# alvinliu0/HumanGaussian

Measured on AMD Instinct MI355X. Metric: rasterize fwd+bwd Gaussians/sec @1024^2, 100k pts, higher is better.
Workload: dtype f32

## Files before the change

### humangaussian_amd/csrc/api.hip

```cpp
#include "hgs_common.h"
#include <stdio.h>
#include <stdlib.h>
#include <algorithm>
#include <atomic>
#include <mutex>

#ifdef HGS_TIMELINE
__device__ unsigned long long hgs_tl[HGS_TL_KERNELS][HGS_TL_SLOTS][4];
#endif
#include "preprocess.hip"
#include "binning.hip"
#include "render_fwd.hip"
#include "knn.hip"
#include "mesh.hip"
#include "fields.hip"
#include "bookkeeping.hip"

extern "C" __global__ void hgs_k_render_bwd(View, Layout, const hgs_status*, const SortRec*, const float*,
                                            const float*, const float*, const float*, const float*,
                                            const float*, const float*, float*, uint32_t);
extern "C" __global__ void hgs_k_pair_reduce_em(View, Layout, const hgs_status*, const SortRec*, const float*, float*, uint32_t, uint32_t);
extern "C" __global__ void hgs_k_pair_reduce_ch(View, Layout, const hgs_status*, const SortRec*, const float*, float*, uint32_t, uint32_t);

namespace {

#ifdef HGS_KNOBS
inline int hgs_knob(const char* name, int dflt) { const char* e = getenv(name); return (e && atoi(e) > 0) ? atoi(e) : dflt; }
#else
inline int hgs_knob(const char*, int dflt) { return dflt; }
#endif

#define HGS_CHUNK_ROWS_MIN_VIEWS 3
#ifndef HGS_PRE_BWD_VPAR_MIN_VIEWS
#define HGS_PRE_BWD_VPAR_MIN_VIEWS 2
#endif
constexpr size_t ALIGN = 256;
struct Carver {
  size_t off = 0;
  size_t take(size_t bytes) { const size_t o = off; off = hgs_align_up(off + bytes, ALIGN); return o; }
};
constexpr size_t HGS_LDS_BINS_MAX = 16384;
#define HGS_BIN_WGS_PER_VIEW_MAX 512
#define HGS_BIN_WGS_TOTAL_MAX 1024
constexpr int HGS_MAX_BIN_WGS_PER_VIEW = HGS_BIN_WGS_PER_VIEW_MAX;
constexpr int HGS_BIN_WGS_TOTAL = HGS_BIN_WGS_TOTAL_MAX;

struct GeomCarve {
  size_t geom, tile_n, tile_start, tile_order, tile_rec, cell_info, items_part, fwd_cells,
      hist, tile_gbase, tile_count, chunk_sums, chunk_base, ctr, status, total;
};

inline int grid_dim(int pixels) { return (pixels + HGS_TILE - 1) / HGS_TILE; }

inline void bin_shape(int B, int P, int& nblk, int& cpw, int& nwg) {
  nblk = (P + HGS_BLOCK - 1) / HGS_BLOCK;
  int want = HGS_BIN_WGS_TOTAL / (B > 0 ? B : 1);
  if (want > HGS_MAX_BIN_WGS_PER_VIEW) want = HGS_MAX_BIN_WGS_PER_VIEW;
  if (want < 1) want = 1;
  cpw = (nblk + want - 1) / want;
  if (cpw < 1) cpw = 1;
  nwg = (nblk + cpw - 1) / cpw;
}

GeomCarve carve_geom(int B, int P, int H, int W) {
  const size_t T = (size_t)grid_dim(W) * grid_dim(H);
  const size_t TT = T * (size_t)B;
  int nblk, cpw, nwg;
  bin_shape(B, P, nblk, cpw, nwg);
  const bool lds = T <= HGS_LDS_BINS_MAX;
  GeomCarve c;
  Carver cv;
  c.geom = cv.take((size_t)B * P * sizeof(GeomRec));
  c.tile_n = cv.take(TT * 4);
  c.tile_start = cv.take(TT * 4);
  c.tile_order = cv.take(TT * 4);
  c.tile_rec = cv.take(TT * 16);
  c.cell_info = cv.take(TT * 16 * sizeof(CellInfo));
  const size_t dcap = hgs_die_cells((int)TT);
  c.items_part = cv.take(HGS_NXCD * 2 * dcap * sizeof(uint4));
  c.fwd_cells = cv.take((size_t)HGS_NXCD * HGS_NFC * dcap * 4);
  c.hist = cv.take(lds ? (size_t)B * nwg * T * 4 : 0);
  c.tile_gbase = cv.take(lds ? (size_t)HGS_ROW_GROUPS * TT * 4 : 0);
  c.tile_count = cv.take(lds ? 0 : TT * 4);
  c.chunk_sums = cv.take((size_t)B * nblk * 4);
  c.chunk_base = cv.take((size_t)B * nblk * 4);
  c.ctr = cv.take(sizeof(Counters));
  c.status = cv.take(sizeof(hgs_status));
  c.total = cv.off;
  return c;
}

struct BinCarve { size_t keys, recs, cell_list, entpair, cstate, items_full, total; };

BinCarve carve_bin(int64_t cap) {
  BinCarve c;
  Carver cv;
  const size_t C = (size_t)(cap > 0 ? cap : 0);
  const size_t NP = C * HGS_PAIRS_PER_ENTRY;
  c.keys = cv.take(C * 8);
  c.recs = cv.take(C * sizeof(SortRec));
  c.cell_list = cv.take(NP * 8);
  c.entpair = cv.take(C * 8);
  c.cstate = cv.take((NP / HGS_SEGLEN + 1) * HGS_CSTATE_FLOATS * sizeof(float));
// ... 355 lines not shown
    if ((scales != nullptr) != (rotations != nullptr)) return HGS_ESHAPE;
    if (has_sr == (cov3D_precomp != nullptr)) return HGS_ESHAPE;
    if (shs && M < (s->sh_degree + 1) * (s->sh_degree + 1)) return HGS_ESHAPE;
    if (entry_capacity > 0 && !bin) return HGS_EINVAL;
    if ((int64_t)B * P >= (1ll << 31) || P >= (1 << 28)) return HGS_EINVAL;
  }
  if (entry_capacity > HGS_MAX_ENTRY_CAPACITY) return HGS_EINVAL;
  hipStream_t stream = static_cast<hipStream_t>(stream_);
  DeviceState* const ds = device_state(stream);
  const int ncu = cu_count(ds);
  const bool aa = (activation_flags & HGS_ANTIALIAS) != 0;
  const View v = make_view(s, B, P, M, entry_capacity, max_tile_entries_hint > 0 ? max_tile_entries_hint : 0,
                           activation_flags & 7);
  const Layout L = make_layout(geom, bin, img, B, P, v.H, v.W, entry_capacity);
  hgs_status* status_dev =
      reinterpret_cast<hgs_status*>(static_cast<char*>(geom) + carve_geom(B, P, v.H, v.W).status);

  HGS_STAGE(0);
  hipError_t e = hipSuccess;
  if (v.nblk == 0) {
    e = hipMemsetAsync(L.ctr, 0, sizeof(Counters), stream);
    if (e != hipSuccess) return hip_rc(e);
  }
  const size_t lds_bytes = (size_t)v.T * 4;
  if (!v.lds_bins) {
    e = hipMemsetAsync(L.tile_count, 0, (size_t)v.TT * 4, stream);
    if (e != hipSuccess) return hip_rc(e);
  }
  if (v.nblk > 0) {
    if (v.lds_bins)
      hipLaunchKernelGGL(aa ? hgs_k_preprocess_fwd_aa : hgs_k_preprocess_fwd, dim3(v.B * v.nwg), dim3(HGS_BLOCK), lds_bytes,
                         stream, v, L, means3D, shs, colors_precomp, opacities, scales, rotations,
                         cov3D_precomp, radii, means2D_leaf);
    else
      hipLaunchKernelGGL(aa ? hgs_k_preprocess_fwd_ga_aa : hgs_k_preprocess_fwd_ga, dim3(v.B * v.nblk), dim3(HGS_BLOCK), 0,
                         stream, v, L, means3D, shs, colors_precomp, opacities, scales, rotations,
                         cov3D_precomp, radii, means2D_leaf);
    HGS_LAUNCH_CHECK();
  }
  HGS_STAGE(1);
  const unsigned bpv = (unsigned)((v.T + HGS_TILES_PER_WG - 1) / HGS_TILES_PER_WG);
  hipLaunchKernelGGL(hgs_k_tiles, dim3(bpv * (unsigned)v.B), dim3(64 * HGS_ROW_GROUPS), 0, stream, v, L);
  HGS_LAUNCH_CHECK();
  HGS_STAGE(2);
  const unsigned order_wgs = (unsigned)((v.TT + HGS_BLOCK - 1) / HGS_BLOCK);
  hgs_status* status_mapped = status_host_mapped ? status_host : nullptr;
  const unsigned nbin = entry_capacity > 0 ? (unsigned)(v.B * (v.lds_bins ? v.nwg : v.nblk)) : 0u;
  if (v.lds_bins && nbin)
    hipLaunchKernelGGL(hgs_k_fill, dim3(nbin + order_wgs), dim3(HGS_BLOCK), lds_bytes, stream, v, L, status_dev,
                       status_mapped, (int)nbin);
  else
    hipLaunchKernelGGL(hgs_k_fill_ga, dim3(nbin + order_wgs), dim3(HGS_BLOCK), 0, stream, v, L, status_dev,
                       status_mapped, (int)nbin);
  HGS_LAUNCH_CHECK();
  if (status_host && !status_host_mapped) {
    e = hipMemcpyAsync(status_host, status_dev, sizeof(hgs_status), hipMemcpyDeviceToHost, stream);
    if (e != hipSuccess) return hip_rc(e);
  }
  if (status_event) {
    e = hipEventRecord(static_cast<hipEvent_t>(status_event), stream);
    if (e != hipSuccess) return hip_rc(e);
  }
  if (entry_capacity > 0) {
    HGS_STAGE(3);
    auto class_grid = [&](int64_t lo) {
      const int64_t g = entry_capacity / lo + 1;
      return (unsigned)(g < v.TT ? g : v.TT);
    };
    const int hint = v.max_tile_hint;
    const bool need_huge = hint <= 0 || hint > 16384, need_large = hint <= 0 || hint > HGS_SORT_LDS_MAX;
    const bool expect_long = hint <= 0 || hint > HGS_SORT_LDS_MAX + HGS_SORT_LDS_MAX / 2 + 64;
    SideStream* side = ((need_huge || need_large) && expect_long) ? side_stream(ds) : nullptr;
    {
      std::unique_lock<std::mutex> side_lk;
      hipStream_t s2 = stream;
      if (side) {
        side_lk = std::unique_lock<std::mutex>(side->mu);
        e = hipEventRecord(side->fork, stream);
        if (e == hipSuccess) e = hipStreamWaitEvent(side->s, side->fork, 0);
        if (e != hipSuccess) return hip_rc(e);
        s2 = side->s;
      }
      if (need_huge) {
        hipLaunchKernelGGL(hgs_k_sort_huge, dim3(class_grid(16384)), dim3(1024), 0, s2, v, L, status_dev);
        HGS_LAUNCH_CHECK();
      }
      if (need_large) {
        hipLaunchKernelGGL(hgs_k_sort_large, dim3(class_grid(HGS_SORT_LDS_MAX)), dim3(1024), 0, s2, v, L, status_dev);
        HGS_LAUNCH_CHECK();
      }
      if (side) {
        e = hipEventRecord(side->join, side->s);
        if (e != hipSuccess) return hip_rc(e);
      }
      const unsigned sort_wgs = std::min<unsigned>(class_grid(1), (unsigned)(hgs_knob("HGS_SORT_WGS_PER_CU", 3) * ncu));
      hipLaunchKernelGGL(v.pairchunks ? hgs_k_sort_lds_ch : hgs_k_sort_lds, dim3(sort_wgs), dim3(HGS_SORT_NT), 0, stream, v, L,
                         status_dev);
      HGS_LAUNCH_CHECK();
      if (side) {
        e = hipStreamWaitEvent(stream, side->join, 0);
        if (e != hipSuccess) return hip_rc(e);
      }
    }
  } else {
    HGS_STAGE(3);
  }
  HGS_STAGE(4);
  {
    const int64_t cells = std::min<int64_t>((int64_t)16 * v.TT, (int64_t)HGS_PAIRS_PER_ENTRY * entry_capacity);
    const int64_t fwd_blocks = (int64_t)hgs_knob("HGS_FWD_BLOCKS_PER_CU", 4) * ncu;
    const unsigned cell_blocks = (unsigned)std::max<int64_t>(4, std::min<int64_t>(fwd_blocks, (cells + 3) / 4) & ~int64_t(3));
    const unsigned bg_blocks = (unsigned)v.TT;
    hipLaunchKernelGGL(store_bwd_state ? hgs_k_render_fwd_store : hgs_k_render_fwd_nostore, dim3(cell_blocks + bg_blocks),
                       dim3(HGS_FWD_THREADS), 0, stream, v, L, cell_blocks, status_dev, status_mapped, L.recs, L.cstate,
                       out_color, out_depth, out_alpha);
  }
  HGS_LAUNCH_CHECK();
  HGS_STAGE(5);
  return HGS_OK;
}

int hgs_forward_batch(const hgs_settings* s, int32_t B, int32_t P, int32_t M, const float* means3D,
                      const float* shs, const float* colors_precomp, const float* opacities,
                      const float* scales, const float* rotations, const float* cov3D_precomp,
                      float* out_color, float* out_depth, float* out_alpha, int32_t* radii,
                      void* geom, void* bin, int64_t entry_capacity, void* img,
                      int32_t store_bwd_state, int32_t max_tile_entries_hint, hgs_status* status_host,
                      int32_t status_host_mapped, void* status_event, void* const* stage_events,
                      void* stream_) {
  return hgs_forward_batch_act(s, B, P, M, means3D, shs, colors_precomp, opacities, scales, rotations, cov3D_precomp,
                               out_color, out_depth, out_alpha, radii, geom, bin, entry_capacity, img, store_bwd_state,
                               max_tile_entries_hint, status_host, status_host_mapped, status_event, stage_events, 0,
                               stream_);
}

int hgs_forward(const hgs_settings* s, int32_t P, int32_t M, const float* means3D,
                const float* shs, const float* colors_precomp, const float* opacities,
                const float* scales, const float* rotations, const float* cov3D_precomp,
                float* out_color, float* out_depth, float* out_alpha, int32_t* radii,
                void* geom, void* bin, int64_t entry_capacity, void* img,
                int32_t store_bwd_state, int32_t max_tile_entries_hint, hgs_status* status_host,
                int32_t status_host_mapped, void* status_event, void* const* stage_events,
                void* stream_) {
  return hgs_forward_batch(s, 1, P, M, means3D, shs, colors_precomp, opacities, scales, rotations,
                           cov3D_precomp, out_color, out_depth, out_alpha, radii, geom, bin, entry_capacity,
                           img, store_bwd_state, max_tile_entries_hint, status_host, status_host_mapped,
                           status_event, stage_events, stream_);
}

}

namespace {
int backward_impl(const hgs_settings* s, int32_t B, int32_t P, int32_t M, const float* means3D,
                           const float* shs, const float* colors_precomp, const float* opacities,
                           const float* scales, const float* rotations, const float* cov3D_precomp,
                           const int32_t* radii, const float* out_color, const float* out_depth,
                           const float* out_alpha, const float* dL_dout_color,
                           const float* dL_dout_depth, const float* dL_dout_alpha, const void* geom,
                           const void* bin, const void* img, const hgs_status* status,
                           int64_t entry_capacity, void* bwd_scratch, float* dL_dmeans3D, float* dL_dmeans2D, float* dL_dshs,
                           float* dL_dcolors_precomp, float* dL_dopacities, float* dL_dscales,
                           float* dL_drotations, float* dL_dcov3D_precomp, void* const* stage_events,
                           int32_t activation_flags, float* pack, int32_t pack_F, void* stream_) {
  (void)radii;
  if (activation_flags & ~(7 | HGS_GRAD_SCALE_TRUE_DERIVATIVE | HGS_ANTIALIAS)) return HGS_EINVAL;
  if ((activation_flags & (HGS_ACT_OPACITY_SIGMOID | HGS_ANTIALIAS)) && P > 0 && !opacities) return HGS_EINVAL;
  if (!batch_ok(s, B) || P < 0 || !geom || !img || entry_capacity < 0 || entry_capacity > HGS_MAX_ENTRY_CAPACITY) return HGS_EINVAL;
  if (status && status->overflow) return HGS_EINVAL;
  if (status && (int64_t)status->reserved[0] != entry_capacity) return HGS_EINVAL;
  if (P == 0) return HGS_OK;
  if (!means3D || !out_color || !out_depth || !out_alpha) return HGS_EINVAL;
  if ((shs != nullptr) == (colors_precomp != nullptr)) return HGS_ESHAPE;
  if ((scales != nullptr) != (rotations != nullptr)) return HGS_ESHAPE;
  if ((scales != nullptr) == (cov3D_precomp != nullptr)) return HGS_ESHAPE;
  if (shs && !dL_dshs) return HGS_EINVAL;
  const bool maybe_entries = status ? status->num_rendered > 0 : entry_capacity > 0;
  if (maybe_entries && (!bin || !bwd_scratch)) return HGS_EINVAL;
  hipStream_t stream = static_cast<hipStream_t>(stream_);
  DeviceState* const ds = device_state(stream);
  const int64_t cap = entry_capacity;
  const View v = make_view(s, B, P, M, cap, 0, activation_flags);
  const Layout L = make_layout(const_cast<void*>(geom), const_cast<void*>(bin),
                               const_cast<void*>(img), B, P, v.H, v.W, cap);
  const hgs_status* status_dev = reinterpret_cast<const hgs_status*>(
      static_cast<const char*>(geom) + carve_geom(B, P, v.H, v.W).status);
  const int64_t X = status ? (int64_t)status->num_rendered : cap;
  const int64_t worst = X * HGS_PAIRS_PER_ENTRY;
  const int64_t pc = (status && status->num_pairs > 0 && (int64_t)status->num_pairs < worst) ? (int64_t)status->num_pairs : worst;
  const uint32_t pair_cap = (uint32_t)(pc > 0xffffffffll ? 0xffffffffll : pc);
  float* rows = static_cast<float*>(bwd_scratch);
  float* pair_rows = rows + (size_t)X * HGS_ROW_FLOATS;
  HGS_STAGE(0);
  if (maybe_entries) {
    const int resident = hgs_knob("HGS_BWD_WAVES_PER_CU", 12) * cu_count(ds);
    hipLaunchKernelGGL(hgs_k_render_bwd, dim3((unsigned)std::max(HGS_NXCD, resident / HGS_BWD_BLOCK_WAVES / HGS_NXCD * HGS_NXCD)), dim3(64 * HGS_BWD_BLOCK_WAVES), 0, stream, v, L, status_dev, L.recs, L.cstate,
                       out_color, out_depth, out_alpha, dL_dout_color, dL_dout_depth, dL_dout_alpha, pair_rows, pair_cap);
    HGS_LAUNCH_CHECK();
    HGS_STAGE(1);
    if (X > 0) {
      const uint32_t R_host = status ? status->num_rendered : 0xffffffffu;
      hipLaunchKernelGGL(v.pairchunks ? hgs_k_pair_reduce_ch : hgs_k_pair_reduce_em, dim3((unsigned)((X + 255) / 256)), dim3(256), 0,
                         stream, v, L, status_dev, L.recs, pair_rows, rows, pair_cap, R_host);
      HGS_LAUNCH_CHECK();
    }
  }
  if (!maybe_entries) HGS_STAGE(1);
  HGS_STAGE(2);
  const int deg = shs ? v.D : 0;
  const int nc = (deg + 1) * (deg + 1);
  const int aa = (activation_flags & HGS_ANTIALIAS) ? 1 : 0;
  const unsigned thr_p = 64u * (unsigned)v.B;
  const size_t lds_p = (size_t)(23 + 3 * nc) * thr_p * sizeof(float);
  const int row_p = hgs_pre_bwd_row(aa, 2, deg);
  const bool vpar_ok = v.B >= HGS_PRE_BWD_VPAR_MIN_VIEWS && thr_p <= (unsigned)hgs_pre_bwd_forms.row[row_p].threads &&
                       (lds_p <= 65536 || pre_bwd_lds_raised(ds, row_p));
  const int mode = v.B == 1 ? 1 : (vpar_ok ? 2 : 0);
  const PreBwdForm& form = hgs_pre_bwd_forms.row[hgs_pre_bwd_row(aa, mode, deg)];
  const unsigned grid = mode == 2 ? (unsigned)((v.P + 63) / 64) : (unsigned)v.nblk, threads = mode == 2 ? thr_p : HGS_BLOCK;
  const size_t lds = mode == 2 ? lds_p : (mode == 1 ? hgs_pre_bwd_stage_bytes(M, deg, shs != nullptr && dL_dshs != nullptr) : 0);
  hipLaunchKernelGGL(form.kernel, dim3(grid), dim3(threads), lds, stream, v, L, status_dev, rows, means3D, shs,
                     colors_precomp, opacities, scales, rotations, cov3D_precomp, dL_dmeans3D, dL_dmeans2D,
                     dL_dshs, dL_dcolors_precomp, dL_dopacities, dL_dscales, dL_drotations,
                     dL_dcov3D_precomp, pack, (int)pack_F);
  HGS_LAUNCH_CHECK();
  HGS_STAGE(3);
  return HGS_OK;
}
}

extern "C" {

int hgs_backward_batch_act(const hgs_settings* s, int32_t B, int32_t P, int32_t M, const float* means3D,
                           const float* shs, const float* colors_precomp, const float* opacities,
                           const float* scales, const float* rotations, const float* cov3D_precomp,
                           const int32_t* radii, const float* out_color, const float* out_depth,
                           const float* out_alpha, const float* dL_dout_color,
                           const float* dL_dout_depth, const float* dL_dout_alpha, const void* geom,
                           const void* bin, const void* img, const hgs_status* status,
                           int64_t entry_capacity, void* bwd_scratch, float* dL_dmeans3D, float* dL_dmeans2D, float* dL_dshs,
                           float* dL_dcolors_precomp, float* dL_dopacities, float* dL_dscales,
                           float* dL_drotations, float* dL_dcov3D_precomp, void* const* stage_events,
                           int32_t activation_flags, void* stream_) {
  return backward_impl(s, B, P, M, means3D, shs, colors_precomp, opacities, scales, rotations, cov3D_precomp, radii, out_color,
                       out_depth, out_alpha, dL_dout_color, dL_dout_depth, dL_dout_alpha, geom, bin, img, status,
                       entry_capacity, bwd_scratch, dL_dmeans3D, dL_dmeans2D, dL_dshs, dL_dcolors_precomp, dL_dopacities,
                       dL_dscales, dL_drotations, dL_dcov3D_precomp, stage_events, activation_flags, nullptr, 0, stream_);
}

int hgs_backward_batch_packed(const hgs_settings* s, int32_t B, int32_t P, int32_t M, const float* means3D,
                              const float* shs, const float* opacities, const float* scales, const float* rotations,
                              const int32_t* radii, const float* out_color, const float* out_depth, const float* out_alpha,
                              const float* dL_dout_color, const float* dL_dout_depth, const float* dL_dout_alpha,
                              const void* geom, const void* bin, const void* img, const hgs_status* status,
                              int64_t entry_capacity, void* bwd_scratch, float* pack, float* dL_dmeans2D_views,
                              void* const* stage_events, int32_t activation_flags, void* stream_) {
  if (!pack || !shs || !scales || !rotations || M < 1) return P == 0 ? HGS_OK : HGS_EINVAL;
  float* marker = pack;
  return backward_impl(s, B, P, M, means3D, shs, nullptr, opacities, scales, rotations, nullptr, radii, out_color, out_depth,
                       out_alpha, dL_dout_color, dL_dout_depth, dL_dout_alpha, geom, bin, img, status, entry_capacity,
                       bwd_scratch, marker, dL_dmeans2D_views, marker, nullptr, marker, marker, marker, nullptr, stage_events,
                       activation_flags, pack, 15 + 3 * M, stream_);
}

int hgs_backward_batch(const hgs_settings* s, int32_t B, int32_t P, int32_t M, const float* means3D,
                       const float* shs, const float* colors_precomp, const float* opacities,
                       const float* scales, const float* rotations, const float* cov3D_precomp,
                       const int32_t* radii, const float* out_color, const float* out_depth,
                       const float* out_alpha, const float* dL_dout_color,
                       const float* dL_dout_depth, const float* dL_dout_alpha, const void* geom,
                       const void* bin, const void* img, const hgs_status* status,
                       int64_t entry_capacity, void* bwd_scratch, float* dL_dmeans3D, float* dL_dmeans2D, float* dL_dshs,
                       float* dL_dcolors_precomp, float* dL_dopacities, float* dL_dscales,
                       float* dL_drotations, float* dL_dcov3D_precomp, void* const* stage_events,
                       void* stream_) {
  return hgs_backward_batch_act(s, B, P, M, means3D, shs, colors_precomp, opacities, scales, rotations, cov3D_precomp,
                                radii, out_color, out_depth, out_alpha, dL_dout_color, dL_dout_depth, dL_dout_alpha,
                                geom, bin, img, status, entry_capacity, bwd_scratch, dL_dmeans3D, dL_dmeans2D, dL_dshs,
                                dL_dcolors_precomp, dL_dopacities, dL_dscales, dL_drotations, dL_dcov3D_precomp,
// ... 372 lines not shown
```

### humangaussian_amd/csrc/binning.hip

```cpp
#include "hgs_common.h"

extern "C" __global__ void __launch_bounds__(64 * HGS_ROW_GROUPS)
hgs_k_tiles(View v, Layout L) {
  __shared__ uint32_t gt[HGS_ROW_GROUPS][HGS_TILES_PER_WG];
  __shared__ uint32_t start_s[HGS_TILES_PER_WG];
  __shared__ uint32_t cls_s[HGS_NCLS];
  const int tid = threadIdx.x, tl = tid & 63;
  const int rg = __builtin_amdgcn_readfirstlane(tid >> 6);
  const int bpv = (v.T + HGS_TILES_PER_WG - 1) / HGS_TILES_PER_WG;
  const int b = (int)blockIdx.x / bpv;
  const int t = ((int)blockIdx.x % bpv) * HGS_TILES_PER_WG + tl;
  const bool valid = t < v.T;
  const size_t g = (size_t)b * v.T + t;
  if (tid < HGS_NCLS) cls_s[tid] = 0;
  uint32_t run = 0;
  if (v.lds_bins) {
    const int rpg = (v.nwg + HGS_ROW_GROUPS - 1) / HGS_ROW_GROUPS;
    const int r0 = rg * rpg, r1 = min(v.nwg, r0 + rpg);
    if (valid) {
      uint32_t* col = L.hist + (size_t)b * v.nwg * v.T + t;
      constexpr int BR = 16;
      for (int r = r0; r < r1; r += BR) {
        uint32_t c[BR];
#pragma unroll
// ... 99 lines not shown
  const int g = blk * HGS_BLOCK + tid;
  const bool valid = g < v.TT;
  const uint32_t n = valid ? L.tile_n[g] : 0u;
  const int c = (valid && n) ? 32 - __clz(n) : 0;
  int leader_of = 0;
  uint32_t rank = 0, cnt = 0;
  unsigned long long todo = __ballot(valid);
  while (todo) {
    const int leader = (int)__builtin_ctzll(todo);
    const int cl = __builtin_amdgcn_readlane(c, leader);
    const unsigned long long same = __ballot(valid && c == cl);
    if (valid && c == cl) {
      leader_of = leader;
      rank = __builtin_amdgcn_mbcnt_hi((uint32_t)(same >> 32), __builtin_amdgcn_mbcnt_lo((uint32_t)same, 0u));
      cnt = (uint32_t)__popcll(same);
    }
    todo &= ~same;
  }
  uint32_t base = 0;
  if (valid && lane == leader_of) base = atomicAdd(&L.ctr->cls_cur[c].v, cnt);
  base = (uint32_t)__shfl((int)base, leader_of, 64);
  const uint32_t pos = cls_base[c] + base + rank;
  if (!valid) return;
  L.tile_order[pos] = (uint32_t)g;
  L.tile_rec[pos] = make_uint4((uint32_t)g, n, L.tile_start[g], 0u);
}

extern "C" __global__ void __launch_bounds__(HGS_BLOCK)
hgs_k_fill(View v, Layout L, hgs_status* __restrict__ status, hgs_status* __restrict__ status_host, int nbin) {
  extern __shared__ __attribute__((aligned(16))) uint32_t lds_cur[];
  if ((int)blockIdx.x >= nbin) {
    place_tiles(v, L, (int)blockIdx.x - nbin, (int)gridDim.x - nbin, status, status_host);
    return;
  }
  if (overflow_from_counters(v, L)) return;
  const int b = (int)blockIdx.x / v.nwg, lw = (int)blockIdx.x % v.nwg;
  const uint32_t* __restrict__ base_row = L.hist + (size_t)blockIdx.x * v.T;
  const int rpg = (v.nwg + HGS_ROW_GROUPS - 1) / HGS_ROW_GROUPS;
  const uint32_t* __restrict__ grp_row = L.tile_gbase + (size_t)(lw / rpg) * v.TT + (size_t)b * v.T;
  for (int t = threadIdx.x; t < v.T; t += HGS_BLOCK) lds_cur[t] = grp_row[t] + base_row[t];
  __syncthreads();
  const GeomRec* __restrict__ geom = L.geom + (size_t)b * v.P;
  for (int c = 0; c < v.cpw; ++c) {
    const int chunk = lw * v.cpw + c;
    if (chunk >= v.nblk) break;
    const int i = chunk * HGS_BLOCK + threadIdx.x;
    if (i >= v.P) continue;
    const uint4 q2 = reinterpret_cast<const uint4*>(&geom[i])[2];
    const uint32_t depth_bits = q2.y, lo = q2.z, hi = q2.w;
    const int minx = lo & 0xffffu, miny = lo >> 16, maxx = hi & 0xffffu, maxy = hi >> 16;
    const unsigned long long key_hi = (unsigned long long)depth_bits << 32;
    for (int ty = miny; ty < maxy; ++ty)
      for (int tx = minx; tx < maxx; ++tx) {
        const uint32_t slot = atomicAdd(&lds_cur[ty * v.grid_x + tx], 1u);
        L.keys[slot] = key_hi | (uint32_t)i;
      }
  }
}

extern "C" __global__ void __launch_bounds__(HGS_BLOCK)
hgs_k_fill_ga(View v, Layout L, hgs_status* __restrict__ status, hgs_status* __restrict__ status_host, int nbin) {
  if ((int)blockIdx.x >= nbin) {
    place_tiles(v, L, (int)blockIdx.x - nbin, (int)gridDim.x - nbin, status, status_host);
    return;
  }
  if (overflow_from_counters(v, L)) return;
  const int b = (int)blockIdx.x / v.nblk, chunk = (int)blockIdx.x % v.nblk;
  const int i = chunk * HGS_BLOCK + threadIdx.x;
  if (i >= v.P) return;
  const uint4 q2 = reinterpret_cast<const uint4*>(&L.geom[(size_t)b * v.P + i])[2];
  const uint32_t depth_bits = q2.y, lo = q2.z, hi = q2.w;
  const int minx = lo & 0xffffu, miny = lo >> 16, maxx = hi & 0xffffu, maxy = hi >> 16;
  const unsigned long long key_hi = (unsigned long long)depth_bits << 32;
  for (int ty = miny; ty < maxy; ++ty)
    for (int tx = minx; tx < maxx; ++tx) {
      const size_t g = (size_t)b * v.T + ty * v.grid_x + tx;
      const uint32_t slot = L.tile_start[g] + atomicAdd(&L.tile_count[g], 1u);
      L.keys[slot] = key_hi | (uint32_t)i;
    }
}

namespace {

__device__ __forceinline__ void hgs_put_pair(const Layout& L, uint32_t rec, uint32_t row_id, uint32_t slot) {
  L.cell_list[slot] = make_uint2(rec, row_id);
}

struct CellAlloc {
  uint32_t len, nfull, rem, nst, i_len, i_st, i_full, pcls, fcls, frank, die;
  unsigned long long b1, b2, b3, got;
};

__device__ __forceinline__ void hgs_alloc_cell_ranges_issue(const Layout& L, uint32_t order_pos, uint32_t len_of_lane, CellAlloc& a) {
  const int lane = (int)threadIdx.x & 63;
  a.die = order_pos % HGS_NXCD;
  const bool cl = lane < 16;
  a.len = cl ? len_of_lane : 0u;
  a.nfull = a.len / HGS_SEGLEN; a.rem = a.len % HGS_SEGLEN;
  const uint32_t nseg = a.nfull + (a.rem ? 1u : 0u);
  a.nst = nseg ? nseg - 1u : 0u;
  a.i_len = hgs_wave_incl_scan(a.len); a.i_st = hgs_wave_incl_scan(a.nst); a.i_full = hgs_wave_incl_scan(a.nfull);
  a.pcls = a.rem ? hgs_item_class(a.rem) : 0u;
  a.b1 = __ballot(a.pcls == 1u); a.b2 = __ballot(a.pcls == 2u); a.b3 = __ballot(a.pcls == 3u);
  const uint32_t t_len = (uint32_t)__builtin_amdgcn_readlane((int)a.i_len, 63);
  const uint32_t t_st = (uint32_t)__builtin_amdgcn_readlane((int)a.i_st, 63);
  const uint32_t t_full = (uint32_t)__builtin_amdgcn_readlane((int)a.i_full, 63);
  a.fcls = hgs_cell_class(a.len);
  unsigned long long fb_ = 0;
  a.frank = 0;
#pragma unroll
  for (int c = 0; c < HGS_NFC; ++c) {
    const unsigned long long bc = __ballot(cl && a.len && a.fcls == (uint32_t)c);
    if (lane == 3 + c) fb_ = bc;
    if (a.fcls == (uint32_t)c) a.frank = (uint32_t)__popcll(bc & ((1ull << lane) - 1ull));
  }
  const unsigned long long add = lane == 0 ? ((unsigned long long)t_len | ((unsigned long long)t_st << 32))
                               : lane == 1 ? ((unsigned long long)t_full | ((unsigned long long)__popcll(a.b1) << 32))
                               : lane == 2 ? ((unsigned long long)__popcll(a.b2) | ((unsigned long long)__popcll(a.b3) << 32))
                                           : (unsigned long long)__popcll(fb_);
  a.got = 0;
  unsigned long long* ctr = lane == 0 ? &L.ctr->alloc_ps : &L.ctr->sched[a.die][min(lane, 2 + HGS_NFC) - 1];
  if (lane < 3 + HGS_NFC && add) a.got = atomicAdd(ctr, add);
}

__device__ __forceinline__ void hgs_alloc_cell_ranges_finish(const View& v, const Layout& L, int g, const CellAlloc& a,
                                                             uint32_t* cell_base, uint32_t& pair_base_out) {
  int lane = (int)threadIdx.x & 63;
  asm volatile("" : "+v"(lane));
  const bool cl = lane < 16;
  const uint32_t fpos = (uint32_t)__shfl((int)(uint32_t)a.got, 3 + (int)a.fcls, 64) + a.frank;
  const uint32_t got_lo = (uint32_t)a.got, got_hi = (uint32_t)(a.got >> 32);
  const uint32_t pb = (uint32_t)__builtin_amdgcn_readlane((int)got_lo, 0);
  const uint32_t sb = (uint32_t)__builtin_amdgcn_readlane((int)got_hi, 0);
  const uint32_t fb = (uint32_t)__builtin_amdgcn_readlane((int)got_lo, 1);
  const uint32_t p1 = (uint32_t)__builtin_amdgcn_readlane((int)got_hi, 1);
  const uint32_t p2 = (uint32_t)__builtin_amdgcn_readlane((int)got_lo, 2);
  const uint32_t p3 = (uint32_t)__builtin_amdgcn_readlane((int)got_hi, 2);
  if (cl) {
    const uint32_t len = a.len, nfull = a.nfull, rem = a.rem;
    const uint32_t base = pb + a.i_len - len;
    cell_base[lane] = base;
    CellInfo ci;
    ci.base = base; ci.len = len; ci.sbase = sb + a.i_st - a.nst; ci.pbase = pb;
    L.cell_info[(size_t)g * 16 + lane] = ci;
    const uint32_t key = (uint32_t)g * 16u + (uint32_t)lane;
    const size_t dcap = hgs_die_cells(v.TT);
    if (len) L.fwd_cells[((size_t)a.die * HGS_NFC + a.fcls) * dcap + fpos] = key;
    uint4* full = L.items_full + ((size_t)a.die * L.full_cap + fb + a.i_full - nfull);
    for (uint32_t sgm = 0; sgm < nfull; ++sgm)
      full[sgm] = make_uint4(key, HGS_SEGLEN, base + sgm * HGS_SEGLEN, sgm ? ci.sbase + sgm - 1u : 0xffffffffu);
    if (rem) {
      const unsigned long long below = (1ull << lane) - 1ull;
      uint4* part = L.items_part + (size_t)a.die * 2 * dcap;
      const uint4 it = make_uint4(key, rem, base + nfull * HGS_SEGLEN, nfull ? ci.sbase + nfull - 1u : 0xffffffffu);
      if (a.pcls == 1u) part[p1 + (uint32_t)__popcll(a.b1 & below)] = it;
      else if (a.pcls == 2u) part[dcap - 1 - (p2 + (uint32_t)__popcll(a.b2 & below))] = it;
      else part[dcap + p3 + (uint32_t)__popcll(a.b3 & below)] = it;
    }
  }
  if (lane == 0) pair_base_out = pb;
}

__device__ __forceinline__ void hgs_alloc_cell_ranges(const View& v, const Layout& L, int g, uint32_t order_pos, const uint32_t* cell_tot,
                                                      uint32_t* cell_base, uint32_t& pair_base_out) {
  if (threadIdx.x < 64) {
    CellAlloc a;
    hgs_alloc_cell_ranges_issue(L, order_pos, (threadIdx.x & 63) < 16 ? cell_tot[threadIdx.x & 63] : 0u, a);
    hgs_alloc_cell_ranges_finish(v, L, g, a, cell_base, pair_base_out);
  }
}

template <int MAXCH>
struct GatherLds {
  uint32_t tab[MAXCH][17];
  uint32_t run[17];
  uint32_t cell_tot[16];
  uint32_t cell_base[16];
  uint32_t pair_base;
};

template <int MAXCH>
__device__ __forceinline__ void gather_records(const View& v, const Layout& L, int g, uint32_t order_pos,
                                               uint32_t start, uint32_t n,
                                               unsigned long long* sorted, int nt, GatherLds<MAXCH>& S) {
  const int t = g % v.T;
  const GeomRec* __restrict__ geom = L.geom + (size_t)(g / v.T) * v.P;
  const uint32_t* __restrict__ cbase = L.chunk_base + (size_t)(g / v.T) * v.nblk;
  const int tx = t % v.grid_x, ty = t / v.grid_x;
  const float x0 = (float)(tx * HGS_TILE), y0 = (float)(ty * HGS_TILE);
  const int tid = (int)threadIdx.x, lane = tid & 63;
  const int wv = tid >> 6, nwaves = nt >> 6;
  if (tid < 16) S.cell_tot[tid] = 0;
  if (tid < 17) S.run[tid] = 0;
  __syncthreads();
  constexpr int GU = 4;
  uint32_t mytot = 0;
  for (uint32_t kb0 = 0; kb0 < n; kb0 += (uint32_t)nt * GU) {
    const uint32_t kb = kb0 + threadIdx.x;
    uint32_t idxv[GU];
    uint4 q0[GU], q1[GU], q2[GU];
    uint32_t q3[GU];
#pragma unroll
    for (int u = 0; u < GU; ++u) {
      const uint32_t k = kb + (uint32_t)u * nt;
      idxv[u] = (k < n) ? (uint32_t)sorted[k] : 0u;
    }
#pragma unroll
    for (int u = 0; u < GU; ++u) {
      const uint32_t k = kb + (uint32_t)u * nt;
      if (k < n) {
        const uint4* gp = reinterpret_cast<const uint4*>(&geom[idxv[u]]);
        q0[u] = gp[0]; q1[u] = gp[1]; q2[u] = gp[2]; q3[u] = gp[3].x;
      }
    }
#pragma unroll
    for (int u = 0; u < GU; ++u) {
      const uint32_t k = kb + (uint32_t)u * nt;
      uint32_t mask = 0;
      if (k < n) {
        const uint32_t idx = idxv[u];
        const uint4 g0 = q0[u], g1 = q1[u], g2 = q2[u];
        const int minx = g2.z & 0xffffu, miny = g2.z >> 16, maxx = g2.w & 0xffffu;
        const uint32_t entry = cbase[idx >> 8] + q3[u] + (uint32_t)((ty - miny) * (maxx - minx) + (tx - minx));
        const float mx = __uint_as_float(g0.x), my = __uint_as_float(g0.y);
        const float ca = __uint_as_float(g0.z), cb = __uint_as_float(g0.w), cc = __uint_as_float(g1.x);
        mask = hgs_cell_mask(mx, my, ca, cb, cc, __uint_as_float(g1.y), x0, y0);
        uint4* dst = reinterpret_cast<uint4*>(&L.recs[start + k]);
        const float qa = -0.5f * ca * HGS_LOG2E, qb = -cb * HGS_LOG2E, qc = -0.5f * cc * HGS_LOG2E;
        dst[0] = make_uint4(g0.x, g0.y, __float_as_uint(qa), __float_as_uint(qb));
        dst[1] = make_uint4(__float_as_uint(qc), g1.y, g1.z, g1.w);
        dst[2] = make_uint4(g2.x, g2.y, entry, v.pairchunks ? hgs_rec_tag(mask, k, n, false) : 0u);
        L.entpair[start + k].x = entry | ((uint32_t)__popc(mask) << 27);
        sorted[k] = (unsigned long long)mask;
      }
#pragma unroll
      for (int c = 0; c < 16; ++c) {
        const unsigned long long bal = __ballot((mask >> c) & 1u);
        if (lane == c) mytot += (uint32_t)__popcll(bal);
      }
    }
  }
  if (lane < 16 && mytot) atomicAdd(&S.cell_tot[lane], mytot);
  __syncthreads();
  hgs_alloc_cell_ranges(v, L, g, order_pos, S.cell_tot, S.cell_base, S.pair_base);
  __syncthreads();
  const uint32_t pair_base = S.pair_base;
  for (uint32_t sc0 = 0; sc0 < n; sc0 += (uint32_t)MAXCH * 64u) {
    const uint32_t nch = min((uint32_t)MAXCH, (n - sc0 + 63u) / 64u);
    for (uint32_t ch = wv; ch < nch; ch += nwaves) {
      const uint32_t k = sc0 + ch * 64u + lane;
      const uint32_t mask = (k < n) ? (uint32_t)sorted[k] : 0u;
      uint32_t mine = 0;
#pragma unroll
      for (int c = 0; c < 16; ++c) {
        const unsigned long long bal = __ballot((mask >> c) & 1u);
        if (lane == c) mine = (uint32_t)__popcll(bal);
      }
      uint32_t tot = mine;
      tot += __builtin_amdgcn_update_dpp(0, (int)tot, HGS_DPP_ROW_SHR(1), 0xf, 0xf, false);
      tot += __builtin_amdgcn_update_dpp(0, (int)tot, HGS_DPP_ROW_SHR(2), 0xf, 0xf, false);
      tot += __builtin_amdgcn_update_dpp(0, (int)tot, HGS_DPP_ROW_SHR(4), 0xf, 0xf, false);
      tot += __builtin_amdgcn_update_dpp(0, (int)tot, HGS_DPP_ROW_SHR(8), 0xf, 0xf, false);
      if (lane < 16) S.tab[ch][lane] = mine;
      if (lane == 15) S.tab[ch][16] = tot;
    }
    __syncthreads();
    for (int col = wv; col < 17; col += nwaves) {
      uint32_t carry = S.run[col];
      for (uint32_t c0 = 0; c0 < nch; c0 += 64u) {
        const uint32_t ch = c0 + lane;
        const uint32_t x = ch < nch ? S.tab[ch][col] : 0u;
        const uint32_t inc = hgs_wave_incl_scan(x);
        if (ch < nch) S.tab[ch][col] = carry + inc - x;
        carry += (uint32_t)__builtin_amdgcn_readlane((int)inc, 63);
      }
      if (lane == 0) S.run[col] = carry;
    }
    __syncthreads();
    for (uint32_t ch = wv; ch < nch; ch += nwaves) {
      const uint32_t k = sc0 + ch * 64u + lane;
      const bool in = k < n;
      const uint32_t mask = in ? (uint32_t)sorted[k] : 0u;
      const uint32_t cnt = (uint32_t)__popc(mask);
      const uint32_t rel = S.tab[ch][16] + hgs_wave_incl_scan(cnt) - cnt;
      if (in) L.entpair[start + k].y = pair_base + rel;
#pragma unroll
      for (int c = 0; c < 16; ++c) {
        const bool bit = (mask >> c) & 1u;
        const unsigned long long bal = __ballot(bit);
        if (bit) {
          const uint32_t rank = S.tab[ch][c] + __builtin_amdgcn_mbcnt_hi((uint32_t)(bal >> 32), __builtin_amdgcn_mbcnt_lo((uint32_t)bal, 0u));
          const uint32_t slot = S.cell_base[c] + rank;
          hgs_put_pair(L, start + k, pair_base + rel + (uint32_t)__popc(mask & ((1u << c) - 1u)), slot);
        }
      }
    }
    __syncthreads();
  }
}

__device__ __forceinline__ uint32_t hgs_spread4(uint32_t nib) {
  return (nib * 0x00204081u) & 0x01010101u;
}
__device__ __forceinline__ uint32_t hgs_bytesum(uint32_t w) { return __builtin_amdgcn_sad_u8(w, 0u, 0u); }

template <int MAXCH>
__device__ __forceinline__ void gather_records_single(const View& v, const Layout& L, int g, uint32_t order_pos,
                                                      uint32_t start, uint32_t n,
                                                      unsigned long long* sorted, int nt, GatherLds<MAXCH>& S) {
  const int t = g % v.T;
  const GeomRec* __restrict__ geom = L.geom + (size_t)(g / v.T) * v.P;
  const uint32_t* __restrict__ cbase = L.chunk_base + (size_t)(g / v.T) * v.nblk;
  const int tx = t % v.grid_x, ty = t / v.grid_x;
  const float x0 = (float)(tx * HGS_TILE), y0 = (float)(ty * HGS_TILE);
  const int tid = (int)threadIdx.x, lane = tid & 63;
  const int wv = tid >> 6, nwaves = nt >> 6;
  const uint32_t nch = (n + 63u) / 64u;
#ifdef HGS_TIMELINE
  const unsigned long long tg0 = wall_clock64();
#define HGS_TG(i) const unsigned long long tg##i = wall_clock64()
#else
#define HGS_TG(i)
#endif
  constexpr int GU = 2;
  for (uint32_t kb0 = 0; kb0 < n; kb0 += (uint32_t)nt * GU) {
    const uint32_t kb = kb0 + threadIdx.x;
    uint32_t idxv[GU];
    uint4 q0[GU], q1[GU], q2[GU];
    uint32_t q3[GU];
#pragma unroll
    for (int u = 0; u < GU; ++u) {
      const uint32_t k = kb + (uint32_t)u * nt;
      idxv[u] = (k < n) ? (uint32_t)sorted[k] : 0u;
    }
#pragma unroll
    for (int u = 0; u < GU; ++u) {
      const uint32_t k = kb + (uint32_t)u * nt;
      if (k < n) {
        const uint4* gp = reinterpret_cast<const uint4*>(&geom[idxv[u]]);
        q0[u] = gp[0]; q1[u] = gp[1]; q2[u] = gp[2]; q3[u] = gp[3].x;
      }
    }
#pragma unroll
    for (int u = 0; u < GU; ++u) {
      const uint32_t k = kb + (uint32_t)u * nt;
      if (kb0 + (uint32_t)u * nt + (uint32_t)(wv * 64) >= n) continue;
      uint32_t mask = 0;
      if (k < n) {
        const uint32_t idx = idxv[u];
        const uint4 g0 = q0[u], g1 = q1[u], g2 = q2[u];
        const int minx = g2.z & 0xffffu, miny = g2.z >> 16, maxx = g2.w & 0xffffu;
        const uint32_t entry = cbase[idx >> 8] + q3[u] + (uint32_t)((ty - miny) * (maxx - minx) + (tx - minx));
        const float mx = __uint_as_float(g0.x), my = __uint_as_float(g0.y);
        const float ca = __uint_as_float(g0.z), cb = __uint_as_float(g0.w), cc = __uint_as_float(g1.x);
        mask = hgs_cell_mask(mx, my, ca, cb, cc, __uint_as_float(g1.y), x0, y0);
        uint4* dst = reinterpret_cast<uint4*>(&L.recs[start + k]);
        const float qa = -0.5f * ca * HGS_LOG2E, qb = -cb * HGS_LOG2E, qc = -0.5f * cc * HGS_LOG2E;
        dst[0] = make_uint4(g0.x, g0.y, __float_as_uint(qa), __float_as_uint(qb));
        dst[1] = make_uint4(__float_as_uint(qc), g1.y, g1.z, g1.w);
        dst[2] = make_uint4(g2.x, g2.y, entry, v.pairchunks ? hgs_rec_tag(mask, k, n, false) : 0u);
        L.entpair[start + k].x = entry | ((uint32_t)__popc(mask) << 27);
        sorted[k] = (unsigned long long)mask;
      }
      const uint32_t ch = k >> 6;
      uint32_t tot[4];
#pragma unroll
      for (int wd = 0; wd < 4; ++wd) tot[wd] = hgs_wave_incl_scan(hgs_spread4((mask >> (4 * wd)) & 0xfu));
      if (lane == 63) {
        S.tab[ch][0] = tot[0]; S.tab[ch][1] = tot[1]; S.tab[ch][2] = tot[2]; S.tab[ch][3] = tot[3];
        S.tab[ch][16] = hgs_bytesum(tot[0]) + hgs_bytesum(tot[1]) + hgs_bytesum(tot[2]) + hgs_bytesum(tot[3]);
      }
    }
  }
  __syncthreads();
  HGS_TG(1);
  {
    uint32_t pk[(MAXCH + 63) / 64][4];
#pragma unroll
    for (int r = 0; r < (MAXCH + 63) / 64; ++r) {
      const uint32_t ch = (uint32_t)r * 64u + lane;
#pragma unroll
      for (int wd = 0; wd < 4; ++wd) pk[r][wd] = (wv < 5 && ch < nch) ? S.tab[ch][wd] : 0u;
    }
    __syncthreads();
    for (int col = wv; col < 5; col += nwaves) {
      uint32_t carry[4] = {0u, 0u, 0u, 0u};
#pragma unroll
      for (int r = 0; r < (MAXCH + 63) / 64; ++r) {
        const uint32_t ch = (uint32_t)r * 64u + lane;
        if ((uint32_t)r * 64u >= nch) break;
        if (col < 4) {
#pragma unroll
          for (int b = 0; b < 4; ++b) {
            const uint32_t x = (pk[r][col] >> (8 * b)) & 0xffu;
            const uint32_t inc = hgs_wave_incl_scan(x);
            if (ch < nch) S.tab[ch][4 * col + b] = carry[b] + inc - x;
            carry[b] += (uint32_t)__builtin_amdgcn_readlane((int)inc, 63);
          }
        } else {
          const uint32_t x = ch < nch ? S.tab[ch][16] : 0u;
          const uint32_t inc = hgs_wave_incl_scan(x);
          if (ch < nch) S.tab[ch][16] = carry[0] + inc - x;
          carry[0] += (uint32_t)__builtin_amdgcn_readlane((int)inc, 63);
        }
      }
      if (col < 4 && lane < 4) S.cell_tot[4 * col + lane] = lane == 0 ? carry[0] : lane == 1 ? carry[1] : lane == 2 ? carry[2] : carry[3];
    }
  }
  __syncthreads();
  HGS_TG(2);
  hgs_alloc_cell_ranges(v, L, g, order_pos, S.cell_tot, S.cell_base, S.pair_base);
  __syncthreads();
  HGS_TG(3);
  const uint32_t pair_base = S.pair_base;
  for (uint32_t ch = wv; ch < nch; ch += nwaves) {
    const uint32_t k = ch * 64u + lane;
    const bool in = k < n;
    uint32_t mask = in ? (uint32_t)sorted[k] : 0u;
    uint32_t ex[4], before = 0;
#pragma unroll
    for (int wd = 0; wd < 4; ++wd) {
      const uint32_t mine = hgs_spread4((mask >> (4 * wd)) & 0xfu);
      ex[wd] = hgs_wave_incl_scan(mine) - mine;
      before += hgs_bytesum(ex[wd]);
    }
    const uint32_t rel = S.tab[ch][16] + before;
    if (in) L.entpair[start + k].y = pair_base + rel;
    uint32_t r = 0;
    while (mask) {
      const int c = __builtin_ctz(mask);
      mask &= mask - 1u;
      const uint32_t exw = (c < 8) ? (c < 4 ? ex[0] : ex[1]) : (c < 12 ? ex[2] : ex[3]);
      const uint32_t slot = S.cell_base[c] + S.tab[ch][c] + ((exw >> (8 * (c & 3))) & 0xffu);
      hgs_put_pair(L, start + k, pair_base + rel + r, slot);
      ++r;
    }
  }
#ifdef HGS_TIMELINE
  if (threadIdx.x == 0 && blockIdx.x < HGS_TL_SLOTS) {
    const unsigned long long tg4 = wall_clock64();
    auto cl = [](unsigned long long d) { return d > 0xffffull ? 0xffffull : d; };
    hgs_tl[2][blockIdx.x][0] = cl(tg1 - tg0) | (cl(tg2 - tg1) << 16) | (cl(tg3 - tg2) << 32) | (cl(tg4 - tg3) << 48);
  }
#endif
}

template <int NT>
__device__ __forceinline__ void bitonic_sort(unsigned long long* keys, uint32_t n) {
  uint32_t npad = 2;
  while (npad < n) npad <<= 1;
  const uint32_t half = npad >> 1;
  for (uint32_t kk = 2; kk <= npad; kk <<= 1) {
    const uint32_t hk = kk >> 1;
    for (uint32_t i = threadIdx.x; i < half; i += NT) {
      const uint32_t blk = i / hk, off = i - blk * hk;
      const uint32_t lo = blk * kk + off, hi = blk * kk + (kk - 1 - off);
      if (hi < n) {
        const unsigned long long a = keys[lo], c = keys[hi];
        if (a > c) { keys[lo] = c; keys[hi] = a; }
      }
    }
    __syncthreads();
    for (uint32_t j = kk >> 2; j > 0; j >>= 1) {
      for (uint32_t i = threadIdx.x; i < half; i += NT) {
        const uint32_t lo = ((i & ~(j - 1)) << 1) | (i & (j - 1));
        const uint32_t hi = lo | j;
        if (hi < n) {
          const unsigned long long a = keys[lo], c = keys[hi];
          if (a > c) { keys[lo] = c; keys[hi] = a; }
        }
      }
      __syncthreads();
    }
  }
}

typedef unsigned long long u64;

}

#define HGS_SORT_LIGHT 16
#define HGS_RANK_BUCKET_MAX 192
#define HGS_RANK_NB_MAX 2048
#define HGS_SORT_NT 256
#define HGS_SORT_WAVES_PER_EU 3
#define HGS_RANK_GU 2

namespace {

#ifdef HGS_TIMELINE
__shared__ unsigned long long hgs_s_tq[8];
#define HGS_TQ(i) { if (threadIdx.x == 0) hgs_s_tq[(i)] = wall_clock64(); }
#else
#define HGS_TQ(i) {}
#endif

__device__ __forceinline__ void lds_barrier() { asm volatile("s_waitcnt lgkmcnt(0)\n\ts_barrier" ::: "memory"); }

struct __attribute__((aligned(16))) RankLds {
  uint32_t hist[HGS_RANK_NB_MAX + 1];
  uint32_t wtot[16];
  uint32_t tot16[8];
  uint32_t dmin, dmax, maxcnt, pad;
};
static_assert(sizeof(uint32_t) * (HGS_RANK_NB_MAX + 1) >= sizeof(uint16_t) * 4096, "the masks of the longest list fit into the histogram");

template <int NT>
__device__ __forceinline__ void bucket_scan(RankLds& R, uint32_t NB) {
  int tid = (int)threadIdx.x;
  asm volatile("" : "+v"(tid));
  const int lane = tid & 63, wv = tid >> 6;
  const uint32_t PER = NB / (uint32_t)NT;
  uint32_t* __restrict__ h = R.hist + (uint32_t)tid * PER;
  uint32_t c[8];
  auto load_counts = [&]() {
#pragma unroll
    for (int i = 0; i < 8; ++i) c[i] = 0u;
    if (PER == 8u) {
      const uint4 a = *reinterpret_cast<const uint4*>(h), b = *reinterpret_cast<const uint4*>(h + 4);
      c[0] = a.x; c[1] = a.y; c[2] = a.z; c[3] = a.w; c[4] = b.x; c[5] = b.y; c[6] = b.z; c[7] = b.w;
    } else if (PER == 4u) {
      const uint4 a = *reinterpret_cast<const uint4*>(h);
      c[0] = a.x; c[1] = a.y; c[2] = a.z; c[3] = a.w;
    } else if (PER == 2u) {
      const uint2 a = *reinterpret_cast<const uint2*>(h);
      c[0] = a.x; c[1] = a.y;
    } else {
      c[0] = h[0];
    }
  };
  load_counts();
  uint32_t sum = 0, mx = 0;
#pragma unroll
  for (int i = 0; i < 8; ++i) { sum += c[i]; mx = max(mx, c[i]); }
  const uint32_t inc = hgs_wave_incl_scan(sum);
  mx = hgs_wave_max_u32(mx);
  if (lane == 63) R.wtot[wv] = inc;
  if (lane == 0 && mx) atomicMax(&R.maxcnt, mx);
  uint32_t base = inc - sum;
  asm volatile("" : "+v"(base));
  lds_barrier();
  load_counts();
#pragma unroll
  for (int w = 0; w < NT / 64; ++w) base += (w < wv) ? R.wtot[w] : 0u;
  uint32_t e[8];
#pragma unroll
  for (int i = 0; i < 8; ++i) { e[i] = base; base += c[i]; }
  if (PER == 8u) {
    *reinterpret_cast<uint4*>(h) = make_uint4(e[0], e[1], e[2], e[3]);
    *reinterpret_cast<uint4*>(h + 4) = make_uint4(e[4], e[5], e[6], e[7]);
  } else if (PER == 4u) {
    *reinterpret_cast<uint4*>(h) = make_uint4(e[0], e[1], e[2], e[3]);
  } else if (PER == 2u) {
    *reinterpret_cast<uint2*>(h) = make_uint2(e[0], e[1]);
  } else {
    h[0] = e[0];
  }
}

template <int NT, bool CH>
__device__ __forceinline__ void cell_lists_from_masks(const View& v, const Layout& L, uint32_t order_pos, uint32_t start, uint32_t n,
                                                      const uint16_t* __restrict__ masks, GatherLds<64>& S, const CellAlloc& ca,
                                                      unsigned long long* tp) {
  const int tid = (int)threadIdx.x, lane = tid & 63, wv = tid >> 6;
  constexpr int nwaves = NT / 64;
  const uint32_t nch = (n + 63u) / 64u;
  for (uint32_t ch = wv; ch < nch; ch += nwaves) {
    const uint32_t k = ch * 64u + lane;
    const uint32_t mask = (k < n) ? (uint32_t)masks[k] : 0u;
    uint32_t tot[4];
#pragma unroll
    for (int wd = 0; wd < 4; ++wd) tot[wd] = hgs_wave_incl_scan(hgs_spread4((mask >> (4 * wd)) & 0xfu));
    if (lane == 63) {
      S.tab[ch][0] = tot[0]; S.tab[ch][1] = tot[1]; S.tab[ch][2] = tot[2]; S.tab[ch][3] = tot[3];
      S.tab[ch][16] = hgs_bytesum(tot[0]) + hgs_bytesum(tot[1]) + hgs_bytesum(tot[2]) + hgs_bytesum(tot[3]);
    }
  }
  lds_barrier();
  {
    uint32_t pk[4];
    const uint32_t ch = (uint32_t)lane;
#pragma unroll
    for (int wd = 0; wd < 4; ++wd) pk[wd] = (ch < nch) ? S.tab[ch][wd] : 0u;
    lds_barrier();
    for (int col = wv; col < 5; col += nwaves) {
      if (col < 4) {
        const uint32_t word = col == 0 ? pk[0] : col == 1 ? pk[1] : col == 2 ? pk[2] : pk[3];
#pragma unroll
        for (int b = 0; b < 4; ++b) {
          const uint32_t x = (word >> (8 * b)) & 0xffu;
          const uint32_t inc = hgs_wave_incl_scan(x);
          if (ch < nch) S.tab[ch][4 * col + b] = inc - x;
        }
      } else {
        const uint32_t x = ch < nch ? S.tab[ch][16] : 0u;
        const uint32_t inc = hgs_wave_incl_scan(x);
        if (ch < nch) S.tab[ch][16] = inc - x;
      }
    }
  }
#ifdef HGS_TIMELINE
  tp[2] = wall_clock64();
#endif
  if (tid < 64) hgs_alloc_cell_ranges_finish(v, L, (int)L.tile_rec[order_pos].x, ca, S.cell_base, S.pair_base);
  lds_barrier();
#ifdef HGS_TIMELINE
  tp[3] = wall_clock64();
#endif
  const uint32_t pair_base = S.pair_base;
  for (uint32_t ch = wv; ch < nch; ch += nwaves) {
    const uint32_t k = ch * 64u + lane;
    const bool in = k < n;
    const uint32_t mask = in ? (uint32_t)masks[k] : 0u;
    uint32_t ex[4], before = 0;
    uint32_t tot[4];
#pragma unroll
    for (int wd = 0; wd < 4; ++wd) {
      const uint32_t mine = hgs_spread4((mask >> (4 * wd)) & 0xfu);
      const uint32_t inc = hgs_wave_incl_scan(mine);
      ex[wd] = inc - mine;
      if (CH) tot[wd] = (uint32_t)__builtin_amdgcn_readlane((int)inc, 63);
      before += hgs_bytesum(ex[wd]);
    }
    const uint32_t rel_chunk = pair_base + S.tab[ch][16];
    const uint32_t rel = rel_chunk + before;
    if (in) L.entpair[start + k].y = CH ? rel_chunk : rel;
    const uint32_t cb = lane < 16 ? S.cell_base[lane] + S.tab[ch][lane] : 0u;
    uint32_t cp = 0;
#pragma unroll
    for (int c = 0; c < 16; ++c) {
      const uint32_t cbase = (uint32_t)__builtin_amdgcn_readlane((int)cb, c);
      if ((mask >> c) & 1u) {
        const uint32_t exc = (ex[c >> 2] >> (8 * (c & 3))) & 0xffu;
        const uint32_t slot = cbase + exc;
        hgs_put_pair(L, start + k, CH ? rel_chunk + cp + exc : rel + (uint32_t)__popc(mask & ((1u << c) - 1u)), slot);
      }
      if (CH) cp += (tot[c >> 2] >> (8 * (c & 3))) & 0xffu;
    }
  }
}

template <int E, int NT>
__device__ __forceinline__ bool rank_keys(const Layout& L, uint32_t start, uint32_t n, uint32_t NB, const u64 (&keyp)[HGS_RANK_GU],
                                          unsigned long long* pairs, RankLds& R) {
  int tid = (int)threadIdx.x;
  asm volatile("" : "+v"(tid));
  const int lane = tid & 63, wv = tid >> 6;
  u64 key[E];
#pragma unroll
  for (int e = 0; e < E; ++e) {
    if (e < HGS_RANK_GU) key[e] = keyp[e];
    else {
      const uint32_t k = (uint32_t)e * NT + (uint32_t)tid;
      const u64 kv = L.keys[start + min(k, n - 1u)];
      key[e] = (k < n) ? kv : ~0ull;
    }
  }
  {
    uint32_t lo = 0xffffffffu, hi = 0u;
#pragma unroll
    for (int e = 0; e < E; ++e) {
      const uint32_t d = (uint32_t)(key[e] >> 32);
      lo = min(lo, d);
      hi = max(hi, key[e] != ~0ull ? d : 0u);
    }
    hi = hgs_wave_max_u32(hi);
    lo = ~hgs_wave_max_u32(~lo);
    lds_barrier();
    if (lane == 0) { atomicMin(&R.dmin, lo); atomicMax(&R.dmax, hi); }
  }
  lds_barrier();
  HGS_TQ(0)
  const float flo = __uint_as_float(R.dmin);
  const float range = __uint_as_float(R.dmax) - flo;
  const float scale = range > 1e-30f ? (float)NB / range : 0.0f;
  uint32_t bp[E];
#pragma unroll
  for (int e = 0; e < E; ++e) {
    bp[e] = 0u;
    if (key[e] != ~0ull) {
      const float x = (__uint_as_float((uint32_t)(key[e] >> 32)) - flo) * scale;
      const uint32_t bkt = (uint32_t)fminf(x, (float)(NB - 1u));
      bp[e] = bkt | (atomicAdd(&R.hist[bkt], 1u) << 12);
    }
  }
  lds_barrier();
  HGS_TQ(1)
  bucket_scan<NT>(R, NB);
  if (tid == 0) R.hist[NB] = n;
  lds_barrier();
  HGS_TQ(2)
  const bool degenerate = R.maxcnt > (uint32_t)HGS_RANK_BUCKET_MAX;
  if (!degenerate) {
    constexpr int EG = E < 8 ? E : 8;
    uint32_t lmax[E / EG];
#pragma unroll
    for (int h = 0; h < E / EG; ++h) lmax[h] = 0u;
#pragma unroll
    for (int e = 0; e < E; ++e) {
      if (key[e] != ~0ull) {
        const uint32_t j0 = R.hist[bp[e] & 0xfffu], j1 = R.hist[(bp[e] & 0xfffu) + 1u];
        pairs[j0 + (bp[e] >> 12)] = key[e];
        bp[e] = j0 | ((j1 - j0) << 12);
        lmax[e / EG] = max(lmax[e / EG], j1 - j0);
      }
    }
    lds_barrier();
    HGS_TQ(3)
#pragma unroll
    for (int h = 0; h < E / EG; ++h) {
      for (uint32_t sidx = 0; sidx < lmax[h]; ++sidx) {
        u64 other[EG];
#pragma unroll
        for (int e = 0; e < EG; ++e) {
          const uint32_t w = bp[h * EG + e];
          const bool on = sidx < ((w >> 12) & 0xffu);
          other[e] = pairs[on ? (w & 0xfffu) + sidx : 0u];
        }
// ... 48 lines not shown
    }
    hi = hgs_wave_max_u32(hi);
    lo = ~hgs_wave_max_u32(~lo);
    lds_barrier();
    if (lane == 0) { atomicMin(&R.dmin, lo); atomicMax(&R.dmax, hi); }
  }
  lds_barrier();
  const float flo = __uint_as_float(R.dmin);
  const float range = __uint_as_float(R.dmax) - flo;
  const float scale = range > 1e-30f ? (float)NB / range : 0.0f;
  const float bmax = (float)(NB - 1u);
  auto bucket_of = [&](u64 key) { return (uint32_t)fminf((__uint_as_float((uint32_t)(key >> 32)) - flo) * scale, bmax); };
#pragma unroll 4
  for (uint32_t k = tid; k < n; k += NT) atomicAdd(&R.hist[bucket_of(keys[k])], 1u);
  lds_barrier();
  bucket_scan<NT>(R, NB);
  lds_barrier();
  const bool degenerate = R.maxcnt > (uint32_t)HGS_RANK_BUCKET_MAX;
  uint32_t rk[16];
  if (!degenerate) {
#pragma unroll 4
    for (uint32_t k = tid; k < n; k += NT) {
      const u64 key = keys[k];
      pairs[atomicAdd(&R.hist[bucket_of(key)], 1u)] = key;
    }
    lds_barrier();
#pragma unroll
    for (int e0 = 0; e0 < 16; e0 += 4) {
      if ((uint32_t)e0 * NT >= n) break;
      u64 key[4];
      uint32_t w[4], lmax = 0;
#pragma unroll
      for (int e = 0; e < 4; ++e) {
        const uint32_t k = (uint32_t)(e0 + e) * NT + (uint32_t)tid;
        key[e] = keys[min(k, last)];
      }
#pragma unroll
      for (int e = 0; e < 4; ++e) {
        const uint32_t k = (uint32_t)(e0 + e) * NT + (uint32_t)tid;
        const uint32_t b = bucket_of(key[e]);
        const uint32_t j1 = R.hist[b], j0 = b ? R.hist[b - 1u] : 0u;
        const uint32_t len = k < n ? j1 - j0 : 0u;
        w[e] = j0 | (len << JB);
        lmax = max(lmax, len);
      }
      for (uint32_t sidx = 0; sidx < lmax; ++sidx) {
        u64 other[4];
#pragma unroll
        for (int e = 0; e < 4; ++e) {
          const bool on = sidx < ((w[e] >> JB) & 0xffu);
          other[e] = pairs[on ? (w[e] & JM) + sidx : 0u];
        }
#pragma unroll
        for (int e = 0; e < 4; ++e) {
          const bool on = sidx < ((w[e] >> JB) & 0xffu);
          w[e] += (on && other[e] < key[e]) ? (1u << (JB + 8)) : 0u;
        }
      }
#pragma unroll
      for (int e = 0; e < 4; ++e) rk[e0 + e] = (w[e] & JM) + (w[e] >> (JB + 8));
    }
    lds_barrier();
#pragma unroll
    for (int e = 0; e < 16; ++e) {
      const uint32_t k = (uint32_t)e * NT + (uint32_t)tid;
      if (k < n) {
        if (SORTED) pairs[rk[e]] = keys[k];
        else pairs[k] = (keys[k] & 0xffffffffull) | ((u64)rk[e] << 32);
      }
    }
    if (SORTED) lds_barrier();
  } else {
    for (uint32_t k = tid; k < n; k += NT) pairs[k] = keys[k];
    __syncthreads();
    bitonic_sort<NT>(pairs, n);
    if (!SORTED) {
      for (uint32_t k = tid; k < n; k += NT) pairs[k] = (pairs[k] & 0xffffffffull) | ((u64)k << 32);
      lds_barrier();
    }
  }
  return degenerate;
}

template <int NT, bool CH>
__device__ __forceinline__ void rank_sort_tile(const View& v, const Layout& L, uint32_t order_pos, int g, uint32_t start, uint32_t n,
                                               unsigned long long* pairs, RankLds& R, GatherLds<64>& S, bool& degenerate_out,
                                               unsigned long long* tp) {
  const int tid = (int)threadIdx.x, lane = tid & 63;
  constexpr int GU = HGS_RANK_GU;
  const int t = g % v.T;
  const GeomRec* __restrict__ geom = L.geom + (size_t)(g / v.T) * v.P;
  const uint32_t* __restrict__ cbase = L.chunk_base + (size_t)(g / v.T) * v.nblk;
  const int tx = t % v.grid_x, ty = t / v.grid_x;
  const float x0 = (float)(tx * HGS_TILE), y0 = (float)(ty * HGS_TILE);
  uint32_t NB = 256u;
  while (NB < 2u * n && NB < (uint32_t)HGS_RANK_NB_MAX) NB <<= 1;
  for (uint32_t i = tid; i <= NB; i += NT) R.hist[i] = 0u;
  if (tid < 8) R.tot16[tid] = 0u;
  if (tid == 0) { R.dmin = 0xffffffffu; R.dmax = 0u; R.maxcnt = 0u; }
  u64 keyp[GU];
#pragma unroll
  for (int u = 0; u < GU; ++u) {
    const uint32_t k = (uint32_t)u * NT + (uint32_t)tid;
    const u64 kv = L.keys[start + min(k, n - 1u)];
    keyp[u] = (k < n) ? kv : ~0ull;
  }
  uint4 Aa[GU], Ab[GU], Ac[GU], Ba[GU], Bb[GU], Bc[GU];
  uint32_t Aoff[GU], Acb[GU], Boff[GU], Bcb[GU];
  u64 Apr[GU], Bpr[GU];
#define HGS_RANK_ISSUE(X, u, PR)                                                              \
  {                                                                                           \
    const u64 pr__ = (PR);                                                                    \
    const uint32_t idx__ = pr__ == ~0ull ? 0u : (uint32_t)pr__;                               \
    const uint4* gp__ = reinterpret_cast<const uint4*>(&geom[idx__]);                         \
    X##a[u] = gp__[0]; X##b[u] = gp__[1]; X##c[u] = gp__[2]; X##off[u] = gp__[3].x;           \
    X##cb[u] = cbase[idx__ >> 8];                                                             \
    X##pr[u] = pr__;                                                                          \
  }
  bool degenerate;
  const bool early = n <= 8u * NT;
  if (early) {
#pragma unroll
    for (int u = 0; u < GU; ++u) HGS_RANK_ISSUE(A, u, keyp[u]);
    if (n <= 2u * NT) degenerate = rank_keys<2, NT>(L, start, n, NB, keyp, pairs, R);
    else if (n <= 4u * NT) degenerate = rank_keys<4, NT>(L, start, n, NB, keyp, pairs, R);
    else degenerate = rank_keys<8, NT>(L, start, n, NB, keyp, pairs, R);
  } else {
    degenerate = rank_keys_stream<NT>(L, start, n, NB, pairs, R);
  }
  degenerate_out = degenerate;
#ifdef HGS_TIMELINE
  tp[0] = wall_clock64();
#endif
  uint16_t* __restrict__ masks = reinterpret_cast<uint16_t*>(R.hist);
  uint32_t acc[4] = {0u, 0u, 0u, 0u};
#define HGS_RANK_ROUND(X, r)                       \
  _Pragma("unroll") for (int u = 0; u < GU; ++u) {                                            \
    const uint32_t k__ = ((r) * (uint32_t)GU + (uint32_t)u) * NT + (uint32_t)tid;             \
    HGS_RANK_ISSUE(X, u, (k__ < n) ? pairs[k__] : ~0ull);                                     \
  }
#define HGS_RANK_CONSUME(X)                                                                   \
  _Pragma("unroll") for (int u = 0; u < GU; ++u) {                                            \
    if (X##pr[u] != ~0ull) {                                                                  \
      const uint32_t k = (uint32_t)(X##pr[u] >> 32);                                          \
      const uint4 g0 = X##a[u], g1 = X##b[u], g2 = X##c[u];                                   \
                           \
      const int minx = g2.z & 0xffffu, miny = g2.z >> 16, maxx = g2.w & 0xffffu;              \
      const uint32_t entry = X##cb[u] + X##off[u] + (uint32_t)((ty - miny) * (maxx - minx) + (tx - minx)); \
      const float mx = __uint_as_float(g0.x), my = __uint_as_float(g0.y);                     \
      const float ca = __uint_as_float(g0.z), cb = __uint_as_float(g0.w), cc = __uint_as_float(g1.x); \
      const uint32_t mask = hgs_cell_mask(mx, my, ca, cb, cc, __uint_as_float(g1.y), x0, y0); \
      uint4* dst = reinterpret_cast<uint4*>(&L.recs[start + k]);                              \
      const float qa = -0.5f * ca * HGS_LOG2E, qb = -cb * HGS_LOG2E, qc = -0.5f * cc * HGS_LOG2E; \
      dst[0] = make_uint4(g0.x, g0.y, __float_as_uint(qa), __float_as_uint(qb));              \
      dst[1] = make_uint4(__float_as_uint(qc), g1.y, g1.z, g1.w);                             \
      dst[2] = make_uint4(g2.x, g2.y, entry, CH ? hgs_rec_tag(mask, k, n, true) : 0u);        \
      L.entpair[start + k].x = entry | ((uint32_t)__popc(mask) << 27);    \
      masks[k] = (uint16_t)mask;                                                              \
      _Pragma("unroll") for (int wd = 0; wd < 4; ++wd) acc[wd] += hgs_spread4((mask >> (4 * wd)) & 0xfu); \
    }                                                                                         \
  }
  if (degenerate || !early) {
    HGS_RANK_ROUND(A, 0u)
  } else {
#pragma unroll
    for (int u = 0; u < GU; ++u) {
      const uint32_t k = (uint32_t)u * NT + (uint32_t)tid;
      Apr[u] = (k < n) ? pairs[k] : ~0ull;
    }
  }
  const uint32_t per_round = (uint32_t)GU * NT;
  for (uint32_t r = 0; r * per_round < n; r += 2u) {
    const bool hb = (r + 1u) * per_round < n, ha = (r + 2u) * per_round < n;
    if (hb) { HGS_RANK_ROUND(B, r + 1u) }
    HGS_RANK_CONSUME(A)
    if (r < 4u) HGS_TQ(4 + r)
    if (ha) { HGS_RANK_ROUND(A, r + 2u) }
    if (hb) { HGS_RANK_CONSUME(B) }
    if (r < 3u) HGS_TQ(5 + r)
  }
#undef HGS_RANK_ISSUE
#undef HGS_RANK_ROUND
#undef HGS_RANK_CONSUME
  {
    uint32_t w16[8];
#pragma unroll
    for (int wd = 0; wd < 4; ++wd) { w16[2 * wd] = acc[wd] & 0x00ff00ffu; w16[2 * wd + 1] = (acc[wd] >> 8) & 0x00ff00ffu; }
#pragma unroll
    for (int i = 0; i < 8; ++i) w16[i] = hgs_wave_incl_scan(w16[i]);
    if (lane == 63) {
#pragma unroll
      for (int i = 0; i < 8; ++i) if (w16[i]) atomicAdd(&R.tot16[i], w16[i]);
    }
  }
  lds_barrier();
#ifdef HGS_TIMELINE
  tp[1] = wall_clock64();
#endif
  CellAlloc ca;
  if (tid < 64) {
    const int c = lane & 15;
    const uint32_t word = R.tot16[2 * (c >> 2) + (c & 1)];
    hgs_alloc_cell_ranges_issue(L, order_pos, (word >> (16 * ((c >> 1) & 1))) & 0xffffu, ca);
  }
  cell_lists_from_masks<NT, CH>(v, L, order_pos, start, n, masks, S, ca, tp);
}

template <int NT, bool CH>
__device__ __forceinline__ void sort_rank_body(const View& v, const Layout& L, const hgs_status* __restrict__ status,
                                               unsigned long long* pairs, RankLds& R, GatherLds<64>& S) {
  if (status->overflow) return;
  const uint32_t active = status->active_tiles;
  const uint32_t G = gridDim.x, ncu = G / 3u, na = min(active, G);
  const bool remap = HGS_SORT_LIGHT > 0 && G == 3u * ncu && status->reserved[1] >= 768u &&
                     na >= 2u * ncu + 3u * (uint32_t)HGS_SORT_LIGHT;
  for (uint32_t b0 = blockIdx.x; b0 < active; b0 += gridDim.x) {
    uint32_t b = b0;
    if (remap && b0 < na) {
      constexpr uint32_t H = (uint32_t)HGS_SORT_LIGHT;
      if (b0 >= ncu && b0 < ncu + H) b = na - 1u - (b0 - ncu);
      else if (b0 >= 2u * ncu && b0 < 2u * ncu + H) b = na - 1u - H - (b0 - 2u * ncu);
      else if (b0 >= na - 2u * H) { const uint32_t j = na - 1u - b0; b = j < H ? ncu + j : 2u * ncu + (j - H); }
    }
    const uint4 tr = L.tile_rec[b];
    const int g = (int)tr.x;
    const uint32_t n = tr.y, start = tr.z;
    if (n == 0 || n > (uint32_t)HGS_SORT_LDS_MAX) continue;
#ifdef HGS_TIMELINE
    const unsigned long long tp0 = wall_clock64();
#endif
    bool degenerate;
    unsigned long long tp[4] = {0, 0, 0, 0};
    rank_sort_tile<NT, CH>(v, L, b, g, start, n, pairs, R, S, degenerate, tp);
#ifdef HGS_TIMELINE
    if (threadIdx.x == 0 && b < HGS_TL_SLOTS) {
      const unsigned long long tpe = wall_clock64();
      auto cl = [](unsigned long long d) { return d > 0xffffull ? 0xffffull : d; };
      hgs_tl[5][b][0] = tp0;
      hgs_tl[5][b][1] = tpe;
      hgs_tl[5][b][2] = degenerate ? 1 : 0;
      hgs_tl[5][b][3] = ((unsigned long long)1 << 32) | n;
      hgs_tl[2][b][0] = cl(tp[0] - tp0) | (cl(tp[1] - tp[0]) << 16) | (cl(tp[2] - tp[1]) << 32) | (cl(tp[3] - tp[2]) << 48);
      hgs_tl[2][b][1] = cl(tpe - tp[3]);
      hgs_tl[2][b][2] = cl(hgs_s_tq[0] - tp0) | (cl(hgs_s_tq[1] - hgs_s_tq[0]) << 16) | (cl(hgs_s_tq[2] - hgs_s_tq[1]) << 32) | (cl(hgs_s_tq[3] - hgs_s_tq[2]) << 48);
      hgs_tl[2][b][3] = cl(hgs_s_tq[4] - tp[0]) | (cl(hgs_s_tq[5] - tp[0]) << 16) | (cl(hgs_s_tq[6] - tp[0]) << 32) | (cl(hgs_s_tq[7] - tp[0]) << 48);
    }
#endif
    lds_barrier();
  }
}
}

static_assert(16 * HGS_SORT_NT >= 4096, "the rank sort takes every list of the LDS class");
#define HGS_SORT_LDS_KERNEL(NAME, CH)                                                                                  \
  extern "C" __global__ void __launch_bounds__(HGS_SORT_NT) __attribute__((amdgpu_waves_per_eu(HGS_SORT_WAVES_PER_EU, HGS_SORT_WAVES_PER_EU))) \
  NAME(View v, Layout L, const hgs_status* __restrict__ status) {                                                      \
    __shared__ unsigned long long pairs[4096];                                                                         \
    __shared__ GatherLds<64> S;                                                                                        \
    __shared__ RankLds R;                                                                                              \
    HGS_TL_BEGIN();                                                                                                    \
    sort_rank_body<HGS_SORT_NT, CH>(v, L, status, pairs, R, S);                                                        \
    HGS_TL_END(3, 0u);                                                                                                 \
  }
HGS_SORT_LDS_KERNEL(hgs_k_sort_lds, false)
HGS_SORT_LDS_KERNEL(hgs_k_sort_lds_ch, true)

extern "C" __global__ void __launch_bounds__(1024)
hgs_k_sort_large(View v, Layout L, const hgs_status* __restrict__ status) {
  __shared__ unsigned long long keys[16384];
  __shared__ GatherLds<256> S;
  if (status->overflow) return;
  const uint32_t b = blockIdx.x;
  if (b >= status->active_tiles) return;
  const int t = (int)L.tile_order[b];
  const uint32_t start = L.tile_start[t];
  const uint32_t n = L.tile_n[t];
  if (n <= (uint32_t)HGS_SORT_LDS_MAX || n > 16384u) return;
  {
    __shared__ RankLds R;
    const uint32_t NB = (uint32_t)HGS_RANK_NB_MAX;
    for (uint32_t i = threadIdx.x; i <= NB; i += 1024) R.hist[i] = 0u;
    if (threadIdx.x == 0) { R.dmin = 0xffffffffu; R.dmax = 0u; R.maxcnt = 0u; }
    rank_keys_stream<1024, true>(L, start, n, NB, keys, R);
    __syncthreads();
  }
  gather_records_single<256>(v, L, t, b, start, n, keys, 1024, S);
}

extern "C" __global__ void __launch_bounds__(1024)
hgs_k_sort_huge(View v, Layout L, const hgs_status* __restrict__ status) {
  if (status->overflow) return;
  const uint32_t b = blockIdx.x;
  if (b >= status->active_tiles) return;
  const int t = (int)L.tile_order[b];
  const uint32_t start = L.tile_start[t];
  const uint32_t n = L.tile_n[t];
  if (n <= 16384u) return;
  __shared__ GatherLds<256> S;
  bitonic_sort<1024>(L.keys + start, n);
  gather_records<256>(v, L, t, b, start, n, L.keys + start, 1024, S);
}
```

### humangaussian_amd/csrc/hgs_common.h

```cpp
#pragma once
#include <hip/hip_runtime.h>
#include <stdint.h>

#include "../../include/hgs_rast.h"
#include "cellmask.h"

#define HGS_TILE 16
#define HGS_TILE_PIX 256
#define HGS_BLOCK 256
#define HGS_ROW_GROUPS 16
#define HGS_TILES_PER_WG 64
#define HGS_RB 16
#define HGS_ROW_F4 (HGS_RB * 3 + 1)
#define HGS_BWD_BLOCK_WAVES 12
#define HGS_SEGLEN 128
#define HGS_PAIRS_PER_ENTRY 16
#define HGS_NEAR_Z 0.2f
#define HGS_ALPHA_MIN (1.0f / 255.0f)
#define HGS_ALPHA_MAX 0.99f
#define HGS_T_EPS 0.0001f
#define HGS_CSTATE_FLOATS (6 * 16)
#define HGS_ROW_FLOATS 12
#define HGS_GROW_F4 (HGS_ROW_FLOATS / 4)
#define HGS_PROW_FLOATS 10
#define HGS_PROW_F2 (HGS_PROW_FLOATS / 2)
#define HGS_SORT_LDS_MAX 4096
#define HGS_NCLS 33
#define HGS_NXCD 8
#define HGS_NFC 11

struct __attribute__((aligned(16))) GeomRec {
  float mx, my;
  float ca, cb, cc;
  float op;
  float r, g, b;
  float depth;
  uint32_t rect_lo;
  uint32_t rect_hi;
  uint32_t offset;
  int32_t radius;
  uint32_t clamped;
  uint32_t flags;
};

struct __attribute__((aligned(16))) SortRec {
  float mx, my;
  float qa, qb, qc;
  float op, r, g, b, depth;
  uint32_t entry;
  uint32_t pad;
};
#define HGS_LOG2E 1.4426950408889634f
__host__ __device__ __forceinline__ uint32_t hgs_rec_tag(uint32_t mask, uint32_t k, uint32_t n, bool chunk_rows) {
  const uint32_t left = n - (k & ~63u);
  return (mask & 0xffffu) | ((k & 63u) << 16) | (((left < 64u ? left : 64u) - 1u) << 22) | (chunk_rows ? 1u << 28 : 0u);
}

struct __attribute__((aligned(16))) CellInfo {
  uint32_t base;
  uint32_t len;
  uint32_t sbase;
  uint32_t pbase;
};

struct __attribute__((aligned(128))) CounterLine { uint32_t v; };
struct __attribute__((aligned(128))) Counters {
  unsigned long long alloc_eb;
  __attribute__((aligned(128))) uint32_t entry_alloc;
  __attribute__((aligned(128))) uint32_t max_n;
  CounterLine cls_hist[HGS_NCLS];
  CounterLine cls_cur[HGS_NCLS];
  __attribute__((aligned(128))) unsigned long long alloc_ps;
  __attribute__((aligned(128))) unsigned long long sched[HGS_NXCD][16];
};
static_assert(2 + HGS_NFC <= 16, "a die's row of work counters is one 128 B line");

__host__ __device__ __forceinline__ uint32_t hgs_item_class(uint32_t cnt) {
  return cnt >= HGS_SEGLEN ? 0u : (cnt >= (2u * HGS_SEGLEN + 2u) / 3u ? 1u : (cnt >= (HGS_SEGLEN + 2u) / 3u ? 2u : 3u));
}

__host__ __device__ __forceinline__ uint32_t hgs_cell_class(uint32_t len) {
  const uint32_t nb = (len + HGS_RB - 1) / HGS_RB;
  return nb >= 33u ? 0u : nb >= 25u ? 1u : nb >= 17u ? 2u : nb >= 13u ? 3u : nb >= 9u ? 4u : nb >= 7u ? 5u : nb >= 5u ? 6u : 11u - nb;
}

struct Layout {
  GeomRec* geom;
  uint32_t* tile_n;
  uint32_t* tile_start;
  uint32_t* tile_order;
  uint4* tile_rec;
  uint32_t* hist;
  uint32_t* tile_gbase;
  uint32_t* tile_count;
  uint32_t* chunk_sums;
  uint32_t* chunk_base;
  CellInfo* cell_info;
  uint32_t* fwd_cells;
  uint4* items_part;
  Counters* ctr;
  unsigned long long* keys;
  SortRec* recs;
  uint2* cell_list;
  uint2* entpair;
  float* cstate;
  uint32_t full_cap;
  uint4* items_full;
  uint32_t* n_contrib;
};

__host__ __device__ __forceinline__ size_t hgs_die_cells(int TT) { return (size_t)16 * (size_t)((TT + HGS_NXCD - 1) / HGS_NXCD); }

struct Cam {
  const float* viewmatrix;
  const float* projmatrix;
  const float* campos;
  const float* bg;
  float tanfovx, tanfovy, focal_x, focal_y;
};

struct View {
  Cam cam[HGS_MAX_VIEWS];
  float scale_modifier;
  int32_t W, H, grid_x, grid_y, T;
  int32_t B, TT;
  int32_t P, M, D, nblk;
  int32_t cpw, nwg, lds_bins;
  uint32_t entry_capacity;
  int32_t max_tile_hint;
  int32_t act;
  int32_t pairchunks;
};

static inline size_t hgs_align_up(size_t v, size_t a) { return (v + a - 1) / a * a; }

__device__ __forceinline__ int hgs_cell_of(int w, int j) { return (((w >> 1) << 1) + (j >> 1)) * 4 + ((w & 1) << 1) + (j & 1); }
#define HGS_FWD_THREADS 256

__device__ __forceinline__ bool hgs_eval_alpha(float dx, float dy, float qa, float qb,
// ... 95 lines not shown
```

### humangaussian_amd/csrc/render_bwd.hip

```cpp
#include "hgs_common.h"

#define HGS_STAGE_STRIDE 68

typedef float hgs_f32x4 __attribute__((ext_vector_type(4)));
typedef float hgs_f32x2 __attribute__((ext_vector_type(2)));

namespace {

__device__ __forceinline__ bool fetch_item(const uint4* __restrict__ full, const uint4* __restrict__ part, size_t dcap,
                                           uint32_t q, uint32_t n0, uint32_t n1, uint32_t n2, uint32_t n3, uint4& item) {
  const bool ok = q < n0 + n1 + n2 + n3;
  const uint4* src = full + q;
  if (q >= n0) {
    const uint32_t q1 = q - n0;
    src = part + q1;
    if (q1 >= n1) {
      const uint32_t q2 = q1 - n1;
      src = (q2 < n2) ? part + (dcap - 1 - q2) : part + (dcap + (q2 - n2));
    }
  }
  if (!ok) src = part;
  item = *src;
  return ok;
}

}

extern "C" __global__ void __launch_bounds__(64 * HGS_BWD_BLOCK_WAVES)
hgs_k_render_bwd(View v, Layout L, const hgs_status* __restrict__ status,
                 const SortRec* __restrict__ recs_all, const float* __restrict__ cstate,
                 const float* __restrict__ out_color,
                 const float* __restrict__ out_depth, const float* __restrict__ out_alpha,
                 const float* __restrict__ dL_dcolor, const float* __restrict__ dL_ddepth,
                 const float* __restrict__ dL_dalpha, float* __restrict__ pair_rows, uint32_t pair_cap) {
  __shared__ float4 s_rec_all[HGS_BWD_BLOCK_WAVES][4 * HGS_ROW_F4];
  __shared__ __attribute__((aligned(16))) float stage_k_all[HGS_BWD_BLOCK_WAVES][HGS_RB * HGS_STAGE_STRIDE];
  __shared__ __attribute__((aligned(16))) float stage_w_all[HGS_BWD_BLOCK_WAVES][HGS_RB * HGS_STAGE_STRIDE];
  __shared__ uint32_t s_ticket;
  __shared__ __attribute__((aligned(16))) float s_tabA[4][36];
  if (status->overflow) return;
  if ((uint32_t)L.ctr->alloc_ps > pair_cap) return;
  const int lane = (int)threadIdx.x & 63;
  const int wv = __builtin_amdgcn_readfirstlane((int)threadIdx.x >> 6);
  float4* __restrict__ s_rec = s_rec_all[wv];
  float* __restrict__ stage_k = stage_k_all[wv];
  float* __restrict__ stage_w = stage_w_all[wv];
  if (threadIdx.x == 0) s_ticket = HGS_BWD_BLOCK_WAVES;
  if (threadIdx.x < 128) {
    const int qs = (int)threadIdx.x >> 5, e = (int)threadIdx.x & 31, t = e & 15;
    const float u = (float)(t & 3) - 1.5f, w_ = (float)(t >> 2) - 1.5f;
    s_tabA[qs][e] = e < 16 ? (qs == 0 ? 1.0f : (qs == 1 ? u : (qs == 2 ? w_ : u * u)))
                           : (qs == 0 ? u * w_ : (qs == 1 ? w_ * w_ : 0.0f));
  }
  __syncthreads();
  const int j = lane >> 4, i = lane & 15;
  const uint32_t die = blockIdx.x % HGS_NXCD, lb = blockIdx.x / HGS_NXCD, nlb = gridDim.x / HGS_NXCD;
  const size_t dcap = hgs_die_cells(v.TT);
  const uint4* __restrict__ it_full = L.items_full + (size_t)die * L.full_cap;
  const uint4* __restrict__ it_part = L.items_part + (size_t)die * 2 * dcap;
  const uint32_t n0 = (uint32_t)L.ctr->sched[die][0], n1 = (uint32_t)(L.ctr->sched[die][0] >> 32);
  const uint32_t n2 = (uint32_t)L.ctr->sched[die][1], n3 = (uint32_t)(L.ctr->sched[die][1] >> 32);
  const uint32_t ngroups = (n0 + n1 + n2 + n3 + 3u) / 4u;
  const float4 zero4 = make_float4(0.f, 0.f, 0.f, 0.f);
  const float4* __restrict__ recs = reinterpret_cast<const float4*>(recs_all);
  float4* __restrict__ srow = s_rec + j * HGS_ROW_F4;

  const int qsel = lane & 3;
  const float* __restrict__ tabA = s_tabA[qsel];

#ifdef HGS_TIMELINE
  unsigned long long tl_w0 = 0, tl_w1 = 0;
  uint32_t tl_nb = 0, tl_live = 0;
#endif
  auto group_of = [&](uint32_t tk) {
    return tk * nlb + ((tk & 1u) ? nlb - 1u - lb : lb);
  };
  uint32_t grp = group_of((uint32_t)wv);
  uint4 item;
  bool have = fetch_item(it_full, it_part, dcap, 4u * grp + (uint32_t)j, n0, n1, n2, n3, item);
  while (grp < ngroups) {
    uint32_t grp_next;
    {
      uint32_t t_next = 0;
      if (lane == 0) t_next = atomicAdd(&s_ticket, 1u);
      grp_next = group_of((uint32_t)__builtin_amdgcn_readfirstlane((int)t_next));
    }
#ifdef HGS_TIMELINE
    tl_w0 = wall_clock64(); tl_nb = 0; tl_live = 0;
#endif
    const uint32_t key = item.x, cnt = have ? item.y : 0u;
    const int g = (int)(key >> 4), c = (int)(key & 15u);
    const int bview = g / v.T, t_ = g % v.T;
    const int cx0 = (t_ % v.grid_x) * HGS_TILE + (c & 3) * HGS_CELL, cy0 = (t_ / v.grid_x) * HGS_TILE + (c >> 2) * HGS_CELL;
    const int px = cx0 + (i & 3), py = cy0 + (i >> 2);
    const float pxf = (float)px, pyf = (float)py;
    const float cxq = (float)cx0 + 1.5f, cyq = (float)cy0 + 1.5f;
    const uint32_t tstart1 = L.tile_start[have ? g : 0] - 1u;
    const uint2* __restrict__ list = L.cell_list + (have ? item.z : 0u);

    const uint32_t safe_rec = tstart1 + 1u;
    auto list_at = [&](uint32_t e) { return list[(e < cnt) ? e : 0u]; };
    auto gather = [&](const uint2 le, bool valid, float4& r0, float4& r1, float4& r2) {
      const uint32_t idx = valid ? le.x : safe_rec;
      r0 = recs[3 * (size_t)idx]; r1 = recs[3 * (size_t)idx + 1];
      const float4 t2 = recs[3 * (size_t)idx + 2];
      r2 = make_float4(t2.x, t2.y, t2.z, __uint_as_float(valid ? idx - tstart1 : 0xffffffffu));
    };
    float4 c0, c1, c2;
    uint2 le_next = list_at((uint32_t)i);
    const uint2 le_second = list_at(HGS_RB + (uint32_t)i);
    const bool inside = have && px < v.W && py < v.H;
    const bool has_state = inside && item.w != 0xffffffffu;
    float g0, g1, g2, gd, ga, fp, T, F;
    uint32_t nc;
    {
      const size_t HW = (size_t)v.H * v.W, pix = inside ? (size_t)py * v.W + px : 0;
      const size_t o1 = inside ? (size_t)bview * HW : 0, o3 = 3 * o1;
      const float* pc = dL_dcolor ? dL_dcolor : out_color;
      const float* pd = dL_ddepth ? dL_ddepth : out_depth;
      const float* pa = dL_dalpha ? dL_dalpha : out_alpha;
      const float r_g0 = pc[o3 + pix], r_g1 = pc[o3 + HW + pix], r_g2 = pc[o3 + 2 * HW + pix];
      const float r_gd = pd[o1 + pix], r_ga = pa[o1 + pix];
      const float r_c0 = out_color[o3 + pix], r_c1 = out_color[o3 + HW + pix], r_c2 = out_color[o3 + 2 * HW + pix];
      const float r_d = out_depth[o1 + pix], r_a = out_alpha[o1 + pix];
      const uint32_t r_nc = L.n_contrib[o1 + pix];
      const float* cs = cstate + (size_t)(has_state ? item.w : 0u) * HGS_CSTATE_FLOATS + i;
      const float r_s0 = cs[0 * 16], r_s1 = cs[1 * 16], r_s2 = cs[2 * 16], r_s3 = cs[3 * 16], r_s4 = cs[4 * 16], r_s5 = cs[5 * 16];
      gather(le_next, (uint32_t)i < cnt, c0, c1, c2);
      g0 = (inside && dL_dcolor) ? r_g0 : 0.0f; g1 = (inside && dL_dcolor) ? r_g1 : 0.0f; g2 = (inside && dL_dcolor) ? r_g2 : 0.0f;
      gd = (inside && dL_ddepth) ? r_gd : 0.0f;
      ga = (inside && dL_dalpha) ? r_ga : 0.0f;
      fp = inside ? r_c0 * g0 + r_c1 * g1 + r_c2 * g2 + r_d * gd + r_a * ga : 0.0f;
      nc = inside ? r_nc : 0u;
      T = has_state ? r_s0 : 1.0f;
      F = has_state ? r_s1 * g0 + r_s2 * g1 + r_s3 * g2 + r_s4 * gd + r_s5 * ga : 0.0f;
      F = fp - F;
    }
    __builtin_amdgcn_wave_barrier();
    stage_k[0 * 64 + lane] = g0; stage_k[1 * 64 + lane] = g1; stage_k[2 * 64 + lane] = g2; stage_k[3 * 64 + lane] = gd;
    __builtin_amdgcn_fence(__ATOMIC_ACQ_REL, "wavefront");
    __builtin_amdgcn_wave_barrier();
    float A3[16];
    {
      const float* ar = stage_k + qsel * 64 + 16 * (lane >> 4);
#pragma unroll
      for (int q4 = 0; q4 < 4; ++q4) {
        const float4 a = *reinterpret_cast<const float4*>(ar + 4 * q4);
        A3[4 * q4 + 0] = a.x; A3[4 * q4 + 1] = a.y; A3[4 * q4 + 2] = a.z; A3[4 * q4 + 3] = a.w;
      }
    }
    __builtin_amdgcn_fence(__ATOMIC_ACQ_REL, "wavefront");
    __builtin_amdgcn_wave_barrier();

    uint32_t maxcnt = (uint32_t)__builtin_amdgcn_readlane((int)cnt, 0);
    maxcnt = max(maxcnt, (uint32_t)__builtin_amdgcn_readlane((int)cnt, 16));
    maxcnt = max(maxcnt, (uint32_t)__builtin_amdgcn_readlane((int)cnt, 32));
    maxcnt = max(maxcnt, (uint32_t)__builtin_amdgcn_readlane((int)cnt, 48));

    uint32_t pid_cur = le_next.y;
    le_next = le_second;
    uint4 item_next;
    const bool have_next = fetch_item(it_full, it_part, dcap, 4u * grp_next + (uint32_t)j, n0, n1, n2, n3, item_next);
    {
      const uint32_t first = (uint32_t)__shfl((int)__float_as_uint(c2.w), lane & 48, 64);
      if (!(have && nc >= first)) { T = 1.0f; F = 0.0f; nc = 0; }
    }

    float pmx = 0.f, pmy = 0.f, pqa = 0.f, pqb = 0.f, pqc = 0.f, pop = 0.f;
    uint32_t ppid = 0;
    auto finish = [&](const hgs_f32x4& a1, const hgs_f32x4& a2, const hgs_f32x4& a3, uint32_t it0) {
      if (it0 + (uint32_t)i >= cnt) return;
      const float a = pmx - cxq, bb = pmy - cyq;
      const float k00 = a1[0], k10 = a1[1], k01 = a1[2], k20 = a1[3], k11 = a2[0], k02 = a2[1];
      const float sdx = __builtin_fmaf(a, k00, -k10), sdy = __builtin_fmaf(bb, k00, -k01);
      const float sxx = __builtin_fmaf(a, __builtin_fmaf(a, k00, -(k10 + k10)), k20);
      const float sxy = __builtin_fmaf(a, sdy, __builtin_fmaf(-bb, k10, k11));
      const float syy = __builtin_fmaf(bb, __builtin_fmaf(bb, k00, -(k01 + k01)), k02);
      const float x0 = __builtin_fmaf(pqa + pqa, sdx, pqb * sdy);
      const float x1 = __builtin_fmaf(pqb, sdx, (pqc + pqc) * sdy);
      const float il = 1.0f / HGS_LOG2E;
      const float opi = (pop != 0.0f) ? 1.0f / pop : 0.0f;
      float2* row = reinterpret_cast<float2*>(pair_rows + (size_t)ppid * HGS_PROW_FLOATS);
      row[0] = make_float2(x0 * il, x1 * il);
      row[1] = make_float2(sxx * -0.5f, sxy * -1.0f);
      row[2] = make_float2(syy * -0.5f, k00 * opi);
      row[3] = make_float2(a3[0], a3[1]);
      row[4] = make_float2(a3[2], a3[3]);
    };
    for (uint32_t it0 = 0; it0 < maxcnt; it0 += HGS_RB) {
      const uint32_t bfirst = (uint32_t)__shfl((int)__float_as_uint(c2.w), lane & 48, 64);
      const unsigned long long act = __ballot((it0 < cnt) && (bfirst <= nc));
#ifdef HGS_TIMELINE
      if (tl_nb == 0) tl_w1 = wall_clock64() + (act & 1ull) * 0ull;
      ++tl_nb;
      tl_live += ((act & 0xffffull) != 0) + (((act >> 16) & 0xffffull) != 0) + (((act >> 32) & 0xffffull) != 0) + ((act >> 48) != 0);
#endif
      const float mxr = c0.x, myr = c0.y, qar = c0.z, qbr = c0.w, qcr = c1.x, opr = c1.y;
      if (act != 0ull) {
        __builtin_amdgcn_wave_barrier();
        float* pb = reinterpret_cast<float*>(srow + 6 * (i >> 1)) + (i & 1);
        pb[0] = c0.x; pb[2] = c0.y; pb[4] = c0.z; pb[6] = c0.w;
        pb[8] = c1.x; pb[10] = c1.y; pb[12] = c1.z; pb[14] = c1.w;
        pb[16] = c2.x; pb[18] = c2.y; pb[20] = c2.w;
      }
      const uint2 le_use = le_next;
      const uint32_t in2 = it0 + 2 * HGS_RB + (uint32_t)i;
      le_next = list_at(in2);
      const uint32_t pid_this = pid_cur;
      pid_cur = le_use.y;
      gather(le_use, it0 + HGS_RB + (uint32_t)i < cnt, c0, c1, c2);
      if (act == 0ull) {
        if (it0 + (uint32_t)i < cnt) {
          float2* row = reinterpret_cast<float2*>(pair_rows + (size_t)pid_this * HGS_PROW_FLOATS);
          const float2 zero2 = make_float2(0.f, 0.f);
          row[0] = zero2; row[1] = zero2; row[2] = zero2; row[3] = zero2; row[4] = zero2;
        }
        continue;
      }
      __builtin_amdgcn_fence(__ATOMIC_ACQ_REL, "wavefront");
      __builtin_amdgcn_wave_barrier();
      auto eval_pair = [&](int u, const float4& P0, const float4& P1, const float4& P2, const float4& P3, const float4& P4,
                           const float4& P5) {
        const hgs_f32x2 mx2 = {P0.x, P0.y}, my2 = {P0.z, P0.w}, qa2 = {P1.x, P1.y}, qb2 = {P1.z, P1.w};
        const hgs_f32x2 qc2 = {P2.x, P2.y}, op2 = {P2.z, P2.w}, cr2 = {P3.x, P3.y}, cg2 = {P3.z, P3.w};
        const hgs_f32x2 cb2 = {P4.x, P4.y}, cd2 = {P4.z, P4.w};
        const hgs_f32x2 dx2 = mx2 - pxf, dy2 = my2 - pyf;
        const hgs_f32x2 m2 = __builtin_elementwise_fma(qa2, dx2, qb2 * dy2);
        const hgs_f32x2 m3 = qc2 * dy2;
        const hgs_f32x2 p2 = __builtin_elementwise_fma(dx2, m2, m3 * dy2);
        const hgs_f32x2 G2 = {__builtin_amdgcn_exp2f(p2.x), __builtin_amdgcn_exp2f(p2.y)};
        const hgs_f32x2 og2 = op2 * G2;
        const bool on0 = (p2.x <= 0.0f) & (og2.x >= HGS_ALPHA_MIN) & (__float_as_uint(P5.x) <= nc);
        const bool on1 = (p2.y <= 0.0f) & (og2.y >= HGS_ALPHA_MIN) & (__float_as_uint(P5.y) <= nc);
        const hgs_f32x2 am2 = {on0 ? og2.x : 0.0f, on1 ? og2.y : 0.0f};
        const hgs_f32x2 a2 = {fminf(HGS_ALPHA_MAX, am2.x), fminf(HGS_ALPHA_MAX, am2.y)};
        const hgs_f32x2 om2 = 1.0f - a2;
        const hgs_f32x2 rc2 = {__builtin_amdgcn_rcpf(om2.x), __builtin_amdgcn_rcpf(om2.y)};
        const hgs_f32x2 S2 = __builtin_elementwise_fma(cr2, (hgs_f32x2)(g0), __builtin_elementwise_fma(cg2, (hgs_f32x2)(g1),
                             __builtin_elementwise_fma(cb2, (hgs_f32x2)(g2), __builtin_elementwise_fma(cd2, (hgs_f32x2)(gd), (hgs_f32x2)(ga)))));
        const float T1 = T * om2.x;
        const hgs_f32x2 T2 = {T, T1};
        const hgs_f32x2 wgt2 = a2 * T2;
        const float F0 = __builtin_fmaf(-wgt2.x, S2.x, F);
        const float F1 = __builtin_fmaf(-wgt2.y, S2.y, F0);
        const hgs_f32x2 Fn2 = {F0, F1};
        const hgs_f32x2 dl2 = __builtin_elementwise_fma(T2, S2, -(Fn2 * rc2));
        const hgs_f32x2 k2 = am2 * dl2;
        T = T1 * om2.y;
        F = F1;
        stage_k[u * HGS_STAGE_STRIDE + lane] = k2.x;
        stage_k[(u + 1) * HGS_STAGE_STRIDE + lane] = k2.y;
        stage_w[u * HGS_STAGE_STRIDE + lane] = wgt2.x;
        stage_w[(u + 1) * HGS_STAGE_STRIDE + lane] = wgt2.y;
      };
      float4 P[6], N[6];
#pragma unroll
      for (int m = 0; m < 6; ++m) P[m] = srow[m];
#pragma unroll
      for (int u = 0; u < HGS_RB; u += 2) {
        if (u + 2 < HGS_RB) {
#pragma unroll
          for (int m = 0; m < 6; ++m) N[m] = srow[3 * (u + 2) + m];
        }
        __builtin_amdgcn_sched_barrier(0x7f);
        eval_pair(u, P[0], P[1], P[2], P[3], P[4], P[5]);
        if (u + 2 < HGS_RB) {
#pragma unroll
          for (int m = 0; m < 6; ++m) P[m] = N[m];
        }
      }
      __builtin_amdgcn_fence(__ATOMIC_ACQ_REL, "wavefront");
      __builtin_amdgcn_wave_barrier();
      hgs_f32x4 acc1 = {0.f, 0.f, 0.f, 0.f}, acc2 = {0.f, 0.f, 0.f, 0.f}, acc3 = {0.f, 0.f, 0.f, 0.f};
      {
        const float* sk = stage_k + i * HGS_STAGE_STRIDE + 16 * j;
        const float* sw = stage_w + i * HGS_STAGE_STRIDE + 16 * j;
#pragma unroll
        for (int q4 = 0; q4 < 4; ++q4) {
          const float4 bk = *reinterpret_cast<const float4*>(sk + 4 * q4);
          const float4 bw = *reinterpret_cast<const float4*>(sw + 4 * q4);
          const float4 t1 = *reinterpret_cast<const float4*>(tabA + 4 * q4);
          const float4 t2 = *reinterpret_cast<const float4*>(tabA + 16 + 4 * q4);
          const float kx[4] = {bk.x, bk.y, bk.z, bk.w};
          const float wx[4] = {bw.x, bw.y, bw.z, bw.w};
          const float a1x[4] = {t1.x, t1.y, t1.z, t1.w};
          const float a2x[4] = {t2.x, t2.y, t2.z, t2.w};
#pragma unroll
          for (int r = 0; r < 4; ++r) {
            acc1 = __builtin_amdgcn_mfma_f32_4x4x1f32(a1x[r], kx[r], acc1, 0, 0, 0);
            acc2 = __builtin_amdgcn_mfma_f32_4x4x1f32(a2x[r], kx[r], acc2, 0, 0, 0);
            acc3 = __builtin_amdgcn_mfma_f32_4x4x1f32(A3[4 * q4 + r], wx[r], acc3, 0, 0, 0);
          }
        }
      }
      __builtin_amdgcn_fence(__ATOMIC_ACQ_REL, "wavefront");
      __builtin_amdgcn_wave_barrier();
      pmx = mxr; pmy = myr; pqa = qar; pqb = qbr; pqc = qcr; pop = opr; ppid = pid_this;
      finish(acc1, acc2, acc3, it0);
    }
#ifdef HGS_TIMELINE
    if (lane == 0) {
      unsigned long long* o = L.keys + ((size_t)grp * HGS_NXCD + die) * 4;
      const unsigned long long simd_key = ((unsigned long long)(__builtin_amdgcn_s_getreg((31 << 11) | 20) & 0xfu) << 16) |
                                          (__builtin_amdgcn_s_getreg((31 << 11) | 4) & 0xff30u);
      o[0] = tl_w0; o[1] = wall_clock64(); o[2] = tl_nb | ((tl_w1 - tl_w0) << 32); o[3] = (unsigned long long)(cnt) | (simd_key << 8) | ((unsigned long long)tl_live << 32) | 1ull << 63;
    }
#endif
    grp = grp_next; item = item_next; have = have_next;
  }
}

#define HGS_RED_ROWS 128
#define HGS_RED_RUNS 4
extern "C" __global__ void __launch_bounds__(256)
hgs_k_pair_reduce_em(View v, Layout L, const hgs_status* __restrict__ status, const SortRec* __restrict__ recs_all,
                  const float* __restrict__ pair_rows, float* __restrict__ grad_rows, uint32_t pair_cap, uint32_t R_host) {
  __shared__ float2 s_rows[4][HGS_RED_ROWS * HGS_PROW_F2];
  uint32_t R = R_host;
  if (R_host == 0xffffffffu) {
    if (status->overflow) return;
    R = status->num_rendered;
  }
  const int lane = (int)threadIdx.x & 63, w = (int)threadIdx.x >> 6;
  const uint32_t p = blockIdx.x * 256u + threadIdx.x;
  if (p - (uint32_t)lane >= R) return;
  const bool have = p < R;
  uint2 ep = make_uint2(0u, 0u);
  if (have) ep = L.entpair[p];
  const uint32_t entry = ep.x & 0x7ffffffu;
  const bool poisoned = (uint32_t)L.ctr->alloc_ps > pair_cap;
  const uint32_t cnt = poisoned ? 0u : ep.x >> 27;
  const uint32_t incl = hgs_wave_incl_scan(cnt), off = incl - cnt;
  float2 s0 = make_float2(0.f, 0.f), s1 = s0, s2 = s0, s3 = s0, s4 = s0;
  unsigned long long todo = __ballot(cnt != 0u);
  float2* __restrict__ sl = s_rows[w];
  for (int run = 0; run < HGS_RED_RUNS && todo != 0ull; ++run) {
    const int first = __builtin_ctzll(todo);
    const uint32_t base = (uint32_t)__builtin_amdgcn_readlane((int)(ep.y - off), first);
    const bool mine = cnt != 0u && ep.y - off == base;
    const unsigned long long in_run = __ballot(mine);
    todo &= ~in_run;
    const int lastl = 63 - __builtin_clzll(in_run);
    const uint32_t r_lo = (uint32_t)__builtin_amdgcn_readlane((int)off, first);
    const uint32_t r_hi = (uint32_t)__builtin_amdgcn_readlane((int)incl, lastl);
    const uint32_t total = r_hi - r_lo;
    const uint32_t moff = off - r_lo, mcnt = mine ? cnt : 0u;
    const float2* __restrict__ src = reinterpret_cast<const float2*>(pair_rows) + (size_t)(base + r_lo) * HGS_PROW_F2;
    static_assert(HGS_RED_ROWS * HGS_PROW_F2 == 10 * 64, "ten float2 per lane and tile");
    float2 b0, b1, b2, b3, b4, b5, b6, b7, b8, b9;
#define HGS_RED_ISSUE(T0)                                                                                      \
  {                                                                                                            \
    const uint32_t t0n__ = (T0);                                                                               \
    const bool any__ = t0n__ < total;                                                                          \
    const uint32_t last__ = any__ ? min((uint32_t)HGS_RED_ROWS, total - t0n__) * HGS_PROW_F2 - 1u : 0u;        \
    const float2* p__ = src + (any__ ? (size_t)t0n__ * HGS_PROW_F2 : 0);                                       \
    b0 = p__[min((uint32_t)lane, last__)];        b1 = p__[min((uint32_t)lane + 64u, last__)];                 \
    b2 = p__[min((uint32_t)lane + 128u, last__)]; b3 = p__[min((uint32_t)lane + 192u, last__)];                \
    b4 = p__[min((uint32_t)lane + 256u, last__)]; b5 = p__[min((uint32_t)lane + 320u, last__)];                \
    b6 = p__[min((uint32_t)lane + 384u, last__)]; b7 = p__[min((uint32_t)lane + 448u, last__)];                \
    b8 = p__[min((uint32_t)lane + 512u, last__)]; b9 = p__[min((uint32_t)lane + 576u, last__)];                \
  }
    HGS_RED_ISSUE(0u);
    for (uint32_t t0 = 0; t0 < total; t0 += HGS_RED_ROWS) {
      const uint32_t nrow = min((uint32_t)HGS_RED_ROWS, total - t0);
      const uint32_t nfl = nrow * HGS_PROW_F2;
      __builtin_amdgcn_wave_barrier();
      if ((uint32_t)lane < nfl) sl[lane] = b0;
      if ((uint32_t)lane + 64u < nfl) sl[lane + 64] = b1;
      if ((uint32_t)lane + 128u < nfl) sl[lane + 128] = b2;
      if ((uint32_t)lane + 192u < nfl) sl[lane + 192] = b3;
      if ((uint32_t)lane + 256u < nfl) sl[lane + 256] = b4;
      if ((uint32_t)lane + 320u < nfl) sl[lane + 320] = b5;
      if ((uint32_t)lane + 384u < nfl) sl[lane + 384] = b6;
      if ((uint32_t)lane + 448u < nfl) sl[lane + 448] = b7;
      if ((uint32_t)lane + 512u < nfl) sl[lane + 512] = b8;
      if ((uint32_t)lane + 576u < nfl) sl[lane + 576] = b9;
      HGS_RED_ISSUE(t0 + HGS_RED_ROWS);
      __builtin_amdgcn_fence(__ATOMIC_RELEASE, "wavefront");
      __builtin_amdgcn_wave_barrier();
      if (mcnt) {
        const uint32_t r_begin = max(moff, t0), r_end = min(moff + mcnt, t0 + nrow);
        for (uint32_t r = r_begin; r < r_end; ++r) {
          const float2* q = sl + HGS_PROW_F2 * (r - t0);
          const float2 a0 = q[0], a1 = q[1], a2 = q[2], a3 = q[3], a4 = q[4];
          s0.x += a0.x; s0.y += a0.y; s1.x += a1.x; s1.y += a1.y; s2.x += a2.x; s2.y += a2.y;
          s3.x += a3.x; s3.y += a3.y; s4.x += a4.x; s4.y += a4.y;
        }
      }
    }
#undef HGS_RED_ISSUE
  }
  if (todo != 0ull) {
    const bool left = ((todo >> lane) & 1ull) != 0ull;
// ... 137 lines not shown
```

### humangaussian_amd/csrc/render_fwd.hip

```cpp
#include "hgs_common.h"

namespace {

typedef float hgs_fwd_f32x2 __attribute__((ext_vector_type(2)));

struct PixState {
  hgs_fwd_f32x2 C01, C2D;
  float Wt;
  float T;
  uint32_t last;
};

__device__ __forceinline__ void blend_one(PixState& s, float pxf, float pyf, const float4 r0,
                                          const float4 r1, const float4 r2) {
  float G, alpha, m2, m3;
  const bool keep = hgs_eval_alpha(r0.x - pxf, r0.y - pyf, r0.z, r0.w, r1.x, r1.y, G, alpha, m2, m3);
  const float ak = keep ? alpha : 0.0f;
  const float test_T = s.T * (1.0f - ak);
  const bool ok = test_T >= HGS_T_EPS;
  const float wgt = ok ? ak * s.T : 0.0f;
  s.T = ok ? test_T : -__builtin_fabsf(s.T);
  const bool upd = keep && ok;
  const hgs_fwd_f32x2 rg = {r1.z, r1.w}, bd = {r2.x, r2.y}, w2 = {wgt, wgt};
  s.C01 = __builtin_elementwise_fma(rg, w2, s.C01);
  s.C2D = __builtin_elementwise_fma(bd, w2, s.C2D);
  s.Wt += wgt;
  s.last = upd ? __float_as_uint(r2.w) : s.last;
}

}

#define HGS_FWD_C4 4
typedef unsigned hgs_u32x2 __attribute__((ext_vector_type(2)));

__device__ __forceinline__ float hgs_xor16(float x, int lane) {
  const hgs_u32x2 s2 = __builtin_amdgcn_permlane16_swap(__float_as_uint(x), __float_as_uint(x), false, false);
  return __uint_as_float((lane & 16) ? s2.x : s2.y);
}
__device__ __forceinline__ float hgs_xor32(float x, int lane) {
  const hgs_u32x2 s2 = __builtin_amdgcn_permlane32_swap(__float_as_uint(x), __float_as_uint(x), false, false);
  return __uint_as_float((lane & 32) ? s2.x : s2.y);
}
__device__ __forceinline__ float hgs_rows_sum(float x, int lane) {
  (void)lane;
  const hgs_u32x2 s16 = __builtin_amdgcn_permlane16_swap(__float_as_uint(x), __float_as_uint(x), false, false);
  const float s01 = __uint_as_float(s16.x) + __uint_as_float(s16.y);
  const hgs_u32x2 s32 = __builtin_amdgcn_permlane32_swap(__float_as_uint(s01), __float_as_uint(s01), false, false);
  return __uint_as_float(s32.x) + __uint_as_float(s32.y);
}

template <bool STORE>
__device__ __forceinline__ void render_fwd_cell4(const View& v, const Layout& L, uint32_t key,
                                                 const SortRec* __restrict__ recs_all,
                                                 float* __restrict__ cstate,
                                                 float* __restrict__ out_color,
                                                 float* __restrict__ out_depth,
                                                 float* __restrict__ out_alpha, float4* __restrict__ s_rec_w) {
  const int lane = (int)threadIdx.x & 63;
  const int r = lane >> 4, i = lane & 15;
  const int g = (int)(key >> 4), c = (int)(key & 15u);
  const int bview = g / v.T, t = g % v.T;
  const size_t HW = (size_t)v.H * v.W;
  const int px = (t % v.grid_x) * HGS_TILE + (c & 3) * HGS_CELL + (i & 3);
  const int py = (t / v.grid_x) * HGS_TILE + (c >> 2) * HGS_CELL + (i >> 2);
  const bool inside = (px < v.W) && (py < v.H);
  const float pxf = (float)px, pyf = (float)py;
  const uint32_t tstart1 = L.tile_start[g] - 1u;
  const CellInfo ci = L.cell_info[key];
  const uint32_t len = ci.len, sbase = ci.sbase;
  const uint2* __restrict__ list = L.cell_list + ci.base;
  const float4* __restrict__ recs = reinterpret_cast<const float4*>(recs_all);
  const float4 zero4 = make_float4(0.f, 0.f, 0.f, 0.f);

  float T = inside ? 1.0f : 0.0f;
  float tmin = 1.0f;
  float C0 = 0.f, C1 = 0.f, C2 = 0.f, D = 0.f, Wt = 0.f;
  uint32_t last = 0;

  auto load_idx = [&](uint32_t e) { return list[(e < len) ? e : 0u].x; };
  auto gather = [&](uint32_t idx_raw, bool valid, float4& r0, float4& r1, float4& r2) {
    const uint32_t idx = valid ? idx_raw : tstart1 + 1u;
    r0 = recs[3 * (size_t)idx]; r1 = recs[3 * (size_t)idx + 1];
    const float4 t2 = recs[3 * (size_t)idx + 2];
    r2 = make_float4(t2.x, t2.y, t2.z, __uint_as_float(valid ? idx - tstart1 : 0xffffffffu));
  };
  float4 c0, c1, c2;
  gather(load_idx((uint32_t)lane), (uint32_t)lane < len, c0, c1, c2);
  uint32_t idx_a = load_idx(64u + (uint32_t)lane), idx_b = load_idx(128u + (uint32_t)lane);

  for (uint32_t it0 = 0; it0 < len; it0 += 64u) {
    if (__ballot(T != 0.0f) == 0ull) break;
    if (STORE && it0 > 0 && (it0 % HGS_SEGLEN) == 0) {
      const float s0 = hgs_rows_sum(C0, lane), s1 = hgs_rows_sum(C1, lane), s2 = hgs_rows_sum(C2, lane);
      const float sd = hgs_rows_sum(D, lane), sw = hgs_rows_sum(Wt, lane);
      if (r == 0) {
        float* cs = cstate + (size_t)(sbase + it0 / HGS_SEGLEN - 1) * HGS_CSTATE_FLOATS + i;
        cs[0 * 16] = T; cs[1 * 16] = s0; cs[2 * 16] = s1; cs[3 * 16] = s2; cs[4 * 16] = sd; cs[5 * 16] = sw;
      }
    }
    __builtin_amdgcn_wave_barrier();
    c1.y = (__float_as_uint(c2.w) == 0xffffffffu) ? 0.0f : c1.y;
    s_rec_w[3 * lane + 0] = c0; s_rec_w[3 * lane + 1] = c1; s_rec_w[3 * lane + 2] = c2;
    const uint32_t idx_n = load_idx(it0 + 192u + (uint32_t)lane);
    gather(idx_a, it0 + 64u + (uint32_t)lane < len, c0, c1, c2);
    idx_a = idx_b; idx_b = idx_n;
    __builtin_amdgcn_fence(__ATOMIC_RELEASE, "wavefront");
    __builtin_amdgcn_wave_barrier();
    const float4* __restrict__ myrec = s_rec_w + 3 * r;
    float4 ra = myrec[0], rb = myrec[1], rc = myrec[2];
#pragma unroll 2
    for (int k = 0; k < 16; ++k) {
      float4 na = zero4, nb = zero4, nc = zero4;
      if (k + 1 < 16) { na = myrec[12 * (k + 1) + 0]; nb = myrec[12 * (k + 1) + 1]; nc = myrec[12 * (k + 1) + 2]; }
      __builtin_amdgcn_sched_barrier(0x7f);
      float G, alpha, m2, m3;
      const bool keep = hgs_eval_alpha(ra.x - pxf, ra.y - pyf, ra.z, ra.w, rb.x, rb.y, G, alpha, m2, m3);
      const float ak = keep ? alpha : 0.0f;
      const float a = 1.0f - ak;
      const hgs_u32x2 s16 = __builtin_amdgcn_permlane16_swap(__float_as_uint(a), __float_as_uint(a), false, false);
      const float a_even = __uint_as_float(s16.x), a_odd = __uint_as_float(s16.y);
      const float p01 = a_even * a_odd;
      const hgs_u32x2 s32 = __builtin_amdgcn_permlane32_swap(__float_as_uint(p01), __float_as_uint(p01), false, false);
      const float p_lo = __uint_as_float(s32.x), p_hi = __uint_as_float(s32.y);
      const float excl = ((lane & 16) ? a_even : 1.0f) * ((lane & 32) ? p_lo : 1.0f);
      const float Tb = T * excl;
      const float test_T = Tb * a;
      const bool ok = test_T >= HGS_T_EPS;
      const float wgt = ok ? ak * Tb : 0.0f;
      const bool upd = keep && ok;
      C0 = __builtin_fmaf(rb.z, wgt, C0);
      C1 = __builtin_fmaf(rb.w, wgt, C1);
      C2 = __builtin_fmaf(rc.x, wgt, C2);
      D = __builtin_fmaf(rc.y, wgt, D);
      Wt += wgt;
      tmin = upd ? test_T : tmin;
      last = upd ? __float_as_uint(rc.w) : last;
      const unsigned long long okm = __ballot(ok);
      const uint32_t ok2 = (uint32_t)okm & (uint32_t)(okm >> 32);
      const uint32_t ok4 = (ok2 & (ok2 >> 16) & 0xffffu) * 0x10001u;
      const bool go = __builtin_amdgcn_inverse_ballot_w64(((unsigned long long)ok4 << 32) | ok4);
      T = go ? T * (p_lo * p_hi) : 0.0f;
      ra = na; rb = nb; rc = nc;
    }
  }
  const float s0 = hgs_rows_sum(C0, lane), s1 = hgs_rows_sum(C1, lane), s2 = hgs_rows_sum(C2, lane);
  const float sd = hgs_rows_sum(D, lane), sw = hgs_rows_sum(Wt, lane);
  float tm = fminf(tmin, hgs_xor16(tmin, lane));
  tm = fminf(tm, hgs_xor32(tm, lane));
  uint32_t lm = max(last, __float_as_uint(hgs_xor16(__uint_as_float(last), lane)));
  lm = max(lm, __float_as_uint(hgs_xor32(__uint_as_float(lm), lane)));
  if (inside && r == 0) {
    const float* __restrict__ bg = v.cam[bview].bg;
    const size_t pix = (size_t)py * v.W + px, o1 = (size_t)bview * HW, o3 = 3 * o1;
    out_color[o3 + 0 * HW + pix] = s0 + tm * bg[0];
    out_color[o3 + 1 * HW + pix] = s1 + tm * bg[1];
    out_color[o3 + 2 * HW + pix] = s2 + tm * bg[2];
    out_depth[o1 + pix] = sd;
    out_alpha[o1 + pix] = sw;
    L.n_contrib[o1 + pix] = lm;
  }
}

#define HGS_FWD_PRE_STRIDE 12
__device__ __forceinline__ uint32_t fwd_cell_key(const Layout& L, size_t dcap, const uint32_t* pre, int c, uint32_t q) {
  const uint4 p0 = *reinterpret_cast<const uint4*>(pre + c * HGS_FWD_PRE_STRIDE);
  const uint4 p1 = *reinterpret_cast<const uint4*>(pre + c * HGS_FWD_PRE_STRIDE + 4);
  uint32_t x = 0, base = 0;
  if (q >= p0.y) { x = 1; base = p0.y; }
  if (q >= p0.z) { x = 2; base = p0.z; }
  if (q >= p0.w) { x = 3; base = p0.w; }
  if (q >= p1.x) { x = 4; base = p1.x; }
  if (q >= p1.y) { x = 5; base = p1.y; }
  if (q >= p1.z) { x = 6; base = p1.z; }
  if (q >= p1.w) { x = 7; base = p1.w; }
  return L.fwd_cells[((size_t)x * HGS_NFC + (size_t)c) * dcap + (q - base)];
}

template <bool STORE>
__device__ __forceinline__ void render_fwd_cells(const View& v, const Layout& L, const uint32_t* pre, uint32_t wave_id, int w,
                                                 const SortRec* __restrict__ recs_all,
                                                 float* __restrict__ cstate,
                                                 float* __restrict__ out_color,
                                                 float* __restrict__ out_depth,
                                                 float* __restrict__ out_alpha, float4* __restrict__ s_rec_w) {
  const int lane = (int)threadIdx.x & 63;
  const int j = lane >> 4, i = lane & 15;
  uint32_t q = 4u * wave_id + (uint32_t)j;
  uint32_t key = 0;
  bool have = false;
  int mycls = HGS_NFC;
  {
    uint32_t total = 0;
#pragma unroll
    for (int c = HGS_FWD_C4; c < HGS_NFC; ++c) {
      const uint32_t nc = pre[c * HGS_FWD_PRE_STRIDE + HGS_NXCD];
      if (!have && q < nc) { have = true; mycls = c; }
      q -= have ? 0u : nc;
      total += nc;
    }
    if (4u * wave_id >= total) return;
    const uint32_t k_ = fwd_cell_key(L, hgs_die_cells(v.TT), pre, have ? mycls : HGS_FWD_C4, have ? q : 0u);
    key = have ? k_ : 0u;
  }
  const int g = (int)(key >> 4), c = (int)(key & 15u);
  const int bview = g / v.T, t = g % v.T;
  const size_t HW = (size_t)v.H * v.W;
  const int px = (t % v.grid_x) * HGS_TILE + (c & 3) * HGS_CELL + (i & 3);
  const int py = (t / v.grid_x) * HGS_TILE + (c >> 2) * HGS_CELL + (i >> 2);
  const bool inside = have && (px < v.W) && (py < v.H);
  const float pxf = (float)px, pyf = (float)py;

  const uint32_t tstart1 = have ? L.tile_start[g] - 1u : 0u;
  uint32_t len = 0, base = 0, sbase = 0;
  if (have) {
    const CellInfo ci = L.cell_info[key];
    len = ci.len; base = ci.base; sbase = ci.sbase;
  }
  const uint2* __restrict__ list = L.cell_list + base;
  const float4* __restrict__ recs = reinterpret_cast<const float4*>(recs_all);
  float4* __restrict__ srow = s_rec_w + j * HGS_ROW_F4;

  PixState s;
  s.T = inside ? 1.0f : 0.0f;
  s.C01 = s.C2D = (hgs_fwd_f32x2){0.f, 0.f};
  s.Wt = 0.f;
  s.last = 0;

  const float4 zero4 = make_float4(0.f, 0.f, 0.f, 0.f);
  const uint32_t safe_rec = have ? tstart1 + 1u : 0u;
  auto load_idx = [&](uint32_t e) { return list[(e < len) ? e : 0u].x; };
  auto gather = [&](uint32_t idx_raw, bool valid, float4& r0, float4& r1, float4& r2) {
    const uint32_t idx = valid ? idx_raw : safe_rec;
    r0 = recs[3 * (size_t)idx]; r1 = recs[3 * (size_t)idx + 1];
    const float4 t2 = recs[3 * (size_t)idx + 2];
    r2 = make_float4(t2.x, t2.y, t2.z, __uint_as_float(valid ? idx - tstart1 : 0xffffffffu));
  };
  float4 c0, c1, c2, d0, d1, d2;
  gather(load_idx((uint32_t)i), (uint32_t)i < len, c0, c1, c2);
  gather(load_idx(HGS_RB + (uint32_t)i), HGS_RB + (uint32_t)i < len, d0, d1, d2);
  uint32_t idx_a = load_idx(2 * HGS_RB + (uint32_t)i), idx_b = load_idx(3 * HGS_RB + (uint32_t)i);

  for (uint32_t it0 = 0;; it0 += HGS_RB) {
    const unsigned long long act = __ballot((it0 < len) && (s.T > 0.0f));
    if (act == 0ull) break;
    const bool row_on = ((act >> (lane & 48)) & 0xffffull) != 0ull;
    if (STORE && row_on && it0 > 0 && (it0 % HGS_SEGLEN) == 0) {
      float* cs = cstate + (size_t)(sbase + it0 / HGS_SEGLEN - 1) * HGS_CSTATE_FLOATS + i;
      cs[0 * 16] = s.T; cs[1 * 16] = s.C01.x; cs[2 * 16] = s.C01.y; cs[3 * 16] = s.C2D.x; cs[4 * 16] = s.C2D.y; cs[5 * 16] = s.Wt;
    }
    __builtin_amdgcn_wave_barrier();
    c1.y = (__float_as_uint(c2.w) == 0xffffffffu) ? 0.0f : c1.y;
    {
      float* pb = reinterpret_cast<float*>(srow + 6 * (i >> 1)) + (i & 1);
      float* pc = pb + (i & 1);
      pb[0] = c0.x; pb[2] = c0.y; pb[4] = c0.z; pb[6] = c0.w;
      pb[8] = c1.x; pb[10] = c1.y; pc[12] = c1.z; pc[13] = c1.w;
      pc[16] = c2.x; pc[17] = c2.y; pb[20] = c2.w;
    }
    c0 = d0; c1 = d1; c2 = d2;
    const uint32_t idx_n = load_idx(it0 + 4 * HGS_RB + (uint32_t)i);
    gather(idx_a, row_on && (it0 + 2 * HGS_RB + (uint32_t)i < len), d0, d1, d2);
    idx_a = idx_b; idx_b = idx_n;
    __builtin_amdgcn_fence(__ATOMIC_RELEASE, "wavefront");
    __builtin_amdgcn_wave_barrier();
    float4 P[6], N[6];
#pragma unroll
    for (int m = 0; m < 6; ++m) P[m] = srow[m];
#pragma unroll
    for (int u0 = 0; u0 < HGS_RB; u0 += 2) {
      if (u0 + 2 < HGS_RB) {
#pragma unroll
        for (int m = 0; m < 6; ++m) N[m] = srow[3 * (u0 + 2) + m];
      }
      __builtin_amdgcn_sched_barrier(0x7f);
      blend_one(s, pxf, pyf, make_float4(P[0].x, P[0].z, P[1].x, P[1].z), make_float4(P[2].x, P[2].z, P[3].x, P[3].y),
                make_float4(P[4].x, P[4].y, 0.0f, P[5].x));
      blend_one(s, pxf, pyf, make_float4(P[0].y, P[0].w, P[1].y, P[1].w), make_float4(P[2].y, P[2].w, P[3].z, P[3].w),
                make_float4(P[4].z, P[4].w, 0.0f, P[5].y));
      __builtin_amdgcn_sched_barrier(0x7f);
      if (u0 + 2 < HGS_RB) {
#pragma unroll
        for (int m = 0; m < 6; ++m) P[m] = N[m];
      }
    }
  }

  if (inside) {
    const float* __restrict__ bg = v.cam[bview].bg;
    const size_t pix = (size_t)py * v.W + px, o1 = (size_t)bview * HW, o3 = 3 * o1;
    const float Tout = __builtin_fabsf(s.T);
    out_color[o3 + 0 * HW + pix] = s.C01.x + Tout * bg[0];
    out_color[o3 + 1 * HW + pix] = s.C01.y + Tout * bg[1];
    out_color[o3 + 2 * HW + pix] = s.C2D.x + Tout * bg[2];
    out_depth[o1 + pix] = s.C2D.y;
    out_alpha[o1 + pix] = s.Wt;
    L.n_contrib[o1 + pix] = s.last;
  }
}

__device__ __forceinline__ void render_fwd_background(const View& v, const Layout& L, bool overflow, int g,
                                                      float* __restrict__ out_color, float* __restrict__ out_depth,
                                                      float* __restrict__ out_alpha) {
  const int bview = g / v.T, t = g % v.T;
  const int lx = (int)threadIdx.x & 15, ly = (int)threadIdx.x >> 4;
  const int px = (t % v.grid_x) * HGS_TILE + lx, py = (t / v.grid_x) * HGS_TILE + ly;
  if (px >= v.W || py >= v.H) return;
  bool empty = overflow || L.tile_n[g] == 0u;
  if (!empty) empty = L.cell_info[(size_t)g * 16 + (ly >> 2) * 4 + (lx >> 2)].len == 0u;
  if (!empty) return;
  const float* __restrict__ bg = v.cam[bview].bg;
  const size_t HW = (size_t)v.H * v.W, pix = (size_t)py * v.W + px, o1 = (size_t)bview * HW, o3 = 3 * o1;
  out_color[o3 + 0 * HW + pix] = bg[0];
  out_color[o3 + 1 * HW + pix] = bg[1];
  out_color[o3 + 2 * HW + pix] = bg[2];
  out_depth[o1 + pix] = 0.0f;
  out_alpha[o1 + pix] = 0.0f;
  L.n_contrib[o1 + pix] = 0u;
}

#define HGS_RENDER_FWD_KERNEL(NAME, STORE)                                                                 \
  extern "C" __global__ void __launch_bounds__(HGS_FWD_THREADS) NAME(                                       \
      View v, Layout L, uint32_t cell_blocks, hgs_status* __restrict__ status,                               \
      hgs_status* __restrict__ status_host, const SortRec* __restrict__ recs, float* __restrict__ cstate, float* __restrict__ out_color,           \
      float* __restrict__ out_depth, float* __restrict__ out_alpha) {                                        \
    __shared__ float4 s_rec[HGS_FWD_THREADS / 64][4 * HGS_ROW_F4];        \
    __shared__ __attribute__((aligned(16))) uint32_t s_pre[HGS_NFC * HGS_FWD_PRE_STRIDE];                    \
    const bool overflow = status->overflow != 0;                                                             \
    if (blockIdx.x >= cell_blocks) {                                                                         \
      const uint32_t g = blockIdx.x - cell_blocks;                                                           \
      if (g < (uint32_t)v.TT) render_fwd_background(v, L, overflow, (int)g, out_color, out_depth, out_alpha); \
      return;                                                                                                \
    }                                                                                                        \
    if (overflow) return;                                                                                    \
    if (blockIdx.x == 0 && threadIdx.x == 0) {        \
      const uint32_t np = (uint32_t)L.ctr->alloc_ps;                                                         \
      status->num_pairs = np;                                                                                \
      if (status_host) *reinterpret_cast<volatile uint32_t*>(&status_host->num_pairs) = np;                  \
    }                                                                                                        \
    HGS_TL_BEGIN();                                                                                          \
    const int w = __builtin_amdgcn_readfirstlane((int)threadIdx.x >> 6);                                     \
     \
    const size_t dcap = hgs_die_cells(v.TT);                                                                 \
    if (threadIdx.x < HGS_NFC) {                                                                             \
      uint32_t acc = 0;                                                                                      \
      for (int x = 0; x < HGS_NXCD; ++x) {                                                                   \
        s_pre[threadIdx.x * HGS_FWD_PRE_STRIDE + x] = acc;                                                   \
        acc += (uint32_t)L.ctr->sched[x][2 + threadIdx.x];                                                   \
      }                                                                                                      \
      s_pre[threadIdx.x * HGS_FWD_PRE_STRIDE + HGS_NXCD] = acc;                                              \
    }                                                                                                        \
    __syncthreads();                                                                                         \
    uint32_t cnt4[HGS_FWD_C4 + 1], n4 = 0, nrest = 0;             \
    _Pragma("unroll") for (int c = 0; c < HGS_NFC; ++c) {                                                    \
      const uint32_t nc = (uint32_t)__builtin_amdgcn_readfirstlane((int)s_pre[c * HGS_FWD_PRE_STRIDE + HGS_NXCD]); \
      if (c < HGS_FWD_C4) { cnt4[c] = nc; n4 += nc; } else nrest += nc;                                      \
    }                                                                                                        \
    const uint32_t nitems = n4 + (nrest + 3u) / 4u;                                                          \
    const uint32_t ncu = max(1u, cell_blocks / 4u), S = ncu * 4u;                                            \
    const uint32_t slot = (blockIdx.x % ncu) * 4u + (uint32_t)w;                                             \
    HGS_TLI_DECL();                                                                                          \
    for (uint32_t rho = blockIdx.x / ncu; rho * S < nitems; rho += (cell_blocks + ncu - 1u) / ncu) {         \
      const uint32_t it = rho * S + ((rho & 1u) ? S - 1u - slot : slot);                                     \
      if (it >= nitems) continue;                                                                            \
      HGS_TLI_BEGIN();                                                                                       \
      if (it < n4) {                                                                                         \
        uint32_t q = it;                                                                                     \
        int c4 = 0;                                                                                          \
        _Pragma("unroll") for (int c = 0; c < HGS_FWD_C4 - 1; ++c) if (c4 == c && q >= cnt4[c]) { q -= cnt4[c]; c4 = c + 1; } \
        render_fwd_cell4<STORE>(v, L, fwd_cell_key(L, dcap, s_pre, c4, q), recs, cstate, out_color,         \
                                out_depth, out_alpha, s_rec[w]);                                             \
      } else {                                                                                               \
        render_fwd_cells<STORE>(v, L, s_pre, it - n4, w, recs, cstate, out_color, out_depth, out_alpha, s_rec[w]); \
      }                                                                                                      \
      HGS_TLI_END(it, (it < n4 ? 0 : -1));                                                                   \
    }                                                                                                        \
    HGS_TL_END(4, HGS_TLI_TAG());                                                                            \
  }
HGS_RENDER_FWD_KERNEL(hgs_k_render_fwd_store, true)
HGS_RENDER_FWD_KERNEL(hgs_k_render_fwd_nostore, false)
```

Before: 660.5 million.

## Pack per-cell pair list entries into 32-bit words for non-chunked path

Adds a narrow cell-list element format: each cell list entry becomes a single packed 32-bit word (record index, mask, cell) instead of a uint2, and the record tail drops its tag word. Sort/gather kernels write the narrow form and store each record's first pair row separately. Forward and backward render kernels read the narrow index, and chunked-mode variants keep the wide format. The aim is to cut memory traffic and footprint for cell lists, at the cost of extra kernel variants and a dependency on compile-time macros selecting the format.

```diff
diff --git a/humangaussian_amd/csrc/api.hip b/humangaussian_amd/csrc/api.hip
--- a/humangaussian_amd/csrc/api.hip
+++ b/humangaussian_amd/csrc/api.hip
@@ -19,6 +19,14 @@
 extern "C" __global__ void hgs_k_render_bwd(View, Layout, const hgs_status*, const SortRec*, const float*,
                                             const float*, const float*, const float*, const float*,
                                             const float*, const float*, float*, uint32_t);
+#ifdef HGS_NARROW_CELL_ELEMENTS
+extern "C" __global__ void hgs_k_render_bwd_ch(View, Layout, const hgs_status*, const SortRec*, const float*,
+                                               const float*, const float*, const float*, const float*,
+                                               const float*, const float*, float*, uint32_t);
+#define HGS_BY_ELEMENT(K) (v.pairchunks ? K##_ch : K)
+#else
+#define HGS_BY_ELEMENT(K) K
+#endif
 extern "C" __global__ void hgs_k_pair_reduce_em(View, Layout, const hgs_status*, const SortRec*, const float*, float*, uint32_t, uint32_t);
 extern "C" __global__ void hgs_k_pair_reduce_ch(View, Layout, const hgs_status*, const SortRec*, const float*, float*, uint32_t, uint32_t);
 
@@ -540,11 +548,11 @@
         s2 = side->s;
       }
       if (need_huge) {
-        hipLaunchKernelGGL(hgs_k_sort_huge, dim3(class_grid(16384)), dim3(1024), 0, s2, v, L, status_dev);
+        hipLaunchKernelGGL(HGS_BY_ELEMENT(hgs_k_sort_huge), dim3(class_grid(16384)), dim3(1024), 0, s2, v, L, status_dev);
         HGS_LAUNCH_CHECK();
       }
       if (need_large) {
-        hipLaunchKernelGGL(hgs_k_sort_large, dim3(class_grid(HGS_SORT_LDS_MAX)), dim3(1024), 0, s2, v, L, status_dev);
+        hipLaunchKernelGGL(HGS_BY_ELEMENT(hgs_k_sort_large), dim3(class_grid(HGS_SORT_LDS_MAX)), dim3(1024), 0, s2, v, L, status_dev);
         HGS_LAUNCH_CHECK();
       }
       if (side) {
@@ -569,7 +577,7 @@
     const int64_t fwd_blocks = (int64_t)hgs_knob("HGS_FWD_BLOCKS_PER_CU", 4) * ncu;
     const unsigned cell_blocks = (unsigned)std::max<int64_t>(4, std::min<int64_t>(fwd_blocks, (cells + 3) / 4) & ~int64_t(3));
     const unsigned bg_blocks = (unsigned)v.TT;
-    hipLaunchKernelGGL(store_bwd_state ? hgs_k_render_fwd_store : hgs_k_render_fwd_nostore, dim3(cell_blocks + bg_blocks),
+    hipLaunchKernelGGL(store_bwd_state ? HGS_BY_ELEMENT(hgs_k_render_fwd_store) : HGS_BY_ELEMENT(hgs_k_render_fwd_nostore), dim3(cell_blocks + bg_blocks),
                        dim3(HGS_FWD_THREADS), 0, stream, v, L, cell_blocks, status_dev, status_mapped, L.recs, L.cstate,
                        out_color, out_depth, out_alpha);
   }
@@ -651,7 +659,7 @@
   HGS_STAGE(0);
   if (maybe_entries) {
     const int resident = hgs_knob("HGS_BWD_WAVES_PER_CU", 12) * cu_count(ds);
-    hipLaunchKernelGGL(hgs_k_render_bwd, dim3((unsigned)std::max(HGS_NXCD, resident / HGS_BWD_BLOCK_WAVES / HGS_NXCD * HGS_NXCD)), dim3(64 * HGS_BWD_BLOCK_WAVES), 0, stream, v, L, status_dev, L.recs, L.cstate,
+    hipLaunchKernelGGL(HGS_BY_ELEMENT(hgs_k_render_bwd), dim3((unsigned)std::max(HGS_NXCD, resident / HGS_BWD_BLOCK_WAVES / HGS_NXCD * HGS_NXCD)), dim3(64 * HGS_BWD_BLOCK_WAVES), 0, stream, v, L, status_dev, L.recs, L.cstate,
                        out_color, out_depth, out_alpha, dL_dout_color, dL_dout_depth, dL_dout_alpha, pair_rows, pair_cap);
     HGS_LAUNCH_CHECK();
     HGS_STAGE(1);
diff --git a/humangaussian_amd/csrc/binning.hip b/humangaussian_amd/csrc/binning.hip
--- a/humangaussian_amd/csrc/binning.hip
+++ b/humangaussian_amd/csrc/binning.hip
@@ -205,8 +205,21 @@
 
 namespace {
 
-__device__ __forceinline__ void hgs_put_pair(const Layout& L, uint32_t rec, uint32_t row_id, uint32_t slot) {
-  L.cell_list[slot] = make_uint2(rec, row_id);
+template <bool WIDE>
+__device__ __forceinline__ void hgs_put_pair(const Layout& L, uint32_t rec, uint32_t row_id, uint32_t mask, uint32_t cell, uint32_t slot) {
+  if (WIDE) L.cell_list[slot] = make_uint2(rec, row_id);
+  else reinterpret_cast<uint32_t*>(L.cell_list)[slot] = hgs_le_pack(rec, mask, cell);
+}
+template <bool WIDE>
+__device__ __forceinline__ void hgs_put_rec_tail(uint4* dst2, uint32_t b, uint32_t depth, uint32_t entry, uint32_t tag) {
+  if (WIDE) *dst2 = make_uint4(b, depth, entry, tag);
+  else {
+    typedef uint32_t hgs_u32x3 __attribute__((ext_vector_type(3), aligned(16)));
+    *reinterpret_cast<hgs_u32x3*>(dst2) = (hgs_u32x3){b, depth, entry};
+  }
+}
+__device__ __forceinline__ void hgs_put_first_row(const Layout& L, uint32_t rec, uint32_t first_row) {
+  L.recs[rec].pad = first_row;
 }
 
 struct CellAlloc {
@@ -302,7 +315,7 @@
   uint32_t pair_base;
 };
 
-template <int MAXCH>
+template <int MAXCH, bool WIDE>
 __device__ __forceinline__ void gather_records(const View& v, const Layout& L, int g, uint32_t order_pos,
                                                uint32_t start, uint32_t n,
                                                unsigned long long* sorted, int nt, GatherLds<MAXCH>& S) {
@@ -352,7 +365,7 @@
         const float qa = -0.5f * ca * HGS_LOG2E, qb = -cb * HGS_LOG2E, qc = -0.5f * cc * HGS_LOG2E;
         dst[0] = make_uint4(g0.x, g0.y, __float_as_uint(qa), __float_as_uint(qb));
         dst[1] = make_uint4(__float_as_uint(qc), g1.y, g1.z, g1.w);
-        dst[2] = make_uint4(g2.x, g2.y, entry, v.pairchunks ? hgs_rec_tag(mask, k, n, false) : 0u);
+        hgs_put_rec_tail<WIDE>(dst + 2, g2.x, g2.y, entry, v.pairchunks ? hgs_rec_tag(mask, k, n, false) : 0u);
         L.entpair[start + k].x = entry | ((uint32_t)__popc(mask) << 27);
         sorted[k] = (unsigned long long)mask;
       }
@@ -407,6 +420,7 @@
       const uint32_t cnt = (uint32_t)__popc(mask);
       const uint32_t rel = S.tab[ch][16] + hgs_wave_incl_scan(cnt) - cnt;
       if (in) L.entpair[start + k].y = pair_base + rel;
+      if (!WIDE && in) hgs_put_first_row(L, start + k, pair_base + rel);
 #pragma unroll
       for (int c = 0; c < 16; ++c) {
         const bool bit = (mask >> c) & 1u;
@@ -414,7 +428,7 @@
         if (bit) {
           const uint32_t rank = S.tab[ch][c] + __builtin_amdgcn_mbcnt_hi((uint32_t)(bal >> 32), __builtin_amdgcn_mbcnt_lo((uint32_t)bal, 0u));
           const uint32_t slot = S.cell_base[c] + rank;
-          hgs_put_pair(L, start + k, pair_base + rel + (uint32_t)__popc(mask & ((1u << c) - 1u)), slot);
+          hgs_put_pair<WIDE>(L, start + k, pair_base + rel + (uint32_t)__popc(mask & ((1u << c) - 1u)), mask, (uint32_t)c, slot);
         }
       }
     }
@@ -427,7 +441,7 @@
 }
 __device__ __forceinline__ uint32_t hgs_bytesum(uint32_t w) { return __builtin_amdgcn_sad_u8(w, 0u, 0u); }
 
-template <int MAXCH>
+template <int MAXCH, bool WIDE>
 __device__ __forceinline__ void gather_records_single(const View& v, const Layout& L, int g, uint32_t order_pos,
                                                       uint32_t start, uint32_t n,
                                                       unsigned long long* sorted, int nt, GatherLds<MAXCH>& S) {
@@ -481,7 +495,7 @@
         const float qa = -0.5f * ca * HGS_LOG2E, qb = -cb * HGS_LOG2E, qc = -0.5f * cc * HGS_LOG2E;
         dst[0] = make_uint4(g0.x, g0.y, __float_as_uint(qa), __float_as_uint(qb));
         dst[1] = make_uint4(__float_as_uint(qc), g1.y, g1.z, g1.w);
-        dst[2] = make_uint4(g2.x, g2.y, entry, v.pairchunks ? hgs_rec_tag(mask, k, n, false) : 0u);
+        hgs_put_rec_tail<WIDE>(dst + 2, g2.x, g2.y, entry, v.pairchunks ? hgs_rec_tag(mask, k, n, false) : 0u);
         L.entpair[start + k].x = entry | ((uint32_t)__popc(mask) << 27);
         sorted[k] = (unsigned long long)mask;
       }
@@ -549,13 +563,15 @@
     }
     const uint32_t rel = S.tab[ch][16] + before;
     if (in) L.entpair[start + k].y = pair_base + rel;
+    if (!WIDE && in) hgs_put_first_row(L, start + k, pair_base + rel);
+    const uint32_t mask_all = WIDE ? 0u : mask;
     uint32_t r = 0;
     while (mask) {
       const int c = __builtin_ctz(mask);
       mask &= mask - 1u;
       const uint32_t exw = (c < 8) ? (c < 4 ? ex[0] : ex[1]) : (c < 12 ? ex[2] : ex[3]);
       const uint32_t slot = S.cell_base[c] + S.tab[ch][c] + ((exw >> (8 * (c & 3))) & 0xffu);
-      hgs_put_pair(L, start + k, pair_base + rel + r, slot);
+      hgs_put_pair<WIDE>(L, start + k, pair_base + rel + r, mask_all, (uint32_t)c, slot);
       ++r;
     }
   }
@@ -681,7 +697,7 @@
   }
 }
 
-template <int NT, bool CH>
+template <int NT, bool CH, bool WIDE>
 __device__ __forceinline__ void cell_lists_from_masks(const View& v, const Layout& L, uint32_t order_pos, uint32_t start, uint32_t n,
                                                       const uint16_t* __restrict__ masks, GatherLds<64>& S, const CellAlloc& ca,
                                                       unsigned long long* tp) {
@@ -748,6 +764,7 @@
     const uint32_t rel_chunk = pair_base + S.tab[ch][16];
     const uint32_t rel = rel_chunk + before;
     if (in) L.entpair[start + k].y = CH ? rel_chunk : rel;
+    if (!WIDE && in) hgs_put_first_row(L, start + k, rel);
     const uint32_t cb = lane < 16 ? S.cell_base[lane] + S.tab[ch][lane] : 0u;
     uint32_t cp = 0;
 #pragma unroll
@@ -756,7 +773,7 @@
       if ((mask >> c) & 1u) {
         const uint32_t exc = (ex[c >> 2] >> (8 * (c & 3))) & 0xffu;
         const uint32_t slot = cbase + exc;
-        hgs_put_pair(L, start + k, CH ? rel_chunk + cp + exc : rel + (uint32_t)__popc(mask & ((1u << c) - 1u)), slot);
+        hgs_put_pair<WIDE>(L, start + k, CH ? rel_chunk + cp + exc : rel + (uint32_t)__popc(mask & ((1u << c) - 1u)), mask, (uint32_t)c, slot);
       }
       if (CH) cp += (tot[c >> 2] >> (8 * (c & 3))) & 0xffu;
     }
@@ -971,7 +988,7 @@
   return degenerate;
 }
 
-template <int NT, bool CH>
+template <int NT, bool CH, bool WIDE>
 __device__ __forceinline__ void rank_sort_tile(const View& v, const Layout& L, uint32_t order_pos, int g, uint32_t start, uint32_t n,
                                                unsigned long long* pairs, RankLds& R, GatherLds<64>& S, bool& degenerate_out,
                                                unsigned long long* tp) {
@@ -1043,7 +1060,7 @@
       const float qa = -0.5f * ca * HGS_LOG2E, qb = -cb * HGS_LOG2E, qc = -0.5f * cc * HGS_LOG2E; \
       dst[0] = make_uint4(g0.x, g0.y, __float_as_uint(qa), __float_as_uint(qb));              \
       dst[1] = make_uint4(__float_as_uint(qc), g1.y, g1.z, g1.w);                             \
-      dst[2] = make_uint4(g2.x, g2.y, entry, CH ? hgs_rec_tag(mask, k, n, true) : 0u);        \
+      hgs_put_rec_tail<WIDE>(dst + 2, g2.x, g2.y, entry, CH ? hgs_rec_tag(mask, k, n, true) : 0u); \
       L.entpair[start + k].x = entry | ((uint32_t)__popc(mask) << 27);    \
       masks[k] = (uint16_t)mask;                                                              \
       _Pragma("unroll") for (int wd = 0; wd < 4; ++wd) acc[wd] += hgs_spread4((mask >> (4 * wd)) & 0xfu); \
@@ -1092,10 +1109,10 @@
     const uint32_t word = R.tot16[2 * (c >> 2) + (c & 1)];
     hgs_alloc_cell_ranges_issue(L, order_pos, (word >> (16 * ((c >> 1) & 1))) & 0xffffu, ca);
   }
-  cell_lists_from_masks<NT, CH>(v, L, order_pos, start, n, masks, S, ca, tp);
-}
-
-template <int NT, bool CH>
+  cell_lists_from_masks<NT, CH, WIDE>(v, L, order_pos, start, n, masks, S, ca, tp);
+}
+
+template <int NT, bool CH, bool WIDE>
 __device__ __forceinline__ void sort_rank_body(const View& v, const Layout& L, const hgs_status* __restrict__ status,
                                                unsigned long long* pairs, RankLds& R, GatherLds<64>& S) {
   if (status->overflow) return;
@@ -1120,7 +1137,7 @@
 #endif
     bool degenerate;
     unsigned long long tp[4] = {0, 0, 0, 0};
-    rank_sort_tile<NT, CH>(v, L, b, g, start, n, pairs, R, S, degenerate, tp);
+    rank_sort_tile<NT, CH, WIDE>(v, L, b, g, start, n, pairs, R, S, degenerate, tp);
 #ifdef HGS_TIMELINE
     if (threadIdx.x == 0 && b < HGS_TL_SLOTS) {
       const unsigned long long tpe = wall_clock64();
@@ -1141,43 +1158,49 @@
 }
 
 static_assert(16 * HGS_SORT_NT >= 4096, "the rank sort takes every list of the LDS class");
-#define HGS_SORT_LDS_KERNEL(NAME, CH)                                                                                  \
+#define HGS_SORT_LDS_KERNEL(NAME, CH, WIDE)                                                                                  \
   extern "C" __global__ void __launch_bounds__(HGS_SORT_NT) __attribute__((amdgpu_waves_per_eu(HGS_SORT_WAVES_PER_EU, HGS_SORT_WAVES_PER_EU))) \
   NAME(View v, Layout L, const hgs_status* __restrict__ status) {                                                      \
     __shared__ unsigned long long pairs[4096];                                                                         \
     __shared__ GatherLds<64> S;                                                                                        \
     __shared__ RankLds R;                                                                                              \
     HGS_TL_BEGIN();                                                                                                    \
-    sort_rank_body<HGS_SORT_NT, CH>(v, L, status, pairs, R, S);                                                        \
+    sort_rank_body<HGS_SORT_NT, CH, WIDE>(v, L, status, pairs, R, S);                                                        \
     HGS_TL_END(3, 0u);                                                                                                 \
   }
-HGS_SORT_LDS_KERNEL(hgs_k_sort_lds, false)
-HGS_SORT_LDS_KERNEL(hgs_k_sort_lds_ch, true)
-
-extern "C" __global__ void __launch_bounds__(1024)
-hgs_k_sort_large(View v, Layout L, const hgs_status* __restrict__ status) {
-  __shared__ unsigned long long keys[16384];
-  __shared__ GatherLds<256> S;
-  if (status->overflow) return;
-  const uint32_t b = blockIdx.x;
-  if (b >= status->active_tiles) return;
-  const int t = (int)L.tile_order[b];
-  const uint32_t start = L.tile_start[t];
-  const uint32_t n = L.tile_n[t];
-  if (n <= (uint32_t)HGS_SORT_LDS_MAX || n > 16384u) return;
-  {
-    __shared__ RankLds R;
-    const uint32_t NB = (uint32_t)HGS_RANK_NB_MAX;
-    for (uint32_t i = threadIdx.x; i <= NB; i += 1024) R.hist[i] = 0u;
-    if (threadIdx.x == 0) { R.dmin = 0xffffffffu; R.dmax = 0u; R.maxcnt = 0u; }
-    rank_keys_stream<1024, true>(L, start, n, NB, keys, R);
-    __syncthreads();
-  }
-  gather_records_single<256>(v, L, t, b, start, n, keys, 1024, S);
-}
-
-extern "C" __global__ void __launch_bounds__(1024)
-hgs_k_sort_huge(View v, Layout L, const hgs_status* __restrict__ status) {
+HGS_SORT_LDS_KERNEL(hgs_k_sort_lds, false, HGS_EM_WIDE)
+HGS_SORT_LDS_KERNEL(hgs_k_sort_lds_ch, true, true)
+
+#define HGS_SORT_LARGE_KERNEL(NAME, WIDE)                                                                              \
+  extern "C" __global__ void __launch_bounds__(1024)                                                                   \
+  NAME(View v, Layout L, const hgs_status* __restrict__ status) {                                                      \
+    __shared__ unsigned long long keys[16384];                                                                         \
+    __shared__ GatherLds<256> S;                                                                                       \
+    if (status->overflow) return;                                                                                      \
+    const uint32_t b = blockIdx.x;                                                                                     \
+    if (b >= status->active_tiles) return;                                                                             \
+    const int t = (int)L.tile_order[b];                                                                                \
+    const uint32_t start = L.tile_start[t];                                                                            \
+    const uint32_t n = L.tile_n[t];                                                                                    \
+    if (n <= (uint32_t)HGS_SORT_LDS_MAX || n > 16384u) return;                                                         \
+    {                                                                                                                  \
+      __shared__ RankLds R;                                                                                            \
+      const uint32_t NB = (uint32_t)HGS_RANK_NB_MAX;                                                                   \
+      for (uint32_t i = threadIdx.x; i <= NB; i += 1024) R.hist[i] = 0u;                                               \
+      if (threadIdx.x == 0) { R.dmin = 0xffffffffu; R.dmax = 0u; R.maxcnt = 0u; }                                      \
+      rank_keys_stream<1024, true>(L, start, n, NB, keys, R);                                                          \
+      __syncthreads();                                                                                                 \
+    }                                                                                                                  \
+    gather_records_single<256, WIDE>(v, L, t, b, start, n, keys, 1024, S);                                             \
+  }
+HGS_SORT_LARGE_KERNEL(hgs_k_sort_large, HGS_EM_WIDE)
+#ifdef HGS_NARROW_CELL_ELEMENTS
+HGS_SORT_LARGE_KERNEL(hgs_k_sort_large_ch, true)
+#endif
+
+namespace {
+template <bool WIDE>
+__device__ __forceinline__ void sort_huge_body(const View& v, const Layout& L, const hgs_status* __restrict__ status) {
   if (status->overflow) return;
   const uint32_t b = blockIdx.x;
   if (b >= status->active_tiles) return;
@@ -1187,5 +1210,12 @@
   if (n <= 16384u) return;
   __shared__ GatherLds<256> S;
   bitonic_sort<1024>(L.keys + start, n);
-  gather_records<256>(v, L, t, b, start, n, L.keys + start, 1024, S);
-}
+  gather_records<256, WIDE>(v, L, t, b, start, n, L.keys + start, 1024, S);
+}
+}
+extern "C" __global__ void __launch_bounds__(1024)
+hgs_k_sort_huge(View v, Layout L, const hgs_status* __restrict__ status) { sort_huge_body<HGS_EM_WIDE>(v, L, status); }
+#ifdef HGS_NARROW_CELL_ELEMENTS
+extern "C" __global__ void __launch_bounds__(1024)
+hgs_k_sort_huge_ch(View v, Layout L, const hgs_status* __restrict__ status) { sort_huge_body<true>(v, L, status); }
+#endif
diff --git a/humangaussian_amd/csrc/hgs_common.h b/humangaussian_amd/csrc/hgs_common.h
--- a/humangaussian_amd/csrc/hgs_common.h
+++ b/humangaussian_amd/csrc/hgs_common.h
@@ -55,6 +55,17 @@
   const uint32_t left = n - (k & ~63u);
   return (mask & 0xffffu) | ((k & 63u) << 16) | (((left < 64u ? left : 64u) - 1u) << 22) | (chunk_rows ? 1u << 28 : 0u);
 }
+
+#define HGS_LE_RANK_SHIFT 27
+#define HGS_LE_INDEX_MASK 0x7ffffffu
+__host__ __device__ __forceinline__ uint32_t hgs_le_pack(uint32_t rec, uint32_t mask, uint32_t cell) {
+  return rec | ((uint32_t)__builtin_popcount(mask & ((1u << cell) - 1u)) << HGS_LE_RANK_SHIFT);
+}
+#ifdef HGS_NARROW_CELL_ELEMENTS
+#define HGS_EM_WIDE false
+#else
+#define HGS_EM_WIDE true
+#endif
 
 struct __attribute__((aligned(16))) CellInfo {
   uint32_t base;
diff --git a/humangaussian_amd/csrc/render_bwd.hip b/humangaussian_amd/csrc/render_bwd.hip
--- a/humangaussian_amd/csrc/render_bwd.hip
+++ b/humangaussian_amd/csrc/render_bwd.hip
@@ -26,289 +26,18 @@
 
 }
 
-extern "C" __global__ void __launch_bounds__(64 * HGS_BWD_BLOCK_WAVES)
-hgs_k_render_bwd(View v, Layout L, const hgs_status* __restrict__ status,
-                 const SortRec* __restrict__ recs_all, const float* __restrict__ cstate,
-                 const float* __restrict__ out_color,
-                 const float* __restrict__ out_depth, const float* __restrict__ out_alpha,
-                 const float* __restrict__ dL_dcolor, const float* __restrict__ dL_ddepth,
-                 const float* __restrict__ dL_dalpha, float* __restrict__ pair_rows, uint32_t pair_cap) {
-  __shared__ float4 s_rec_all[HGS_BWD_BLOCK_WAVES][4 * HGS_ROW_F4];
-  __shared__ __attribute__((aligned(16))) float stage_k_all[HGS_BWD_BLOCK_WAVES][HGS_RB * HGS_STAGE_STRIDE];
-  __shared__ __attribute__((aligned(16))) float stage_w_all[HGS_BWD_BLOCK_WAVES][HGS_RB * HGS_STAGE_STRIDE];
-  __shared__ uint32_t s_ticket;
-  __shared__ __attribute__((aligned(16))) float s_tabA[4][36];
-  if (status->overflow) return;
-  if ((uint32_t)L.ctr->alloc_ps > pair_cap) return;
-  const int lane = (int)threadIdx.x & 63;
-  const int wv = __builtin_amdgcn_readfirstlane((int)threadIdx.x >> 6);
-  float4* __restrict__ s_rec = s_rec_all[wv];
-  float* __restrict__ stage_k = stage_k_all[wv];
-  float* __restrict__ stage_w = stage_w_all[wv];
-  if (threadIdx.x == 0) s_ticket = HGS_BWD_BLOCK_WAVES;
-  if (threadIdx.x < 128) {
-    const int qs = (int)threadIdx.x >> 5, e = (int)threadIdx.x & 31, t = e & 15;
-    const float u = (float)(t & 3) - 1.5f, w_ = (float)(t >> 2) - 1.5f;
-    s_tabA[qs][e] = e < 16 ? (qs == 0 ? 1.0f : (qs == 1 ? u : (qs == 2 ? w_ : u * u)))
-                           : (qs == 0 ? u * w_ : (qs == 1 ? w_ * w_ : 0.0f));
-  }
-  __syncthreads();
-  const int j = lane >> 4, i = lane & 15;
-  const uint32_t die = blockIdx.x % HGS_NXCD, lb = blockIdx.x / HGS_NXCD, nlb = gridDim.x / HGS_NXCD;
-  const size_t dcap = hgs_die_cells(v.TT);
-  const uint4* __restrict__ it_full = L.items_full + (size_t)die * L.full_cap;
-  const uint4* __restrict__ it_part = L.items_part + (size_t)die * 2 * dcap;
-  const uint32_t n0 = (uint32_t)L.ctr->sched[die][0], n1 = (uint32_t)(L.ctr->sched[die][0] >> 32);
-  const uint32_t n2 = (uint32_t)L.ctr->sched[die][1], n3 = (uint32_t)(L.ctr->sched[die][1] >> 32);
-  const uint32_t ngroups = (n0 + n1 + n2 + n3 + 3u) / 4u;
-  const float4 zero4 = make_float4(0.f, 0.f, 0.f, 0.f);
-  const float4* __restrict__ recs = reinterpret_cast<const float4*>(recs_all);
-  float4* __restrict__ srow = s_rec + j * HGS_ROW_F4;
-
-  const int qsel = lane & 3;
-  const float* __restrict__ tabA = s_tabA[qsel];
-
-#ifdef HGS_TIMELINE
-  unsigned long long tl_w0 = 0, tl_w1 = 0;
-  uint32_t tl_nb = 0, tl_live = 0;
+#define HGS_BWD_NAME hgs_k_render_bwd
+#define HGS_BWD_WIDE HGS_EM_WIDE
+#include "render_bwd_blend.h"
+#undef HGS_BWD_NAME
+#undef HGS_BWD_WIDE
+#ifdef HGS_NARROW_CELL_ELEMENTS
+#define HGS_BWD_NAME hgs_k_render_bwd_ch
+#define HGS_BWD_WIDE true
+#include "render_bwd_blend.h"
+#undef HGS_BWD_NAME
+#undef HGS_BWD_WIDE
 #endif
-  auto group_of = [&](uint32_t tk) {
-    return tk * nlb + ((tk & 1u) ? nlb - 1u - lb : lb);
-  };
-  uint32_t grp = group_of((uint32_t)wv);
-  uint4 item;
-  bool have = fetch_item(it_full, it_part, dcap, 4u * grp + (uint32_t)j, n0, n1, n2, n3, item);
-  while (grp < ngroups) {
-    uint32_t grp_next;
-    {
-      uint32_t t_next = 0;
-      if (lane == 0) t_next = atomicAdd(&s_ticket, 1u);
-      grp_next = group_of((uint32_t)__builtin_amdgcn_readfirstlane((int)t_next));
-    }
-#ifdef HGS_TIMELINE
-    tl_w0 = wall_clock64(); tl_nb = 0; tl_live = 0;
-#endif
-    const uint32_t key = item.x, cnt = have ? item.y : 0u;
-    const int g = (int)(key >> 4), c = (int)(key & 15u);
-    const int bview = g / v.T, t_ = g % v.T;
-    const int cx0 = (t_ % v.grid_x) * HGS_TILE + (c & 3) * HGS_CELL, cy0 = (t_ / v.grid_x) * HGS_TILE + (c >> 2) * HGS_CELL;
-    const int px = cx0 + (i & 3), py = cy0 + (i >> 2);
-    const float pxf = (float)px, pyf = (float)py;
-    const float cxq = (float)cx0 + 1.5f, cyq = (float)cy0 + 1.5f;
-    const uint32_t tstart1 = L.tile_start[have ? g : 0] - 1u;
-    const uint2* __restrict__ list = L.cell_list + (have ? item.z : 0u);
-
-    const uint32_t safe_rec = tstart1 + 1u;
-    auto list_at = [&](uint32_t e) { return list[(e < cnt) ? e : 0u]; };
-    auto gather = [&](const uint2 le, bool valid, float4& r0, float4& r1, float4& r2) {
-      const uint32_t idx = valid ? le.x : safe_rec;
-      r0 = recs[3 * (size_t)idx]; r1 = recs[3 * (size_t)idx + 1];
-      const float4 t2 = recs[3 * (size_t)idx + 2];
-      r2 = make_float4(t2.x, t2.y, t2.z, __uint_as_float(valid ? idx - tstart1 : 0xffffffffu));
-    };
-    float4 c0, c1, c2;
-    uint2 le_next = list_at((uint32_t)i);
-    const uint2 le_second = list_at(HGS_RB + (uint32_t)i);
-    const bool inside = have && px < v.W && py < v.H;
-    const bool has_state = inside && item.w != 0xffffffffu;
-    float g0, g1, g2, gd, ga, fp, T, F;
-    uint32_t nc;
-    {
-      const size_t HW = (size_t)v.H * v.W, pix = inside ? (size_t)py * v.W + px : 0;
-      const size_t o1 = inside ? (size_t)bview * HW : 0, o3 = 3 * o1;
-      const float* pc = dL_dcolor ? dL_dcolor : out_color;
-      const float* pd = dL_ddepth ? dL_ddepth : out_depth;
-      const float* pa = dL_dalpha ? dL_dalpha : out_alpha;
-      const float r_g0 = pc[o3 + pix], r_g1 = pc[o3 + HW + pix], r_g2 = pc[o3 + 2 * HW + pix];
-      const float r_gd = pd[o1 + pix], r_ga = pa[o1 + pix];
-      const float r_c0 = out_color[o3 + pix], r_c1 = out_color[o3 + HW + pix], r_c2 = out_color[o3 + 2 * HW + pix];
-      const float r_d = out_depth[o1 + pix], r_a = out_alpha[o1 + pix];
-      const uint32_t r_nc = L.n_contrib[o1 + pix];
-      const float* cs = cstate + (size_t)(has_state ? item.w : 0u) * HGS_CSTATE_FLOATS + i;
-      const float r_s0 = cs[0 * 16], r_s1 = cs[1 * 16], r_s2 = cs[2 * 16], r_s3 = cs[3 * 16], r_s4 = cs[4 * 16], r_s5 = cs[5 * 16];
-      gather(le_next, (uint32_t)i < cnt, c0, c1, c2);
-      g0 = (inside && dL_dcolor) ? r_g0 : 0.0f; g1 = (inside && dL_dcolor) ? r_g1 : 0.0f; g2 = (inside && dL_dcolor) ? r_g2 : 0.0f;
-      gd = (inside && dL_ddepth) ? r_gd : 0.0f;
-      ga = (inside && dL_dalpha) ? r_ga : 0.0f;
-      fp = inside ? r_c0 * g0 + r_c1 * g1 + r_c2 * g2 + r_d * gd + r_a * ga : 0.0f;
-      nc = inside ? r_nc : 0u;
-      T = has_state ? r_s0 : 1.0f;
-      F = has_state ? r_s1 * g0 + r_s2 * g1 + r_s3 * g2 + r_s4 * gd + r_s5 * ga : 0.0f;
-      F = fp - F;
-    }
-    __builtin_amdgcn_wave_barrier();
-    stage_k[0 * 64 + lane] = g0; stage_k[1 * 64 + lane] = g1; stage_k[2 * 64 + lane] = g2; stage_k[3 * 64 + lane] = gd;
-    __builtin_amdgcn_fence(__ATOMIC_ACQ_REL, "wavefront");
-    __builtin_amdgcn_wave_barrier();
-    float A3[16];
-    {
-      const float* ar = stage_k + qsel * 64 + 16 * (lane >> 4);
-#pragma unroll
-      for (int q4 = 0; q4 < 4; ++q4) {
-        const float4 a = *reinterpret_cast<const float4*>(ar + 4 * q4);
-        A3[4 * q4 + 0] = a.x; A3[4 * q4 + 1] = a.y; A3[4 * q4 + 2] = a.z; A3[4 * q4 + 3] = a.w;
-      }
-    }
-    __builtin_amdgcn_fence(__ATOMIC_ACQ_REL, "wavefront");
-    __builtin_amdgcn_wave_barrier();
-
-    uint32_t maxcnt = (uint32_t)__builtin_amdgcn_readlane((int)cnt, 0);
-    maxcnt = max(maxcnt, (uint32_t)__builtin_amdgcn_readlane((int)cnt, 16));
-    maxcnt = max(maxcnt, (uint32_t)__builtin_amdgcn_readlane((int)cnt, 32));
-    maxcnt = max(maxcnt, (uint32_t)__builtin_amdgcn_readlane((int)cnt, 48));
-
-    uint32_t pid_cur = le_next.y;
-    le_next = le_second;
-    uint4 item_next;
-    const bool have_next = fetch_item(it_full, it_part, dcap, 4u * grp_next + (uint32_t)j, n0, n1, n2, n3, item_next);
-    {
-      const uint32_t first = (uint32_t)__shfl((int)__float_as_uint(c2.w), lane & 48, 64);
-      if (!(have && nc >= first)) { T = 1.0f; F = 0.0f; nc = 0; }
-    }
-
-    float pmx = 0.f, pmy = 0.f, pqa = 0.f, pqb = 0.f, pqc = 0.f, pop = 0.f;
-    uint32_t ppid = 0;
-    auto finish = [&](const hgs_f32x4& a1, const hgs_f32x4& a2, const hgs_f32x4& a3, uint32_t it0) {
-      if (it0 + (uint32_t)i >= cnt) return;
-      const float a = pmx - cxq, bb = pmy - cyq;
-      const float k00 = a1[0], k10 = a1[1], k01 = a1[2], k20 = a1[3], k11 = a2[0], k02 = a2[1];
-      const float sdx = __builtin_fmaf(a, k00, -k10), sdy = __builtin_fmaf(bb, k00, -k01);
-      const float sxx = __builtin_fmaf(a, __builtin_fmaf(a, k00, -(k10 + k10)), k20);
-      const float sxy = __builtin_fmaf(a, sdy, __builtin_fmaf(-bb, k10, k11));
-      const float syy = __builtin_fmaf(bb, __builtin_fmaf(bb, k00, -(k01 + k01)), k02);
-      const float x0 = __builtin_fmaf(pqa + pqa, sdx, pqb * sdy);
-      const float x1 = __builtin_fmaf(pqb, sdx, (pqc + pqc) * sdy);
-      const float il = 1.0f / HGS_LOG2E;
-      const float opi = (pop != 0.0f) ? 1.0f / pop : 0.0f;
-      float2* row = reinterpret_cast<float2*>(pair_rows + (size_t)ppid * HGS_PROW_FLOATS);
-      row[0] = make_float2(x0 * il, x1 * il);
-      row[1] = make_float2(sxx * -0.5f, sxy * -1.0f);
-      row[2] = make_float2(syy * -0.5f, k00 * opi);
-      row[3] = make_float2(a3[0], a3[1]);
-      row[4] = make_float2(a3[2], a3[3]);
-    };
-    for (uint32_t it0 = 0; it0 < maxcnt; it0 += HGS_RB) {
-      const uint32_t bfirst = (uint32_t)__shfl((int)__float_as_uint(c2.w), lane & 48, 64);
-      const unsigned long long act = __ballot((it0 < cnt) && (bfirst <= nc));
-#ifdef HGS_TIMELINE
-      if (tl_nb == 0) tl_w1 = wall_clock64() + (act & 1ull) * 0ull;
-      ++tl_nb;
-      tl_live += ((act & 0xffffull) != 0) + (((act >> 16) & 0xffffull) != 0) + (((act >> 32) & 0xffffull) != 0) + ((act >> 48) != 0);
-#endif
-      const float mxr = c0.x, myr = c0.y, qar = c0.z, qbr = c0.w, qcr = c1.x, opr = c1.y;
-      if (act != 0ull) {
-        __builtin_amdgcn_wave_barrier();
-        float* pb = reinterpret_cast<float*>(srow + 6 * (i >> 1)) + (i & 1);
-        pb[0] = c0.x; pb[2] = c0.y; pb[4] = c0.z; pb[6] = c0.w;
-        pb[8] = c1.x; pb[10] = c1.y; pb[12] = c1.z; pb[14] = c1.w;
-        pb[16] = c2.x; pb[18] = c2.y; pb[20] = c2.w;
-      }
-      const uint2 le_use = le_next;
-      const uint32_t in2 = it0 + 2 * HGS_RB + (uint32_t)i;
-      le_next = list_at(in2);
-      const uint32_t pid_this = pid_cur;
-      pid_cur = le_use.y;
-      gather(le_use, it0 + HGS_RB + (uint32_t)i < cnt, c0, c1, c2);
-      if (act == 0ull) {
-        if (it0 + (uint32_t)i < cnt) {
-          float2* row = reinterpret_cast<float2*>(pair_rows + (size_t)pid_this * HGS_PROW_FLOATS);
-          const float2 zero2 = make_float2(0.f, 0.f);
-          row[0] = zero2; row[1] = zero2; row[2] = zero2; row[3] = zero2; row[4] = zero2;
-        }
-        continue;
-      }
-      __builtin_amdgcn_fence(__ATOMIC_ACQ_REL, "wavefront");
-      __builtin_amdgcn_wave_barrier();
-      auto eval_pair = [&](int u, const float4& P0, const float4& P1, const float4& P2, const float4& P3, const float4& P4,
-                           const float4& P5) {
-        const hgs_f32x2 mx2 = {P0.x, P0.y}, my2 = {P0.z, P0.w}, qa2 = {P1.x, P1.y}, qb2 = {P1.z, P1.w};
-        const hgs_f32x2 qc2 = {P2.x, P2.y}, op2 = {P2.z, P2.w}, cr2 = {P3.x, P3.y}, cg2 = {P3.z, P3.w};
-        const hgs_f32x2 cb2 = {P4.x, P4.y}, cd2 = {P4.z, P4.w};
-        const hgs_f32x2 dx2 = mx2 - pxf, dy2 = my2 - pyf;
-        const hgs_f32x2 m2 = __builtin_elementwise_fma(qa2, dx2, qb2 * dy2);
-        const hgs_f32x2 m3 = qc2 * dy2;
-        const hgs_f32x2 p2 = __builtin_elementwise_fma(dx2, m2, m3 * dy2);
-        const hgs_f32x2 G2 = {__builtin_amdgcn_exp2f(p2.x), __builtin_amdgcn_exp2f(p2.y)};
-        const hgs_f32x2 og2 = op2 * G2;
-        const bool on0 = (p2.x <= 0.0f) & (og2.x >= HGS_ALPHA_MIN) & (__float_as_uint(P5.x) <= nc);
-        const bool on1 = (p2.y <= 0.0f) & (og2.y >= HGS_ALPHA_MIN) & (__float_as_uint(P5.y) <= nc);
-        const hgs_f32x2 am2 = {on0 ? og2.x : 0.0f, on1 ? og2.y : 0.0f};
-        const hgs_f32x2 a2 = {fminf(HGS_ALPHA_MAX, am2.x), fminf(HGS_ALPHA_MAX, am2.y)};
-        const hgs_f32x2 om2 = 1.0f - a2;
-        const hgs_f32x2 rc2 = {__builtin_amdgcn_rcpf(om2.x), __builtin_amdgcn_rcpf(om2.y)};
-        const hgs_f32x2 S2 = __builtin_elementwise_fma(cr2, (hgs_f32x2)(g0), __builtin_elementwise_fma(cg2, (hgs_f32x2)(g1),
-                             __builtin_elementwise_fma(cb2, (hgs_f32x2)(g2), __builtin_elementwise_fma(cd2, (hgs_f32x2)(gd), (hgs_f32x2)(ga)))));
-        const float T1 = T * om2.x;
-        const hgs_f32x2 T2 = {T, T1};
-        const hgs_f32x2 wgt2 = a2 * T2;
-        const float F0 = __builtin_fmaf(-wgt2.x, S2.x, F);
-        const float F1 = __builtin_fmaf(-wgt2.y, S2.y, F0);
-        const hgs_f32x2 Fn2 = {F0, F1};
-        const hgs_f32x2 dl2 = __builtin_elementwise_fma(T2, S2, -(Fn2 * rc2));
-        const hgs_f32x2 k2 = am2 * dl2;
-        T = T1 * om2.y;
-        F = F1;
-        stage_k[u * HGS_STAGE_STRIDE + lane] = k2.x;
-        stage_k[(u + 1) * HGS_STAGE_STRIDE + lane] = k2.y;
-        stage_w[u * HGS_STAGE_STRIDE + lane] = wgt2.x;
-        stage_w[(u + 1) * HGS_STAGE_STRIDE + lane] = wgt2.y;
-      };
-      float4 P[6], N[6];
-#pragma unroll
-      for (int m = 0; m < 6; ++m) P[m] = srow[m];
-#pragma unroll
-      for (int u = 0; u < HGS_RB; u += 2) {
-        if (u + 2 < HGS_RB) {
-#pragma unroll
-          for (int m = 0; m < 6; ++m) N[m] = srow[3 * (u + 2) + m];
-        }
-        __builtin_amdgcn_sched_barrier(0x7f);
-        eval_pair(u, P[0], P[1], P[2], P[3], P[4], P[5]);
-        if (u + 2 < HGS_RB) {
-#pragma unroll
-          for (int m = 0; m < 6; ++m) P[m] = N[m];
-        }
-      }
-      __builtin_amdgcn_fence(__ATOMIC_ACQ_REL, "wavefront");
-      __builtin_amdgcn_wave_barrier();
-      hgs_f32x4 acc1 = {0.f, 0.f, 0.f, 0.f}, acc2 = {0.f, 0.f, 0.f, 0.f}, acc3 = {0.f, 0.f, 0.f, 0.f};
-      {
-        const float* sk = stage_k + i * HGS_STAGE_STRIDE + 16 * j;
-        const float* sw = stage_w + i * HGS_STAGE_STRIDE + 16 * j;
-#pragma unroll
-        for (int q4 = 0; q4 < 4; ++q4) {
-          const float4 bk = *reinterpret_cast<const float4*>(sk + 4 * q4);
-          const float4 bw = *reinterpret_cast<const float4*>(sw + 4 * q4);
-          const float4 t1 = *reinterpret_cast<const float4*>(tabA + 4 * q4);
-          const float4 t2 = *reinterpret_cast<const float4*>(tabA + 16 + 4 * q4);
-          const float kx[4] = {bk.x, bk.y, bk.z, bk.w};
-          const float wx[4] = {bw.x, bw.y, bw.z, bw.w};
-          const float a1x[4] = {t1.x, t1.y, t1.z, t1.w};
-          const float a2x[4] = {t2.x, t2.y, t2.z, t2.w};
-#pragma unroll
-          for (int r = 0; r < 4; ++r) {
-            acc1 = __builtin_amdgcn_mfma_f32_4x4x1f32(a1x[r], kx[r], acc1, 0, 0, 0);
-            acc2 = __builtin_amdgcn_mfma_f32_4x4x1f32(a2x[r], kx[r], acc2, 0, 0, 0);
-            acc3 = __builtin_amdgcn_mfma_f32_4x4x1f32(A3[4 * q4 + r], wx[r], acc3, 0, 0, 0);
-          }
-        }
-      }
-      __builtin_amdgcn_fence(__ATOMIC_ACQ_REL, "wavefront");
-      __builtin_amdgcn_wave_barrier();
-      pmx = mxr; pmy = myr; pqa = qar; pqb = qbr; pqc = qcr; pop = opr; ppid = pid_this;
-      finish(acc1, acc2, acc3, it0);
-    }
-#ifdef HGS_TIMELINE
-    if (lane == 0) {
-      unsigned long long* o = L.keys + ((size_t)grp * HGS_NXCD + die) * 4;
-      const unsigned long long simd_key = ((unsigned long long)(__builtin_amdgcn_s_getreg((31 << 11) | 20) & 0xfu) << 16) |
-                                          (__builtin_amdgcn_s_getreg((31 << 11) | 4) & 0xff30u);
-      o[0] = tl_w0; o[1] = wall_clock64(); o[2] = tl_nb | ((tl_w1 - tl_w0) << 32); o[3] = (unsigned long long)(cnt) | (simd_key << 8) | ((unsigned long long)tl_live << 32) | 1ull << 63;
-    }
-#endif
-    grp = grp_next; item = item_next; have = have_next;
-  }
-}
 
 #define HGS_RED_ROWS 128
 #define HGS_RED_RUNS 4
diff --git a/humangaussian_amd/csrc/render_bwd_blend.h b/humangaussian_amd/csrc/render_bwd_blend.h
--- /dev/null
+++ b/humangaussian_amd/csrc/render_bwd_blend.h
@@ -0,0 +1,288 @@
+extern "C" __global__ void __launch_bounds__(64 * HGS_BWD_BLOCK_WAVES)
+HGS_BWD_NAME(View v, Layout L, const hgs_status* __restrict__ status,
+             const SortRec* __restrict__ recs_all, const float* __restrict__ cstate,
+             const float* __restrict__ out_color,
+             const float* __restrict__ out_depth, const float* __restrict__ out_alpha,
+             const float* __restrict__ dL_dcolor, const float* __restrict__ dL_ddepth,
+             const float* __restrict__ dL_dalpha, float* __restrict__ pair_rows, uint32_t pair_cap) {
+  constexpr bool WIDE = HGS_BWD_WIDE;
+  __shared__ float4 s_rec_all[HGS_BWD_BLOCK_WAVES][4 * HGS_ROW_F4];
+  __shared__ __attribute__((aligned(16))) float stage_k_all[HGS_BWD_BLOCK_WAVES][HGS_RB * HGS_STAGE_STRIDE];
+  __shared__ __attribute__((aligned(16))) float stage_w_all[HGS_BWD_BLOCK_WAVES][HGS_RB * HGS_STAGE_STRIDE];
+  __shared__ uint32_t s_ticket;
+  __shared__ __attribute__((aligned(16))) float s_tabA[4][36];
+  if (status->overflow) return;
+  if ((uint32_t)L.ctr->alloc_ps > pair_cap) return;
+  const int lane = (int)threadIdx.x & 63;
+  const int wv = __builtin_amdgcn_readfirstlane((int)threadIdx.x >> 6);
+  float4* __restrict__ s_rec = s_rec_all[wv];
+  float* __restrict__ stage_k = stage_k_all[wv];
+  float* __restrict__ stage_w = stage_w_all[wv];
+  if (threadIdx.x == 0) s_ticket = HGS_BWD_BLOCK_WAVES;
+  if (threadIdx.x < 128) {
+    const int qs = (int)threadIdx.x >> 5, e = (int)threadIdx.x & 31, t = e & 15;
+    const float u = (float)(t & 3) - 1.5f, w_ = (float)(t >> 2) - 1.5f;
+    s_tabA[qs][e] = e < 16 ? (qs == 0 ? 1.0f : (qs == 1 ? u : (qs == 2 ? w_ : u * u)))
+                           : (qs == 0 ? u * w_ : (qs == 1 ? w_ * w_ : 0.0f));
+  }
+  __syncthreads();
+  const int j = lane >> 4, i = lane & 15;
+  const uint32_t die = blockIdx.x % HGS_NXCD, lb = blockIdx.x / HGS_NXCD, nlb = gridDim.x / HGS_NXCD;
+  const size_t dcap = hgs_die_cells(v.TT);
+  const uint4* __restrict__ it_full = L.items_full + (size_t)die * L.full_cap;
+  const uint4* __restrict__ it_part = L.items_part + (size_t)die * 2 * dcap;
+  const uint32_t n0 = (uint32_t)L.ctr->sched[die][0], n1 = (uint32_t)(L.ctr->sched[die][0] >> 32);
+  const uint32_t n2 = (uint32_t)L.ctr->sched[die][1], n3 = (uint32_t)(L.ctr->sched[die][1] >> 32);
+  const uint32_t ngroups = (n0 + n1 + n2 + n3 + 3u) / 4u;
+  const float4 zero4 = make_float4(0.f, 0.f, 0.f, 0.f);
+  const float4* __restrict__ recs = reinterpret_cast<const float4*>(recs_all);
+  float4* __restrict__ srow = s_rec + j * HGS_ROW_F4;
+
+  const int qsel = lane & 3;
+  const float* __restrict__ tabA = s_tabA[qsel];
+
+#ifdef HGS_TIMELINE
+  unsigned long long tl_w0 = 0, tl_w1 = 0;
+  uint32_t tl_nb = 0, tl_live = 0;
+#endif
+  auto group_of = [&](uint32_t tk) {
+    return tk * nlb + ((tk & 1u) ? nlb - 1u - lb : lb);
+  };
+  uint32_t grp = group_of((uint32_t)wv);
+  uint4 item;
+  bool have = fetch_item(it_full, it_part, dcap, 4u * grp + (uint32_t)j, n0, n1, n2, n3, item);
+  while (grp < ngroups) {
+    uint32_t grp_next;
+    {
+      uint32_t t_next = 0;
+      if (lane == 0) t_next = atomicAdd(&s_ticket, 1u);
+      grp_next = group_of((uint32_t)__builtin_amdgcn_readfirstlane((int)t_next));
+    }
+#ifdef HGS_TIMELINE
+    tl_w0 = wall_clock64(); tl_nb = 0; tl_live = 0;
+#endif
+    const uint32_t key = item.x, cnt = have ? item.y : 0u;
+    const int g = (int)(key >> 4), c = (int)(key & 15u);
+    const int bview = g / v.T, t_ = g % v.T;
+    const int cx0 = (t_ % v.grid_x) * HGS_TILE + (c & 3) * HGS_CELL, cy0 = (t_ / v.grid_x) * HGS_TILE + (c >> 2) * HGS_CELL;
+    const int px = cx0 + (i & 3), py = cy0 + (i >> 2);
+    const float pxf = (float)px, pyf = (float)py;
+    const float cxq = (float)cx0 + 1.5f, cyq = (float)cy0 + 1.5f;
+    const uint32_t tstart1 = L.tile_start[have ? g : 0] - 1u;
+    const uint2* __restrict__ list = L.cell_list + (have ? item.z : 0u);
+    const uint32_t* __restrict__ list4 = reinterpret_cast<const uint32_t*>(L.cell_list) + (have ? item.z : 0u);
+
+    const uint32_t safe_rec = tstart1 + 1u;
+    auto list_at = [&](uint32_t e) {
+      if (WIDE) return list[(e < cnt) ? e : 0u];
+      return make_uint2(list4[(e < cnt) ? e : 0u], 0u);
+    };
+    auto gather = [&](const uint2 le, bool valid, float4& r0, float4& r1, float4& r2, uint32_t& pid) {
+      const uint32_t idx = valid ? (WIDE ? le.x : le.x & HGS_LE_INDEX_MASK) : safe_rec;
+      r0 = recs[3 * (size_t)idx]; r1 = recs[3 * (size_t)idx + 1];
+      const float4 t2 = recs[3 * (size_t)idx + 2];
+      pid = WIDE ? le.y : __float_as_uint(t2.w) + (le.x >> HGS_LE_RANK_SHIFT);
+      r2 = make_float4(t2.x, t2.y, t2.z, __uint_as_float(valid ? idx - tstart1 : 0xffffffffu));
+    };
+    float4 c0, c1, c2;
+    uint32_t pid_cur;
+    uint2 le_next = list_at((uint32_t)i);
+    const uint2 le_second = list_at(HGS_RB + (uint32_t)i);
+    const bool inside = have && px < v.W && py < v.H;
+    const bool has_state = inside && item.w != 0xffffffffu;
+    float g0, g1, g2, gd, ga, fp, T, F;
+    uint32_t nc;
+    {
+      const size_t HW = (size_t)v.H * v.W, pix = inside ? (size_t)py * v.W + px : 0;
+      const size_t o1 = inside ? (size_t)bview * HW : 0, o3 = 3 * o1;
+      const float* pc = dL_dcolor ? dL_dcolor : out_color;
+      const float* pd = dL_ddepth ? dL_ddepth : out_depth;
+      const float* pa = dL_dalpha ? dL_dalpha : out_alpha;
+      const float r_g0 = pc[o3 + pix], r_g1 = pc[o3 + HW + pix], r_g2 = pc[o3 + 2 * HW + pix];
+      const float r_gd = pd[o1 + pix], r_ga = pa[o1 + pix];
+      const float r_c0 = out_color[o3 + pix], r_c1 = out_color[o3 + HW + pix], r_c2 = out_color[o3 + 2 * HW + pix];
+      const float r_d = out_depth[o1 + pix], r_a = out_alpha[o1 + pix];
+      const uint32_t r_nc = L.n_contrib[o1 + pix];
+      const float* cs = cstate + (size_t)(has_state ? item.w : 0u) * HGS_CSTATE_FLOATS + i;
+      const float r_s0 = cs[0 * 16], r_s1 = cs[1 * 16], r_s2 = cs[2 * 16], r_s3 = cs[3 * 16], r_s4 = cs[4 * 16], r_s5 = cs[5 * 16];
+      gather(le_next, (uint32_t)i < cnt, c0, c1, c2, pid_cur);
+      g0 = (inside && dL_dcolor) ? r_g0 : 0.0f; g1 = (inside && dL_dcolor) ? r_g1 : 0.0f; g2 = (inside && dL_dcolor) ? r_g2 : 0.0f;
+      gd = (inside && dL_ddepth) ? r_gd : 0.0f;
+      ga = (inside && dL_dalpha) ? r_ga : 0.0f;
+      fp = inside ? r_c0 * g0 + r_c1 * g1 + r_c2 * g2 + r_d * gd + r_a * ga : 0.0f;
+      nc = inside ? r_nc : 0u;
+      T = has_state ? r_s0 : 1.0f;
+      F = has_state ? r_s1 * g0 + r_s2 * g1 + r_s3 * g2 + r_s4 * gd + r_s5 * ga : 0.0f;
+      F = fp - F;
+    }
+    __builtin_amdgcn_wave_barrier();
+    stage_k[0 * 64 + lane] = g0; stage_k[1 * 64 + lane] = g1; stage_k[2 * 64 + lane] = g2; stage_k[3 * 64 + lane] = gd;
+    __builtin_amdgcn_fence(__ATOMIC_ACQ_REL, "wavefront");
+    __builtin_amdgcn_wave_barrier();
+    float A3[16];
+    {
+      const float* ar = stage_k + qsel * 64 + 16 * (lane >> 4);
+#pragma unroll
+      for (int q4 = 0; q4 < 4; ++q4) {
+        const float4 a = *reinterpret_cast<const float4*>(ar + 4 * q4);
+        A3[4 * q4 + 0] = a.x; A3[4 * q4 + 1] = a.y; A3[4 * q4 + 2] = a.z; A3[4 * q4 + 3] = a.w;
+      }
+    }
+    __builtin_amdgcn_fence(__ATOMIC_ACQ_REL, "wavefront");
+    __builtin_amdgcn_wave_barrier();
+
+    uint32_t maxcnt = (uint32_t)__builtin_amdgcn_readlane((int)cnt, 0);
+    maxcnt = max(maxcnt, (uint32_t)__builtin_amdgcn_readlane((int)cnt, 16));
+    maxcnt = max(maxcnt, (uint32_t)__builtin_amdgcn_readlane((int)cnt, 32));
+    maxcnt = max(maxcnt, (uint32_t)__builtin_amdgcn_readlane((int)cnt, 48));
+
+    le_next = le_second;
+    uint4 item_next;
+    const bool have_next = fetch_item(it_full, it_part, dcap, 4u * grp_next + (uint32_t)j, n0, n1, n2, n3, item_next);
+    {
+      const uint32_t first = (uint32_t)__shfl((int)__float_as_uint(c2.w), lane & 48, 64);
+      if (!(have && nc >= first)) { T = 1.0f; F = 0.0f; nc = 0; }
+    }
+
+    float pmx = 0.f, pmy = 0.f, pqa = 0.f, pqb = 0.f, pqc = 0.f, pop = 0.f;
+    uint32_t ppid = 0;
+    auto finish = [&](const hgs_f32x4& a1, const hgs_f32x4& a2, const hgs_f32x4& a3, uint32_t it0) {
+      if (it0 + (uint32_t)i >= cnt) return;
+      const float a = pmx - cxq, bb = pmy - cyq;
+      const float k00 = a1[0], k10 = a1[1], k01 = a1[2], k20 = a1[3], k11 = a2[0], k02 = a2[1];
+      const float sdx = __builtin_fmaf(a, k00, -k10), sdy = __builtin_fmaf(bb, k00, -k01);
+      const float sxx = __builtin_fmaf(a, __builtin_fmaf(a, k00, -(k10 + k10)), k20);
+      const float sxy = __builtin_fmaf(a, sdy, __builtin_fmaf(-bb, k10, k11));
+      const float syy = __builtin_fmaf(bb, __builtin_fmaf(bb, k00, -(k01 + k01)), k02);
+      const float x0 = __builtin_fmaf(pqa + pqa, sdx, pqb * sdy);
+      const float x1 = __builtin_fmaf(pqb, sdx, (pqc + pqc) * sdy);
+      const float il = 1.0f / HGS_LOG2E;
+      const float opi = (pop != 0.0f) ? 1.0f / pop : 0.0f;
+      float2* row = reinterpret_cast<float2*>(pair_rows + (size_t)ppid * HGS_PROW_FLOATS);
+      row[0] = make_float2(x0 * il, x1 * il);
+      row[1] = make_float2(sxx * -0.5f, sxy * -1.0f);
+      row[2] = make_float2(syy * -0.5f, k00 * opi);
+      row[3] = make_float2(a3[0], a3[1]);
+      row[4] = make_float2(a3[2], a3[3]);
+    };
+    for (uint32_t it0 = 0; it0 < maxcnt; it0 += HGS_RB) {
+      const uint32_t bfirst = (uint32_t)__shfl((int)__float_as_uint(c2.w), lane & 48, 64);
+      const unsigned long long act = __ballot((it0 < cnt) && (bfirst <= nc));
+#ifdef HGS_TIMELINE
+      if (tl_nb == 0) tl_w1 = wall_clock64() + (act & 1ull) * 0ull;
+      ++tl_nb;
+      tl_live += ((act & 0xffffull) != 0) + (((act >> 16) & 0xffffull) != 0) + (((act >> 32) & 0xffffull) != 0) + ((act >> 48) != 0);
+#endif
+      const float mxr = c0.x, myr = c0.y, qar = c0.z, qbr = c0.w, qcr = c1.x, opr = c1.y;
+      if (act != 0ull) {
+        __builtin_amdgcn_wave_barrier();
+        float* pb = reinterpret_cast<float*>(srow + 6 * (i >> 1)) + (i & 1);
+        pb[0] = c0.x; pb[2] = c0.y; pb[4] = c0.z; pb[6] = c0.w;
+        pb[8] = c1.x; pb[10] = c1.y; pb[12] = c1.z; pb[14] = c1.w;
+        pb[16] = c2.x; pb[18] = c2.y; pb[20] = c2.w;
+      }
+      const uint2 le_use = le_next;
+      const uint32_t in2 = it0 + 2 * HGS_RB + (uint32_t)i;
+      le_next = list_at(in2);
+      const uint32_t pid_this = pid_cur;
+      gather(le_use, it0 + HGS_RB + (uint32_t)i < cnt, c0, c1, c2, pid_cur);
+      if (act == 0ull) {
+        if (it0 + (uint32_t)i < cnt) {
+          float2* row = reinterpret_cast<float2*>(pair_rows + (size_t)pid_this * HGS_PROW_FLOATS);
+          const float2 zero2 = make_float2(0.f, 0.f);
+          row[0] = zero2; row[1] = zero2; row[2] = zero2; row[3] = zero2; row[4] = zero2;
+        }
+        continue;
+      }
+      __builtin_amdgcn_fence(__ATOMIC_ACQ_REL, "wavefront");
+      __builtin_amdgcn_wave_barrier();
+      auto eval_pair = [&](int u, const float4& P0, const float4& P1, const float4& P2, const float4& P3, const float4& P4,
+                           const float4& P5) {
+        const hgs_f32x2 mx2 = {P0.x, P0.y}, my2 = {P0.z, P0.w}, qa2 = {P1.x, P1.y}, qb2 = {P1.z, P1.w};
+        const hgs_f32x2 qc2 = {P2.x, P2.y}, op2 = {P2.z, P2.w}, cr2 = {P3.x, P3.y}, cg2 = {P3.z, P3.w};
+        const hgs_f32x2 cb2 = {P4.x, P4.y}, cd2 = {P4.z, P4.w};
+        const hgs_f32x2 dx2 = mx2 - pxf, dy2 = my2 - pyf;
+        const hgs_f32x2 m2 = __builtin_elementwise_fma(qa2, dx2, qb2 * dy2);
+        const hgs_f32x2 m3 = qc2 * dy2;
+        const hgs_f32x2 p2 = __builtin_elementwise_fma(dx2, m2, m3 * dy2);
+        const hgs_f32x2 G2 = {__builtin_amdgcn_exp2f(p2.x), __builtin_amdgcn_exp2f(p2.y)};
+        const hgs_f32x2 og2 = op2 * G2;
+        const bool on0 = (p2.x <= 0.0f) & (og2.x >= HGS_ALPHA_MIN) & (__float_as_uint(P5.x) <= nc);
+        const bool on1 = (p2.y <= 0.0f) & (og2.y >= HGS_ALPHA_MIN) & (__float_as_uint(P5.y) <= nc);
+        const hgs_f32x2 am2 = {on0 ? og2.x : 0.0f, on1 ? og2.y : 0.0f};
+        const hgs_f32x2 a2 = {fminf(HGS_ALPHA_MAX, am2.x), fminf(HGS_ALPHA_MAX, am2.y)};
+        const hgs_f32x2 om2 = 1.0f - a2;
+        const hgs_f32x2 rc2 = {__builtin_amdgcn_rcpf(om2.x), __builtin_amdgcn_rcpf(om2.y)};
+        const hgs_f32x2 S2 = __builtin_elementwise_fma(cr2, (hgs_f32x2)(g0), __builtin_elementwise_fma(cg2, (hgs_f32x2)(g1),
+                             __builtin_elementwise_fma(cb2, (hgs_f32x2)(g2), __builtin_elementwise_fma(cd2, (hgs_f32x2)(gd), (hgs_f32x2)(ga)))));
+        const float T1 = T * om2.x;
+        const hgs_f32x2 T2 = {T, T1};
+        const hgs_f32x2 wgt2 = a2 * T2;
+        const float F0 = __builtin_fmaf(-wgt2.x, S2.x, F);
+        const float F1 = __builtin_fmaf(-wgt2.y, S2.y, F0);
+        const hgs_f32x2 Fn2 = {F0, F1};
+        const hgs_f32x2 dl2 = __builtin_elementwise_fma(T2, S2, -(Fn2 * rc2));
+        const hgs_f32x2 k2 = am2 * dl2;
+        T = T1 * om2.y;
+        F = F1;
+        stage_k[u * HGS_STAGE_STRIDE + lane] = k2.x;
+        stage_k[(u + 1) * HGS_STAGE_STRIDE + lane] = k2.y;
+        stage_w[u * HGS_STAGE_STRIDE + lane] = wgt2.x;
+        stage_w[(u + 1) * HGS_STAGE_STRIDE + lane] = wgt2.y;
+      };
+      float4 P[6], N[6];
+#pragma unroll
+      for (int m = 0; m < 6; ++m) P[m] = srow[m];
+#pragma unroll
+      for (int u = 0; u < HGS_RB; u += 2) {
+        if (u + 2 < HGS_RB) {
+#pragma unroll
+          for (int m = 0; m < 6; ++m) N[m] = srow[3 * (u + 2) + m];
+        }
+        __builtin_amdgcn_sched_barrier(0x7f);
+        eval_pair(u, P[0], P[1], P[2], P[3], P[4], P[5]);
+        if (u + 2 < HGS_RB) {
+#pragma unroll
+          for (int m = 0; m < 6; ++m) P[m] = N[m];
+        }
+      }
+      __builtin_amdgcn_fence(__ATOMIC_ACQ_REL, "wavefront");
+      __builtin_amdgcn_wave_barrier();
+      hgs_f32x4 acc1 = {0.f, 0.f, 0.f, 0.f}, acc2 = {0.f, 0.f, 0.f, 0.f}, acc3 = {0.f, 0.f, 0.f, 0.f};
+      {
+        const float* sk = stage_k + i * HGS_STAGE_STRIDE + 16 * j;
+        const float* sw = stage_w + i * HGS_STAGE_STRIDE + 16 * j;
+#pragma unroll
+        for (int q4 = 0; q4 < 4; ++q4) {
+          const float4 bk = *reinterpret_cast<const float4*>(sk + 4 * q4);
+          const float4 bw = *reinterpret_cast<const float4*>(sw + 4 * q4);
+          const float4 t1 = *reinterpret_cast<const float4*>(tabA + 4 * q4);
+          const float4 t2 = *reinterpret_cast<const float4*>(tabA + 16 + 4 * q4);
+          const float kx[4] = {bk.x, bk.y, bk.z, bk.w};
+          const float wx[4] = {bw.x, bw.y, bw.z, bw.w};
+          const float a1x[4] = {t1.x, t1.y, t1.z, t1.w};
+          const float a2x[4] = {t2.x, t2.y, t2.z, t2.w};
+#pragma unroll
+          for (int r = 0; r < 4; ++r) {
+            acc1 = __builtin_amdgcn_mfma_f32_4x4x1f32(a1x[r], kx[r], acc1, 0, 0, 0);
+            acc2 = __builtin_amdgcn_mfma_f32_4x4x1f32(a2x[r], kx[r], acc2, 0, 0, 0);
+            acc3 = __builtin_amdgcn_mfma_f32_4x4x1f32(A3[4 * q4 + r], wx[r], acc3, 0, 0, 0);
+          }
+        }
+      }
+      __builtin_amdgcn_fence(__ATOMIC_ACQ_REL, "wavefront");
+      __builtin_amdgcn_wave_barrier();
+      pmx = mxr; pmy = myr; pqa = qar; pqb = qbr; pqc = qcr; pop = opr; ppid = pid_this;
+      finish(acc1, acc2, acc3, it0);
+    }
+#ifdef HGS_TIMELINE
+    if (lane == 0) {
+      unsigned long long* o = L.keys + ((size_t)grp * HGS_NXCD + die) * 4;
+      const unsigned long long simd_key = ((unsigned long long)(__builtin_amdgcn_s_getreg((31 << 11) | 20) & 0xfu) << 16) |
+                                          (__builtin_amdgcn_s_getreg((31 << 11) | 4) & 0xff30u);
+      o[0] = tl_w0; o[1] = wall_clock64(); o[2] = tl_nb | ((tl_w1 - tl_w0) << 32); o[3] = (unsigned long long)(cnt) | (simd_key << 8) | ((unsigned long long)tl_live << 32) | 1ull << 63;
+    }
+#endif
+    grp = grp_next; item = item_next; have = have_next;
+  }
+}
diff --git a/humangaussian_amd/csrc/render_fwd.hip b/humangaussian_amd/csrc/render_fwd.hip
--- a/humangaussian_amd/csrc/render_fwd.hip
+++ b/humangaussian_amd/csrc/render_fwd.hip
@@ -28,6 +28,15 @@
   s.last = upd ? __float_as_uint(r2.w) : s.last;
 }
 
+template <bool WIDE>
+struct FwdList {
+  const uint2* __restrict__ p8;
+  const uint32_t* __restrict__ p4;
+  __device__ __forceinline__ FwdList(const Layout& L, uint32_t base)
+      : p8(L.cell_list + base), p4(reinterpret_cast<const uint32_t*>(L.cell_list) + base) {}
+  __device__ __forceinline__ uint32_t index(uint32_t e) const { return WIDE ? p8[e].x : (p4[e] & HGS_LE_INDEX_MASK); }
+};
+
 }
 
 #define HGS_FWD_C4 4
@@ -49,7 +58,7 @@
   return __uint_as_float(s32.x) + __uint_as_float(s32.y);
 }
 
-template <bool STORE>
+template <bool STORE, bool WIDE>
 __device__ __forceinline__ void render_fwd_cell4(const View& v, const Layout& L, uint32_t key,
                                                  const SortRec* __restrict__ recs_all,
                                                  float* __restrict__ cstate,
@@ -68,7 +77,7 @@
   const uint32_t tstart1 = L.tile_start[g] - 1u;
   const CellInfo ci = L.cell_info[key];
   const uint32_t len = ci.len, sbase = ci.sbase;
-  const uint2* __restrict__ list = L.cell_list + ci.base;
+  const FwdList<WIDE> list(L, ci.base);
   const float4* __restrict__ recs = reinterpret_cast<const float4*>(recs_all);
   const float4 zero4 = make_float4(0.f, 0.f, 0.f, 0.f);
 
@@ -77,7 +86,7 @@
   float C0 = 0.f, C1 = 0.f, C2 = 0.f, D = 0.f, Wt = 0.f;
   uint32_t last = 0;
 
-  auto load_idx = [&](uint32_t e) { return list[(e < len) ? e : 0u].x; };
+  auto load_idx = [&](uint32_t e) { return list.index((e < len) ? e : 0u); };
   auto gather = [&](uint32_t idx_raw, bool valid, float4& r0, float4& r1, float4& r2) {
     const uint32_t idx = valid ? idx_raw : tstart1 + 1u;
     r0 = recs[3 * (size_t)idx]; r1 = recs[3 * (size_t)idx + 1];
@@ -176,7 +185,7 @@
   return L.fwd_cells[((size_t)x * HGS_NFC + (size_t)c) * dcap + (q - base)];
 }
 
-template <bool STORE>
+template <bool STORE, bool WIDE>
 __device__ __forceinline__ void render_fwd_cells(const View& v, const Layout& L, const uint32_t* pre, uint32_t wave_id, int w,
                                                  const SortRec* __restrict__ recs_all,
                                                  float* __restrict__ cstate,
@@ -216,7 +225,7 @@
     const CellInfo ci = L.cell_info[key];
     len = ci.len; base = ci.base; sbase = ci.sbase;
   }
-  const uint2* __restrict__ list = L.cell_list + base;
+  const FwdList<WIDE> list(L, base);
   const float4* __restrict__ recs = reinterpret_cast<const float4*>(recs_all);
   float4* __restrict__ srow = s_rec_w + j * HGS_ROW_F4;
 
@@ -228,7 +237,7 @@
 
   const float4 zero4 = make_float4(0.f, 0.f, 0.f, 0.f);
   const uint32_t safe_rec = have ? tstart1 + 1u : 0u;
-  auto load_idx = [&](uint32_t e) { return list[(e < len) ? e : 0u].x; };
+  auto load_idx = [&](uint32_t e) { return list.index((e < len) ? e : 0u); };
   auto gather = [&](uint32_t idx_raw, bool valid, float4& r0, float4& r1, float4& r2) {
     const uint32_t idx = valid ? idx_raw : safe_rec;
     r0 = recs[3 * (size_t)idx]; r1 = recs[3 * (size_t)idx + 1];
@@ -318,7 +327,7 @@
   L.n_contrib[o1 + pix] = 0u;
 }
 
-#define HGS_RENDER_FWD_KERNEL(NAME, STORE)                                                                 \
+#define HGS_RENDER_FWD_KERNEL(NAME, STORE, WIDE)                                                                 \
   extern "C" __global__ void __launch_bounds__(HGS_FWD_THREADS) NAME(                                       \
       View v, Layout L, uint32_t cell_blocks, hgs_status* __restrict__ status,                               \
       hgs_status* __restrict__ status_host, const SortRec* __restrict__ recs, float* __restrict__ cstate, float* __restrict__ out_color,           \
@@ -367,14 +376,18 @@
         uint32_t q = it;                                                                                     \
         int c4 = 0;                                                                                          \
         _Pragma("unroll") for (int c = 0; c < HGS_FWD_C4 - 1; ++c) if (c4 == c && q >= cnt4[c]) { q -= cnt4[c]; c4 = c + 1; } \
-        render_fwd_cell4<STORE>(v, L, fwd_cell_key(L, dcap, s_pre, c4, q), recs, cstate, out_color,         \
+        render_fwd_cell4<STORE, WIDE>(v, L, fwd_cell_key(L, dcap, s_pre, c4, q), recs, cstate, out_color,         \
                                 out_depth, out_alpha, s_rec[w]);                                             \
       } else {                                                                                               \
-        render_fwd_cells<STORE>(v, L, s_pre, it - n4, w, recs, cstate, out_color, out_depth, out_alpha, s_rec[w]); \
+        render_fwd_cells<STORE, WIDE>(v, L, s_pre, it - n4, w, recs, cstate, out_color, out_depth, out_alpha, s_rec[w]); \
       }                                                                                                      \
       HGS_TLI_END(it, (it < n4 ? 0 : -1));                                                                   \
     }                                                                                                        \
     HGS_TL_END(4, HGS_TLI_TAG());                                                                            \
   }
-HGS_RENDER_FWD_KERNEL(hgs_k_render_fwd_store, true)
-HGS_RENDER_FWD_KERNEL(hgs_k_render_fwd_nostore, false)
+HGS_RENDER_FWD_KERNEL(hgs_k_render_fwd_store, true, HGS_EM_WIDE)
+HGS_RENDER_FWD_KERNEL(hgs_k_render_fwd_nostore, false, HGS_EM_WIDE)
+#ifdef HGS_NARROW_CELL_ELEMENTS
+HGS_RENDER_FWD_KERNEL(hgs_k_render_fwd_store_ch, true, true)
+HGS_RENDER_FWD_KERNEL(hgs_k_render_fwd_nostore_ch, false, true)
+#endif
```

After: 648.3 million. 1.8% lower.
